# ivanalberico/End-To-End-Self-Supervised-SLAM

Measured on AMD Instinct MI355X. Metric: online refinement steps/sec @640x480, seq_len=60, higher is better.
Workload: dtype f32

## Files before the change

### end-to-end-self-supervised-slam_amd/csrc/conv.hip

```cpp
#include <cassert>
#include <type_traits>

#include "e2e_common.h"

typedef float f4v __attribute__((ext_vector_type(4)));
typedef float f16v __attribute__((ext_vector_type(16)));

#define CBK 16

enum { ACT_NONE = 0, ACT_RELU = 1, ACT_ELU = 2, ACT_DISP = 3 };

struct ConvArgs {
    const float* src0;
    const float* src1;
    const float* w;
    const float* scale;
    const float* shift;
    const float* res;
    float* out;
    int B, Hs, Ws;
    int Cin, C1, up;
    int Hd, Wd;
    int Ncols, ldw;
    int KH, KW, stride, pad, pad_mode;
// ... 1060 lines not shown
                        int ys = oh * a.stride + b_kh[j] - a.pad, xs = ow * a.stride + b_kw[j] - a.pad;
                        bool ok = true;
                        if (a.pad_mode == 1) { ys = reflect1(ys, a.Hs); xs = reflect1(xs, a.Ws); }
                        else ok = ys >= 0 && ys < a.Hs && xs >= 0 && xs < a.Ws;
                        if (ok) {
                            const int ci = b_ci[j];
                            const float* q = (ci < a.C1)
                                ? a.src0 + (((int64_t)b * Hl + ys / a.up) * Wl + xs / a.up) * a.C1 + ci
                                : a.src1 + (((int64_t)b * a.Hs + ys) * a.Ws + xs) * C2 + (ci - a.C1);
                            v = *(const f4v*)q;
                        }
                    } else if (a.has_bias && b_col[j] == Kconv) {
                        v[0] = 1.f;
                    }
                } else {
#pragma unroll
                    for (int e = 0; e < 4; ++e) {
                        const int n = b_col[j] + e;
                        if (n < Kconv) {
                            const int tp = n / a.Cin, c = n - tp * a.Cin, kh1 = tp / a.KW, kw1 = tp - kh1 * a.KW;
                            const int ys = oh * a.stride + kh1 - a.pad, xs = ow * a.stride + kw1 - a.pad;
                            if (ys >= 0 && ys < a.Hs && xs >= 0 && xs < a.Ws)
                                v[e] = (a.src0[(((int64_t)b * a.Hs + ys) * a.Ws + xs) * a.Cin + c] - a.in_sub) * a.in_mul;
                        } else if (a.has_bias && n == Kconv) v[e] = 1.f;
                    }
                }
            }
            breg[j] = v;
            pow_[j] += CBK;
            while (pow_[j] >= a.Wo) { pow_[j] -= a.Wo; if (++poh[j] == a.Ho) { poh[j] = 0; ++pb[j]; } }
        }
        ++ld_chunk;
    };
    auto store_chunk = [&](int buf) {
#pragma unroll
        for (int j = 0; j < A_PER; ++j) {
            const int idx = tid + j * NT;
            if (idx >= A_CNT) continue;
            const int kr = idx / (BM / 4), mq = idx - kr * (BM / 4);
            *(f4v*)&As[buf][kr][mq * 4] = areg[j];
        }
#pragma unroll
        for (int j = 0; j < B_PER; ++j) {
            const int idx = tid + j * NT;
            if (idx >= B_CNT) continue;
            const int nq = idx - b_kr[j] * (BN / 4);
            *(f4v*)&Bs[buf][b_kr[j]][nq * 4] = breg[j];
        }
    };
    f16v acc;
#pragma unroll
    for (int r = 0; r < 16; ++r) acc[r] = 0.f;
    if (nchunks > 0) {
        load_chunk();
        store_chunk(0);
    }
    __syncthreads();
    const int khalf = lane >> 5;
    for (int c = 0; c < nchunks; ++c) {
        const int buf = c & 1;
        if (c + 1 < nchunks) load_chunk();
        float av[CBK / 2], bv[CBK / 2];
#pragma unroll
        for (int kk = 0; kk < CBK / 2; ++kk) {
            av[kk] = As[buf][kk * 2 + khalf][wm * 32 + (lane & 31)];
            bv[kk] = Bs[buf][kk * 2 + khalf][wn * 32 + (lane & 31)];
        }
#pragma unroll
        for (int kk = 0; kk < CBK / 2; ++kk) acc = __builtin_amdgcn_mfma_f32_32x32x2f32(av[kk], bv[kk], acc, 0, 0, 0);
        __builtin_amdgcn_sched_group_barrier(0x100, CBK / 2, 0);
        __builtin_amdgcn_sched_group_barrier(0x008, CBK / 2, 0);
        if (c + 1 < nchunks) store_chunk(buf ^ 1);
        __syncthreads();
    }
    float* slab = a.slabs + (int64_t)bz * a.Mpad * a.Npad;
    const int n = nn0 + wn * 32 + (lane & 31);
#pragma unroll
    for (int r = 0; r < 16; ++r) {
        const int m = m0 + wm * 32 + (r & 3) + 8 * (r >> 2) + 4 * khalf;
        if (m < a.Mpad && n < a.Npad) slab[(int64_t)m * a.Npad + n] = acc[r];
    }
}

template <int WM, int WN, int CB>
struct WgradGemm4Lds {
    float As[2][CB][32 * WM];
    float Bs[2][CB][32 * WN];
};

template <int WM, int WN, int CB, bool TWO, class Ids>
__device__ __forceinline__ void wgrad_gemm4_body(const WgradArgs& a, const Ids& wg, float (*As)[CB][32 * WM], float (*Bs)[CB][32 * WN]) {
    constexpr int BM = 32 * WM, BN = 32 * WN, NT = 256;
    constexpr int A_CNT = CB * (BM / 4), B_CNT = CB * (BN / 4);
    constexpr int A_PER = A_CNT / NT, B_PER = B_CNT / NT;
    static_assert(A_CNT % NT == 0 && B_CNT % NT == 0, "tile / thread-count mismatch");
    const int tid = threadIdx.x, lane = tid & 63, wave = tid >> 6;
    const int wm = wave % WM, wn = wave / WM;
    unsigned bx, by, bz;
    set_wave_priority(wg.lin());
    {
        const unsigned lin = xcd_contiguous(wg.lin(), wg.gx() * wg.gy() * wg.gz());
        bx = lin % wg.gx();
        const unsigned t_ = lin / wg.gx();
        by = t_ % wg.gy();
        bz = t_ / wg.gy();
    }
    const int m0 = by * BM, nn0 = bx * BN;
    const int P = a.B * a.Ho * a.Wo;
    const int p0 = (int)((int64_t)bz * a.pix_per_slice);
    const int p1 = (p0 + a.pix_per_slice < P) ? (int)(p0 + a.pix_per_slice) : P;
    const int npix = (p1 > p0) ? p1 - p0 : 0;
    const int nchunks = (npix + CB - 1) / CB;
    const int sh = a.up >> 1;
    const int Hl = a.Hs >> sh, Wl = a.Ws >> sh, C2 = a.Cin - a.C1;
    const int Kconv = a.KH * a.KW * a.Cin;
    constexpr unsigned OOB = 0x80000000u;
    const __amdgpu_buffer_rsrc_t rsz = __builtin_amdgcn_make_buffer_rsrc((void*)a.dz, 0, (int)((int64_t)P * a.Cout * 4), 0x00020000);
    const __amdgpu_buffer_rsrc_t rs0 = __builtin_amdgcn_make_buffer_rsrc((void*)a.src0, 0, (int)((int64_t)a.B * Hl * Wl * a.C1 * 4), 0x00020000);
    const __amdgpu_buffer_rsrc_t rs1 = __builtin_amdgcn_make_buffer_rsrc((void*)(a.src1 ? a.src1 : a.src0), 0,
                                                                         (int)(a.src1 ? (int64_t)a.B * a.Hs * a.Ws * C2 * 4 : 0), 0x00020000);

    int a_kr[A_PER];
    unsigned a_off[A_PER];
#pragma unroll
    for (int j = 0; j < A_PER; ++j) {
        const int idx = tid + j * NT;
        a_kr[j] = idx / (BM / 4);
        const int m = m0 + (idx - a_kr[j] * (BM / 4)) * 4;
        a_off[j] = (m < a.Cout) ? (unsigned)(a_kr[j] * a.Cout + m) * 4u : OOB;
    }
    const float inv_cin = 1.0f / (float)a.Cin, inv_kw = 1.0f / (float)a.KW;
    constexpr int QG = (BN / 4) / B_PER;
    static_assert(NT / QG == CB, "one pixel row of the chunk per thread");
    const int b_row = tid / QG;
    int b_quad[B_PER], b_kh[B_PER], b_kw[B_PER], b_ci[B_PER];
    bool b_conv[B_PER], b_ones[B_PER], b_src0[B_PER];
#pragma unroll
    for (int j = 0; j < B_PER; ++j) {
        b_quad[j] = tid % QG + j * QG;
        const int col = nn0 + b_quad[j] * 4;
        b_conv[j] = col < Kconv;
        b_ones[j] = a.has_bias && col == Kconv;
        const int cc = b_conv[j] ? col : 0;
        int tap = (int)((float)cc * inv_cin);
        tap -= (tap * a.Cin > cc) ? 1 : 0;
        tap += ((tap + 1) * a.Cin <= cc) ? 1 : 0;
        b_ci[j] = cc - tap * a.Cin;
        b_src0[j] = b_ci[j] < a.C1;
        int tkh = (int)((float)tap * inv_kw);
        tkh -= (tkh * a.KW > tap) ? 1 : 0;
        tkh += ((tkh + 1) * a.KW <= tap) ? 1 : 0;
        b_kh[j] = tkh - a.pad;
        b_kw[j] = tap - tkh * a.KW - a.pad;
    }
    const int hw = a.Ho * a.Wo;
    const float inv_hw = 1.0f / (float)hw, inv_wo = 1.0f / (float)a.Wo;
    const bool reflect = a.pad_mode == 1;
    f4v areg[2][A_PER], breg[2][B_PER], breg1[2][TWO ? B_PER : 1];
    int left_of[2] = {0, 0};
    int ld_chunk = 0;
    int cur_b = 0, cur_oh = 0, cur_ow = 0;
    const bool incremental = a.Wo >= 11 && a.Ho >= 3;
    auto load_chunk = [&](int set) {
        const int left = npix - ld_chunk * CB;
        left_of[set] = left;
        const int pc = p0 + ld_chunk * CB;
        const int soffz = pc * a.Cout * 4;
#pragma unroll
        for (int j = 0; j < A_PER; ++j)
            areg[set][j] = __builtin_bit_cast(f4v, __builtin_amdgcn_raw_buffer_load_b128(rsz, (a_kr[j] < left) ? a_off[j] : OOB, soffz, 0));
        if (!incremental || ld_chunk == 0) {
            const unsigned p = (unsigned)(pc + b_row);
            unsigned b = (unsigned)((float)p * inv_hw);
            b -= (__umul24(b, (unsigned)hw) > p) ? 1u : 0u;
            b += (__umul24(b + 1u, (unsigned)hw) <= p) ? 1u : 0u;
            const unsigned r = p - __umul24(b, (unsigned)hw);
            unsigned oh = (unsigned)((float)r * inv_wo);
            oh -= (__umul24(oh, (unsigned)a.Wo) > r) ? 1u : 0u;
            oh += (__umul24(oh + 1u, (unsigned)a.Wo) <= r) ? 1u : 0u;
            cur_b = (int)b; cur_oh = (int)oh; cur_ow = (int)(r - __umul24(oh, (unsigned)a.Wo));
        } else {
            cur_ow += CB;
#pragma unroll
            for (int t = 0; t < 3; ++t) {
                const bool c = cur_ow >= a.Wo;
                cur_ow -= c ? a.Wo : 0;
                cur_oh += c ? 1 : 0;
            }
            const bool c = cur_oh >= a.Ho;
            cur_oh -= c ? a.Ho : 0;
            cur_b += c ? 1 : 0;
        }
        const int ybase = (int)__umul24((unsigned)cur_oh, (unsigned)a.stride), xbase = (int)__umul24((unsigned)cur_ow, (unsigned)a.stride);
#pragma unroll
        for (int j = 0; j < B_PER; ++j) {
            const int ys0 = ybase + b_kh[j], xs0 = xbase + b_kw[j];
            const bool inside = ((unsigned)ys0 < (unsigned)a.Hs) & ((unsigned)xs0 < (unsigned)a.Ws);
            const int ys = reflect ? reflect1(ys0, a.Hs) : ys0, xs = reflect ? reflect1(xs0, a.Ws) : xs0;
            const bool ok = b_conv[j] & (b_row < left) & (reflect | inside);
            const unsigned pix0 = umad24(umad24((unsigned)cur_b, (unsigned)Hl, (unsigned)(ys >> sh)), (unsigned)Wl, (unsigned)(xs >> sh));
            const unsigned o0 = umad24(pix0, (unsigned)a.C1, (unsigned)b_ci[j]) * 4u;
            breg[set][j] = __builtin_bit_cast(f4v, __builtin_amdgcn_raw_buffer_load_b128(rs0, o0 | ((ok && b_src0[j]) ? 0u : OOB), 0, 0));
            if (TWO) {
                const unsigned pix1 = umad24(umad24((unsigned)cur_b, (unsigned)a.Hs, (unsigned)ys), (unsigned)a.Ws, (unsigned)xs);
                const unsigned o1 = umad24(pix1, (unsigned)C2, (unsigned)(b_ci[j] - a.C1)) * 4u;
                breg1[set][j] = __builtin_bit_cast(f4v, __builtin_amdgcn_raw_buffer_load_b128(rs1, o1 | ((ok && !b_src0[j]) ? 0u : OOB), 0, 0));
            }
        }
        ++ld_chunk;
    };
    auto store_chunk = [&](int buf, int set) {
#pragma unroll
        for (int j = 0; j < A_PER; ++j) {
            const int idx = tid + j * NT;
            *(f4v*)&As[buf][a_kr[j]][(idx - a_kr[j] * (BM / 4)) * 4] = areg[set][j];
        }
#pragma unroll
        for (int j = 0; j < B_PER; ++j) {
            f4v v = breg[set][j];
            if (TWO) v = b_src0[j] ? v : breg1[set][j];
            const f4v ones = {(b_row < left_of[set]) ? 1.f : 0.f, 0.f, 0.f, 0.f};
            *(f4v*)&Bs[buf][b_row][b_quad[j] * 4] = b_ones[j] ? ones : v;
        }
    };
    f16v acc;
#pragma unroll
    for (int r = 0; r < 16; ++r) acc[r] = 0.f;
    load_chunk(0);
    load_chunk(1);
    store_chunk(0, 0);
    __syncthreads();
    const int khalf = lane >> 5;
    float fa[2][CB / 2], fb[2][CB / 2];
    auto read_frags = [&](auto buf_c) {
        constexpr int buf = decltype(buf_c)::value;
#pragma unroll
        for (int kk = 0; kk < CB / 2; ++kk) {
            fa[buf][kk] = As[buf][kk * 2 + khalf][wm * 32 + (lane & 31)];
            fb[buf][kk] = Bs[buf][kk * 2 + khalf][wn * 32 + (lane & 31)];
        }
    };
    auto pipe_step = [&](auto buf_c) {
        constexpr int buf = decltype(buf_c)::value;
        load_chunk(buf);
        store_chunk(buf ^ 1, buf ^ 1);
#pragma unroll
        for (int kk = 0; kk < CB / 4; ++kk) acc = __builtin_amdgcn_mfma_f32_32x32x2f32(fa[buf][kk], fb[buf][kk], acc, 0, 0, 0);
#pragma unroll
        for (int g = 0; g < CB / 4; ++g) {
            __builtin_amdgcn_sched_group_barrier(0x008, 1, 0);
            __builtin_amdgcn_sched_group_barrier(0x002, 14, 0);
            __builtin_amdgcn_sched_group_barrier(0x004, 4, 0);
            __builtin_amdgcn_sched_group_barrier(0x020, 1, 0);
            __builtin_amdgcn_sched_group_barrier(0x200, 1, 0);
        }
        __builtin_amdgcn_sched_barrier(0);
        __syncthreads();
        __builtin_amdgcn_sched_barrier(0);
        read_frags(std::integral_constant<int, buf ^ 1>{});
#pragma unroll
        for (int kk = CB / 4; kk < CB / 2; ++kk) acc = __builtin_amdgcn_mfma_f32_32x32x2f32(fa[buf][kk], fb[buf][kk], acc, 0, 0, 0);
#pragma unroll
        for (int g = 0; g < CB / 4; ++g) {
            __builtin_amdgcn_sched_group_barrier(0x008, 1, 0);
            __builtin_amdgcn_sched_group_barrier(0x100, 2, 0);
        }
        __builtin_amdgcn_sched_barrier(0);
    };
    if (nchunks > 0) {
        read_frags(std::integral_constant<int, 0>{});
        int c = 0;
        for (; c + 1 < nchunks; c += 2) {
            pipe_step(std::integral_constant<int, 0>{});
            pipe_step(std::integral_constant<int, 1>{});
        }
        if (c < nchunks) pipe_step(std::integral_constant<int, 0>{});
    }
    {
        const __amdgpu_buffer_rsrc_t rsl = __builtin_amdgcn_make_buffer_rsrc((void*)(a.slabs + (int64_t)bz * a.Mpad * a.Npad), 0, a.Mpad * a.Npad * 4, 0x00020000);
        const int n = nn0 + wn * 32 + (lane & 31), mb = m0 + wm * 32 + 4 * khalf;
        const int rows_left = a.Mpad - mb;
        const unsigned voff = (n < a.Npad && rows_left > 0) ? (unsigned)(mb * a.Npad + n) * 4u : OOB;
#pragma unroll
        for (int r = 0; r < 16; ++r) {
            const int dr = (r & 3) + 8 * (r >> 2);
            const float v = acc[r];
            __builtin_amdgcn_raw_buffer_store_b32(__float_as_uint(v), rsl, (dr < rows_left) ? voff : OOB, dr * a.Npad * 4, 0);
        }
    }
}

template <int WM, int WN, int CB, bool TWO>
__global__ __launch_bounds__(256) void k_wgrad_gemm4(WgradArgs a) {
    __shared__ float As[2][CB][32 * WM];
    __shared__ float Bs[2][CB][32 * WN];
    wgrad_gemm4_body<WM, WN, CB, TWO>(a, HwIds{}, As, Bs);
}

struct PairGrid {
    unsigned dgx, dgy, dgz;
    unsigned wgx, wgy, wgz;
    unsigned first;
    int wgrad_first;
};

template <int DWM, int DWN, bool TWO>
__global__ __launch_bounds__(256) void k_conv_bwd_pair(ConvArgs d, WgradArgs w, PairGrid pg) {
    using DL = ConvGemmLds<DWM, DWN, 1, 1, 4, 32>;
    using WL = WgradGemm4Lds<2, 2, 32>;
    static_assert(64 * DWM * DWN == 256, "both parts run 256 threads");
    __shared__ union { DL d; WL w; } lds;
    const bool in_first = blockIdx.x < pg.first;
    const unsigned l = in_first ? blockIdx.x : blockIdx.x - pg.first;
    if (in_first == (pg.wgrad_first != 0)) {
        if (l >= pg.wgx * pg.wgy * pg.wgz) return;
        wgrad_gemm4_body<2, 2, 32, TWO>(w, PartIds{l, pg.wgx, pg.wgy, pg.wgz}, lds.w.As, lds.w.Bs);
    } else {
        if (l >= pg.dgx * pg.dgy * pg.dgz) return;
        conv_gemm_body<DWM, DWN, 1, 1, 4, true, 32>(d, PartIds{l, pg.dgx, pg.dgy, pg.dgz}, lds.d.As, lds.d.Bs);
    }
}

template <int NTL, int CB>
__global__ __launch_bounds__(256) void k_wgrad_gemm16(WgradArgs a) {
    constexpr int BM = 16, BN = 16 * NTL, BNS = (BN % 32 == 16) ? BN : BN + 16, NT = 256;
    constexpr int A_CNT = CB * (BM / 4), B_CNT = CB * (BN / 4);
    constexpr int A_PER = (A_CNT + NT - 1) / NT, B_PER = (B_CNT + NT - 1) / NT;
    static_assert(2 * CB * (BM + BNS) >= 3 * NTL * 4 * 64, "tile memory is reused for the cross-wave sum");
    __shared__ float smem[2 * CB * (BM + BNS)];
    float (*As)[CB][BM] = reinterpret_cast<float (*)[CB][BM]>(smem);
    float (*Bs)[CB][BNS] = reinterpret_cast<float (*)[CB][BNS]>(smem + 2 * CB * BM);
    const int tid = threadIdx.x, lane = tid & 63, wave = tid >> 6;
    WGRAD_BLOCK_IDS
    (void)by;
    const int nn0 = bx * BN;
    const int64_t P = (int64_t)a.B * a.Ho * a.Wo;
    const int64_t p0 = (int64_t)bz * a.pix_per_slice;
    const int64_t p1 = (p0 + a.pix_per_slice < P) ? p0 + a.pix_per_slice : P;
    const int npix = (p1 > p0) ? (int)(p1 - p0) : 0;
    const int nchunks = (npix + CB - 1) / CB;
    const int sh = a.up >> 1;
    const int Hl = a.Hs >> sh, Wl = a.Ws >> sh, C2 = a.Cin - a.C1;
    const int Kconv = a.KH * a.KW * a.Cin;
    constexpr unsigned OOB = 0x80000000u;
    const __amdgpu_buffer_rsrc_t rsz = __builtin_amdgcn_make_buffer_rsrc((void*)a.dz, 0, (int)(P * a.Cout * 4), 0x00020000);
    const __amdgpu_buffer_rsrc_t rs0 = __builtin_amdgcn_make_buffer_rsrc((void*)a.src0, 0, (int)((int64_t)a.B * Hl * Wl * a.C1 * 4), 0x00020000);
    const __amdgpu_buffer_rsrc_t rs1 = __builtin_amdgcn_make_buffer_rsrc((void*)(a.src1 ? a.src1 : a.src0), 0,
                                                                         (int)(a.src1 ? (int64_t)a.B * a.Hs * a.Ws * C2 * 4 : 0), 0x00020000);
    int a_kr[A_PER];
    unsigned a_off[A_PER];
#pragma unroll
    for (int j = 0; j < A_PER; ++j) {
        const int idx = tid + j * NT;
        a_kr[j] = idx / (BM / 4);
        const int m = (idx - a_kr[j] * (BM / 4)) * 4;
        a_off[j] = (idx < A_CNT && m < a.Cout) ? (unsigned)(a_kr[j] * a.Cout + m) * 4u : OOB;
    }
    int b_kr[B_PER], b_kh[B_PER], b_kw[B_PER], b_ci[B_PER], pb[B_PER], poh[B_PER], pow_[B_PER];
    bool b_conv[B_PER], b_ones[B_PER], b_src0[B_PER];
#pragma unroll
    for (int j = 0; j < B_PER; ++j) {
        const int idx = tid + j * NT;
        b_kr[j] = idx / (BN / 4);
        const int col = nn0 + (idx - b_kr[j] * (BN / 4)) * 4;
        b_conv[j] = idx < B_CNT && col < Kconv;
        b_ones[j] = idx < B_CNT && a.has_bias && col == Kconv;
        const int tap = b_conv[j] ? col / a.Cin : 0;
        b_ci[j] = b_conv[j] ? col - tap * a.Cin : 0;
        b_src0[j] = b_ci[j] < a.C1;
        b_kh[j] = tap / a.KW;
        b_kw[j] = tap - b_kh[j] * a.KW;
        const int64_t p = p0 + b_kr[j];
        const int hw = a.Ho * a.Wo;
        pb[j] = (int)(p / hw);
        const int r = (int)(p - (int64_t)pb[j] * hw);
        poh[j] = r / a.Wo;
        pow_[j] = r - poh[j] * a.Wo;
    }
    f4v areg[A_PER], breg[B_PER];
    int ld_chunk = 0;
    auto load_chunk = [&]() {
        const int left = npix - ld_chunk * CB;
        const int soffz = (int)((p0 + (int64_t)ld_chunk * CB) * a.Cout * 4);
#pragma unroll
        for (int j = 0; j < A_PER; ++j)
            areg[j] = __builtin_bit_cast(f4v, __builtin_amdgcn_raw_buffer_load_b128(rsz, (a_kr[j] < left) ? a_off[j] : OOB, soffz, 0));
#pragma unroll
        for (int j = 0; j < B_PER; ++j) {
            int ys = poh[j] * a.stride + b_kh[j] - a.pad, xs = pow_[j] * a.stride + b_kw[j] - a.pad;
            bool ok = b_conv[j] && b_kr[j] < left;
            if (a.pad_mode == 1) { ys = reflect1(ys, a.Hs); xs = reflect1(xs, a.Ws); }
            else ok = ok && ys >= 0 && ys < a.Hs && xs >= 0 && xs < a.Ws;
            const unsigned o0 = (unsigned)(((pb[j] * Hl + (ys >> sh)) * Wl + (xs >> sh)) * a.C1 + b_ci[j]) * 4u;
            const unsigned o1 = (unsigned)(((pb[j] * a.Hs + ys) * a.Ws + xs) * C2 + (b_ci[j] - a.C1)) * 4u;
            f4v v = __builtin_bit_cast(f4v, __builtin_amdgcn_raw_buffer_load_b128(rs0, (ok && b_src0[j]) ? o0 : OOB, 0, 0));
            if (a.src1 != nullptr) {
                const f4v v1 = __builtin_bit_cast(f4v, __builtin_amdgcn_raw_buffer_load_b128(rs1, (ok && !b_src0[j]) ? o1 : OOB, 0, 0));
                v = b_src0[j] ? v : v1;
            }
            if (b_ones[j]) v = (f4v){(b_kr[j] < left) ? 1.f : 0.f, 0.f, 0.f, 0.f};
            breg[j] = v;
            pow_[j] += CB;
#pragma unroll
            for (int w2 = 0; w2 < 4; ++w2)
                if (pow_[j] >= a.Wo) { pow_[j] -= a.Wo; if (++poh[j] == a.Ho) { poh[j] = 0; ++pb[j]; } }
        }
        ++ld_chunk;
    };
    auto store_chunk = [&](int buf) {
#pragma unroll
        for (int j = 0; j < A_PER; ++j) {
            const int idx = tid + j * NT;
            if (idx >= A_CNT) continue;
            *(f4v*)&As[buf][a_kr[j]][(idx - a_kr[j] * (BM / 4)) * 4] = areg[j];
        }
#pragma unroll
        for (int j = 0; j < B_PER; ++j) {
            const int idx = tid + j * NT;
            if (idx >= B_CNT) continue;
            *(f4v*)&Bs[buf][b_kr[j]][(idx - b_kr[j] * (BN / 4)) * 4] = breg[j];
        }
    };
    f4v acc[NTL];
#pragma unroll
    for (int t = 0; t < NTL; ++t) acc[t] = (f4v){0.f, 0.f, 0.f, 0.f};
    if (nchunks > 0) {
        load_chunk();
        store_chunk(0);
    }
    __syncthreads();
    const int kq = lane >> 4, l16 = lane & 15;
    for (int c = 0; c < nchunks; ++c) {
        const int buf = c & 1;
        if (c + 1 < nchunks) load_chunk();
#pragma unroll
        for (int ks = 0; ks < CB / 16; ++ks) {
            const int row = wave * (CB / 4) + ks * 4 + kq;
            const float av = As[buf][row][l16];
#pragma unroll
            for (int t = 0; t < NTL; ++t) acc[t] = __builtin_amdgcn_mfma_f32_16x16x4f32(av, Bs[buf][row][t * 16 + l16], acc[t], 0, 0, 0);
        }
        if (c + 1 < nchunks) store_chunk(buf ^ 1);
        __syncthreads();
    }
    float* red = smem;
    if (wave > 0) {
#pragma unroll
        for (int t = 0; t < NTL; ++t)
#pragma unroll
            for (int i = 0; i < 4; ++i) red[((wave - 1) * NTL * 4 + t * 4 + i) * 64 + lane] = acc[t][i];
    }
    __syncthreads();
    if (wave > 0) return;
    float* slab = a.slabs + (int64_t)bz * a.Mpad * a.Npad;
#pragma unroll
    for (int t = 0; t < NTL; ++t)
#pragma unroll
        for (int i = 0; i < 4; ++i) {
            float v = acc[t][i];
#pragma unroll
            for (int w2 = 0; w2 < 3; ++w2) v += red[(w2 * NTL * 4 + t * 4 + i) * 64 + lane];
            const int m = 4 * kq + i, n = nn0 + t * 16 + l16;
            if (n < a.Npad) slab[(int64_t)m * a.Npad + n] = v;
        }
}

struct ThinWgradArgs {
    const float* dz;
    const float* src0;
    const float* src1;
    float* slabs;
    int B, Hd, Wd, Cin, C1, up, npad, has_bias, tiles_x, nxg;
};

template <int MT>
__global__ __launch_bounds__(256) void k_wgrad3x3_thin(ThinWgradArgs a) {
    constexpr int TH = 4, TW = 64, PH = TH + 2, PW = TW + 2, CO = 16 * MT, NA = 10 * MT;
    __shared__ float smem[PH * PW * 16 + TH * TW * CO];
    float* patch = smem;
    float* dzs = smem + PH * PW * 16;
    const int tid = threadIdx.x, lane = tid & 63, wave = tid >> 6, l16 = lane & 15, kq = lane >> 4;
    const int nhalf = a.Cin >> 4, n0 = a.C1 >> 4;
    const int b = blockIdx.z / nhalf, hf = blockIdx.z % nhalf;
    const bool first = hf < n0;
    const int sh = first ? (a.up >> 1) : 0, Cs = first ? a.C1 : a.Cin - a.C1, cs0 = (first ? hf : hf - n0) * 16;
    const int Hs = a.Hd >> sh, Ws = a.Wd >> sh;
    const int y0 = blockIdx.y * TH;
    const float* sb = (first ? a.src0 : a.src1) + (int64_t)b * Hs * Ws * Cs + cs0;
    const float* zb = a.dz + (int64_t)b * a.Hd * a.Wd * CO;
    f4v acc[NA];
#pragma unroll
    for (int t = 0; t < NA; ++t) acc[t] = (f4v){0.f, 0.f, 0.f, 0.f};
    const float one = (l16 == 0) ? 1.f : 0.f;
    for (int tx = 0; tx < a.tiles_x; ++tx) {
        const int x0 = (blockIdx.x * a.tiles_x + tx) * TW;
        if (x0 >= a.Wd) break;
        __syncthreads();
        for (int idx = tid; idx < PH * PW * 4; idx += 256) {
            const int q = idx & 3, pix = idx >> 2;
            const int py = pix / PW, px = pix - py * PW;
            const int Y = min(max(reflect1(y0 - 1 + py, a.Hd), 0), a.Hd - 1), X = min(max(reflect1(x0 - 1 + px, a.Wd), 0), a.Wd - 1);
            *(f4v*)&patch[pix * 16 + q * 4] = *(const f4v*)(sb + ((int64_t)(Y >> sh) * Ws + (X >> sh)) * Cs + q * 4);
        }
        for (int idx = tid; idx < TH * TW * (CO / 4); idx += 256) {
            const int q = idx % (CO / 4), pix = idx / (CO / 4);
            const int r = pix / TW, x = pix - r * TW;
            const bool ok = y0 + r < a.Hd && x0 + x < a.Wd;
            *(f4v*)&dzs[pix * CO + q * 4] = ok ? *(const f4v*)(zb + ((int64_t)(y0 + r) * a.Wd + x0 + x) * CO + q * 4) : (f4v){0.f, 0.f, 0.f, 0.f};
        }
        __syncthreads();
        const float* ap = dzs + (wave * TW + kq) * CO + l16;
        const float* bp = patch + (wave * PW + kq) * 16 + l16;
#pragma unroll 2
        for (int ks = 0; ks < TW / 4; ++ks) {
            float av[MT];
#pragma unroll
            for (int mt = 0; mt < MT; ++mt) av[mt] = ap[ks * 4 * CO + mt * 16];
#pragma unroll
            for (int t = 0; t < 9; ++t) {
                const float bv = bp[((t / 3) * PW + (t % 3)) * 16 + ks * 64];
#pragma unroll
                for (int mt = 0; mt < MT; ++mt) acc[mt * 10 + t] = __builtin_amdgcn_mfma_f32_16x16x4f32(av[mt], bv, acc[mt * 10 + t], 0, 0, 0);
            }
#pragma unroll
            for (int mt = 0; mt < MT; ++mt) acc[mt * 10 + 9] = __builtin_amdgcn_mfma_f32_16x16x4f32(av[mt], one, acc[mt * 10 + 9], 0, 0, 0);
        }
    }
    float* red = smem;
    static_assert(2 * NA * 4 * 64 <= PH * PW * 16 + TH * TW * CO, "reduction scratch");
    __syncthreads();
    if (wave >= 2) {
#pragma unroll
        for (int t = 0; t < NA; ++t)
#pragma unroll
            for (int i = 0; i < 4; ++i) red[((wave - 2) * NA * 4 + t * 4 + i) * 64 + lane] = acc[t][i];
    }
    __syncthreads();
    if (wave < 2) {
#pragma unroll
        for (int t = 0; t < NA; ++t)
#pragma unroll
            for (int i = 0; i < 4; ++i) acc[t][i] += red[(wave * NA * 4 + t * 4 + i) * 64 + lane];
    }
    __syncthreads();
    if (wave == 1) {
#pragma unroll
        for (int t = 0; t < NA; ++t)
#pragma unroll
            for (int i = 0; i < 4; ++i) red[(t * 4 + i) * 64 + lane] = acc[t][i];
    }
    __syncthreads();
    if (wave != 0) return;
    const int64_t sid = ((int64_t)b * gridDim.y + blockIdx.y) * a.nxg + blockIdx.x;
    float* slab = a.slabs + sid * CO * a.npad;
    const int kconv = 9 * a.Cin, cg0 = hf * 16;
#pragma unroll
    for (int mt = 0; mt < MT; ++mt)
#pragma unroll
        for (int t = 0; t < 10; ++t)
#pragma unroll
            for (int i = 0; i < 4; ++i) {
                const float v = acc[mt * 10 + t][i] + red[((mt * 10 + t) * 4 + i) * 64 + lane];
                const int co = mt * 16 + 4 * kq + i;
                if (t < 9) slab[co * a.npad + t * a.Cin + cg0 + l16] = v;
                else if (a.has_bias && hf == 0 && l16 == 0) slab[co * a.npad + kconv] = v;
            }
}

struct StemWgradArgs {
    const float* dz;
    const float* src;
    float* slabs;
    int B, Hs, Ws, Hd, Wd, tiles_x, nxg;
    float in_sub, in_mul;
};

__global__ __launch_bounds__(256) void k_wgrad7x7_stem(StemWgradArgs a) {
    constexpr int TH = 4, TW = 32, PH = 2 * TH + 6, PW = 2 * TW + 5, ROW = 208, NPAD = 148;
    __shared__ float patch[PH * ROW];
    __shared__ float dzs[TH * TW * 64];
    const int tid = threadIdx.x, lane = tid & 63, wave = tid >> 6, l16 = lane & 15, kq = lane >> 4;
    const int y0 = blockIdx.y * TH, b = blockIdx.z;
    int offn[10];
#pragma unroll
    for (int nt = 0; nt < 10; ++nt) {
        const int k = 16 * nt + l16;
        offn[nt] = k + (k / 21) * (ROW - 21) + 48 * kq;
    }
    f4v acc[10];
#pragma unroll
    for (int nt = 0; nt < 10; ++nt) acc[nt] = (f4v){0.f, 0.f, 0.f, 0.f};
    const float* sb = a.src + (int64_t)b * a.Hs * a.Ws * 3;
    const float* zb = a.dz + (int64_t)b * a.Hd * a.Wd * 64;
    for (int tx = 0; tx < a.tiles_x; ++tx) {
        const int x0 = (blockIdx.x * a.tiles_x + tx) * TW;
        if (x0 >= a.Wd) break;
        __syncthreads();
        for (int idx = tid; idx < PH * ROW; idx += 256) {
            const int py = idx / ROW, e = idx - py * ROW;
            const int Y = 2 * y0 - 3 + py, X = 2 * x0 - 3 + e / 3;
            const bool ok = e < 3 * PW && Y >= 0 && Y < a.Hs && X >= 0 && X < a.Ws;
            patch[idx] = ok ? (sb[((int64_t)Y * a.Ws + X) * 3 + (e - (e / 3) * 3)] - a.in_sub) * a.in_mul : 0.f;
        }
        for (int idx = tid; idx < TH * TW * 16; idx += 256) {
            const int q = idx & 15, pix = idx >> 4;
            const int r = pix / TW, x = pix - r * TW;
            const bool ok = y0 + r < a.Hd && x0 + x < a.Wd;
            *(f4v*)&dzs[pix * 64 + q * 4] = ok ? *(const f4v*)(zb + ((int64_t)(y0 + r) * a.Wd + x0 + x) * 64 + q * 4) : (f4v){0.f, 0.f, 0.f, 0.f};
        }
        __syncthreads();
#pragma unroll 1
        for (int r = 0; r < TH; ++r) {
            const float* ap = dzs + (r * TW + 8 * kq) * 64 + 16 * wave + l16;
            const float* bp = patch + 2 * r * ROW;
#pragma unroll 2
            for (int ks = 0; ks < TW / 4; ++ks) {
                const float av = ap[ks * 64];
#pragma unroll
                for (int nt = 0; nt < 10; ++nt) acc[nt] = __builtin_amdgcn_mfma_f32_16x16x4f32(av, bp[offn[nt] + ks * 6], acc[nt], 0, 0, 0);
            }
        }
    }
    float* slab = a.slabs + (((int64_t)b * gridDim.y + blockIdx.y) * a.nxg + blockIdx.x) * 64 * NPAD;
#pragma unroll
    for (int nt = 0; nt < 10; ++nt)
#pragma unroll
        for (int i = 0; i < 4; ++i) {
            const int n = 16 * nt + l16;
            if (n < 147) slab[(16 * wave + 4 * kq + i) * NPAD + n] = acc[nt][i];
        }
}

struct TapWgradArgs {
    const float* dz;
    const float* src0;
    const float* src1;
    float* slabs;
    int B, H, W, Cin, C1, up, Cout, reflect, has_bias, Mpad, Npad;
    int ptx, pty;
    int nchunks, cps;
};

#define TAP_NT 192
template <bool BIAS>
__global__ __launch_bounds__(TAP_NT) void k_wgrad3x3_taps(TapWgradArgs a) {
    __shared__ float dzs[64 * 32];
    __shared__ float xs[100 * 32];
    const int tid = threadIdx.x, lane = tid & 63, wave = tid >> 6, kh_ = lane >> 5, l32 = lane & 31;
    const int ci0 = blockIdx.x * 32, co0 = blockIdx.y * 32;
    const bool first = ci0 < a.C1;
    const int sh = first ? (a.up >> 1) : 0, Cs = first ? a.C1 : a.Cin - a.C1, cs0 = first ? ci0 : ci0 - a.C1;
    const int Hs = a.H >> sh, Ws = a.W >> sh;
    const float* sbase = first ? a.src0 : a.src1;
    const int c_begin = blockIdx.z * a.cps, c_end = min(c_begin + a.cps, a.nchunks);
    const bool want_bias = BIAS && blockIdx.x == 0 && wave == 0;
    f16v acc[3], accb;
#pragma unroll
    for (int t = 0; t < 3; ++t)
#pragma unroll
        for (int r = 0; r < 16; ++r) acc[t][r] = 0.f;
#pragma unroll
    for (int r = 0; r < 16; ++r) accb[r] = 0.f;
    const float one = (l32 == 0) ? 1.f : 0.f;
    f4v rz[3], rx[5];
    auto load_chunk = [&](int g) {
        const int b = g / (a.pty * a.ptx), rem = g - b * (a.pty * a.ptx), py = rem / a.ptx, px = rem - py * a.ptx;
        const int y0 = py * 8, x0 = px * 8;
        const float* zb = a.dz + (int64_t)b * a.H * a.W * a.Cout + co0;
        const float* sb = sbase + (int64_t)b * Hs * Ws * Cs + cs0;
#pragma unroll
        for (int i = 0; i < 3; ++i) {
            const int f = tid + TAP_NT * i, pix = f >> 3, q = f & 7, y = y0 + (pix >> 3), x = x0 + (pix & 7);
            const bool ok = f < 512 && y < a.H && x < a.W;
            rz[i] = ok ? *(const f4v*)(zb + ((int64_t)y * a.W + x) * a.Cout + q * 4) : (f4v){0.f, 0.f, 0.f, 0.f};
        }
#pragma unroll
        for (int i = 0; i < 5; ++i) {
            const int f = tid + TAP_NT * i;
            f4v v = {0.f, 0.f, 0.f, 0.f};
            if (f < 800) {
                const int pix = f >> 3, q = f & 7;
                int y = y0 - 1 + pix / 10, x = x0 - 1 + pix % 10;
                bool ok = true;
                if (a.reflect) {
                    y = min(max(reflect1(y, a.H), 0), a.H - 1);
                    x = min(max(reflect1(x, a.W), 0), a.W - 1);
                } else {
                    ok = y >= 0 && y < a.H && x >= 0 && x < a.W;
                }
                if (ok) v = *(const f4v*)(sb + ((int64_t)(y >> sh) * Ws + (x >> sh)) * Cs + q * 4);
            }
            rx[i] = v;
        }
    };
    auto store_chunk = [&]() {
#pragma unroll
        for (int i = 0; i < 3; ++i) {
            const int f = tid + TAP_NT * i;
            if (f < 512) *(f4v*)&dzs[f * 4] = rz[i];
        }
#pragma unroll
        for (int i = 0; i < 5; ++i) {
            const int f = tid + TAP_NT * i;
            if (f < 800) *(f4v*)&xs[f * 4] = rx[i];
        }
    };
    if (c_begin < c_end) load_chunk(c_begin);
    const float* ap = dzs + kh_ * 32 + l32;
    const float* bp = xs + (kh_ + wave * 10) * 32 + l32;
    for (int c = c_begin; c < c_end; ++c) {
        __syncthreads();
        store_chunk();
        __syncthreads();
        if (c + 1 < c_end) load_chunk(c + 1);
        constexpr int QB = 4, NQ = 32 / QB;
        float av[2][QB], bv[2][QB][3];
        auto read_q = [&](int set, int qt) {
#pragma unroll
            for (int j = 0; j < QB; ++j) {
                const int ks = QB * qt + j, q0 = (ks >> 2) * 10 + 2 * (ks & 3);
                av[set][j] = ap[2 * ks * 32];
#pragma unroll
                for (int t = 0; t < 3; ++t) bv[set][j][t] = bp[(q0 + t) * 32];
            }
        };
        auto pin_q = [&](int set) {
#pragma unroll
            for (int j = 0; j < QB; ++j) {
                asm volatile("" : "+v"(av[set][j]));
#pragma unroll
                for (int t = 0; t < 3; ++t) asm volatile("" : "+v"(bv[set][j][t]));
            }
        };
        read_q(0, 0);
#pragma unroll
        for (int qt = 0; qt < NQ; ++qt) {
            if (qt + 1 < NQ) read_q((qt + 1) & 1, qt + 1);
            __builtin_amdgcn_sched_barrier(0);
            pin_q(qt & 1);
            __builtin_amdgcn_sched_barrier(0);
#pragma unroll
            for (int j = 0; j < QB; ++j) {
#pragma unroll
                for (int t = 0; t < 3; ++t) acc[t] = __builtin_amdgcn_mfma_f32_32x32x2f32(av[qt & 1][j], bv[qt & 1][j][t], acc[t], 0, 0, 0);
                if (BIAS && want_bias) accb = __builtin_amdgcn_mfma_f32_32x32x2f32(av[qt & 1][j], one, accb, 0, 0, 0);
            }
            __builtin_amdgcn_sched_barrier(0);
        }
    }
    float* slab = a.slabs + (int64_t)blockIdx.z * a.Mpad * a.Npad;
#pragma unroll
    for (int t = 0; t < 3; ++t)
#pragma unroll
        for (int r = 0; r < 16; ++r) {
            const int m = co0 + (r & 3) + 8 * (r >> 2) + 4 * kh_;
            slab[(int64_t)m * a.Npad + (wave * 3 + t) * a.Cin + ci0 + l32] = acc[t][r];
        }
    if (BIAS && want_bias && l32 == 0) {
#pragma unroll
        for (int r = 0; r < 16; ++r) slab[(int64_t)(co0 + (r & 3) + 8 * (r >> 2) + 4 * kh_) * a.Npad + 9 * a.Cin] = accb[r];
    }
}

template <int ZL>
__device__ __forceinline__ void wgrad_reduce_group(const float* __restrict__ slabs, int S, int Mpad, int Npad, int Cout, int Cin, int KH, int KW, int has_bias,
                                                   float* __restrict__ dw, float* __restrict__ dbias, int accumulate, const float* __restrict__ scale,
                                                   int64_t base, int e, int w, f4v (*part)[64]) {
    const int Kconv = KH * KW * Cin, Ng = Kconv + (has_bias ? 1 : 0);
    const int nq = (Ng + 3) / 4;
    const int64_t totalq = (int64_t)Cout * nq;
    const int64_t slab_q = (int64_t)Mpad * Npad / 4;
    const f4v zero = {0.f, 0.f, 0.f, 0.f};
    const int64_t q = base + e;
    const bool on = q < totalq;
    const int m = on ? (int)(q / nq) : 0, n = on ? (int)(q - (int64_t)m * nq) * 4 : 0;
    const f4v* src = (const f4v*)(slabs + (int64_t)m * Npad + n);
    f4v sacc = zero;
    int z = w;
    for (; z + 3 * ZL < S; z += 4 * ZL) {
        f4v v[4];
#pragma unroll
        for (int j = 0; j < 4; ++j) v[j] = on ? src[(int64_t)(z + ZL * j) * slab_q] : zero;
#pragma unroll
        for (int j = 0; j < 4; ++j) sacc += v[j];
    }
    for (; z < S; z += ZL) sacc += on ? src[(int64_t)z * slab_q] : zero;
    part[w][e] = sacc;
    __syncthreads();
    if (w == 0 && on) {
        f4v t = part[0][e];
#pragma unroll
        for (int j = 1; j < ZL; ++j) t += part[j][e];
        const float sc = scale ? scale[m] : 1.f;
#pragma unroll
        for (int k = 0; k < 4; ++k) {
            const int nn = n + k;
            if (nn < Kconv) {
                const int tap = nn / Cin, ci = nn - tap * Cin, kh = tap / KW, kw = tap - kh * KW;
                float* d = dw + (((int64_t)m * Cin + ci) * KH + kh) * KW + kw;
                const float v = scale ? t[k] * sc : t[k];
                *d = accumulate ? *d + v : v;
            } else if (nn == Kconv && dbias) {
                dbias[m] = accumulate ? dbias[m] + t[k] : t[k];
            }
        }
    }
    __syncthreads();
}

template <int ZL>
__global__ __launch_bounds__(64 * ZL) void k_wgrad_reduce(const float* __restrict__ slabs, int S, int Mpad, int Npad, int Cout, int Cin,
                                                         int KH, int KW, int has_bias, float* __restrict__ dw, float* __restrict__ dbias,
                                                         int accumulate, const float* __restrict__ scale) {
    __shared__ f4v part[ZL][64];
    const int64_t totalq = (int64_t)Cout * ((KH * KW * Cin + (has_bias ? 1 : 0) + 3) / 4);
    for (int64_t base = (int64_t)blockIdx.x * 64; base < totalq; base += (int64_t)gridDim.x * 64)
        wgrad_reduce_group<ZL>(slabs, S, Mpad, Npad, Cout, Cin, KH, KW, has_bias, dw, dbias, accumulate, scale, base, threadIdx.x & 63, threadIdx.x >> 6, part);
}

__global__ __launch_bounds__(512) void k_wgrad_reduce_batched(const e2e_wgrad_reduce_desc* __restrict__ d, int n, long long total_items) {
    __shared__ f4v part[8][64];
    const int e = threadIdx.x & 63, w = threadIdx.x >> 6;
    for (long long item = blockIdx.x; item < total_items; item += gridDim.x) {
        int lo = 0, hi = n - 1;
        while (lo < hi) {
            const int mid = (lo + hi + 1) >> 1;
            if (d[mid].first_item <= item) lo = mid; else hi = mid - 1;
        }
        const e2e_wgrad_reduce_desc D = d[lo];
        const long long local = item - D.first_item;
        if (D.zl == 8)
            wgrad_reduce_group<8>(D.slabs, D.S, D.Mpad, D.Npad, D.Cout, D.Cin, D.KH, D.KW, D.has_bias, D.dw, D.dbias, D.accumulate, D.scale, local * 64, e, w, part);
        else
            wgrad_reduce_group<2>(D.slabs, D.S, D.Mpad, D.Npad, D.Cout, D.Cin, D.KH, D.KW, D.has_bias, D.dw, D.dbias, D.accumulate, D.scale,
                                  (local * 4 + (w >> 1)) * 64, e, w & 1, part + 2 * (w >> 1));
    }
}

__global__ __launch_bounds__(256) void k_weight_layouts(const float* __restrict__ w, int Cout, int Cin, int KH, int KW,
                                                        float* __restrict__ wf, int ldf, float* __restrict__ wb, int ldb) {
    const int64_t total = (int64_t)Cout * Cin * KH * KW;
    for (int64_t i = (int64_t)blockIdx.x * 256 + threadIdx.x; i < total; i += (int64_t)gridDim.x * 256) {
        int64_t t = i;
        const int kw = (int)(t % KW); t /= KW;
        const int kh = (int)(t % KH); t /= KH;
        const int ci = (int)(t % Cin); t /= Cin;
        const int co = (int)t;
        const float v = w[i];
        if (wf) wf[((int64_t)(kh * KW + kw) * Cin + ci) * ldf + co] = v;
        if (wb) wb[((int64_t)(kh * KW + kw) * Cout + co) * ldb + ci] = v;
    }
}

constexpr int WL_TS = 32, WL_ELEMS = 1024, WL_MAXL = 256;

template <int T>
__device__ __forceinline__ void weight_layout_tile(const float* __restrict__ w, float* __restrict__ wf, float* __restrict__ wb, const float* __restrict__ bsc,
                                                   int Cout, int Cin, int ldf, int ldb, int co0, int ci0, float* tile) {
    constexpr int R = WL_TS * T + 1;
    const int nci = min(WL_TS, Cin - ci0), nco = min(WL_TS, Cout - co0);
    const int lane = threadIdx.x & 63, wave = threadIdx.x >> 6;
    const int row = nci * T;
    if ((Cin & 3) == 0 && ((uintptr_t)w & 15) == 0) {
        const int rot = (lane >> 3) & 3;
        for (int co_l = wave; co_l < nco; co_l += 4) {
            const f4v* src = (const f4v*)(w + ((int64_t)(co0 + co_l) * Cin + ci0) * T);
            float* dst = tile + co_l * R;
            for (int x = lane; x < row / 4; x += 64) {
                const f4v v = src[x];
#pragma unroll
                for (int s = 0; s < 4; ++s) {
                    const int k = (s + rot) & 3;
                    dst[4 * x + k] = k == 0 ? v[0] : k == 1 ? v[1] : k == 2 ? v[2] : v[3];
                }
            }
        }
    } else {
        for (int co_l = wave; co_l < nco; co_l += 4) {
            const float* src = w + ((int64_t)(co0 + co_l) * Cin + ci0) * T;
            float* dst = tile + co_l * R;
            for (int x = lane; x < row; x += 64) dst[x] = src[x];
        }
    }
    __syncthreads();
    const int l32 = threadIdx.x & 31, g = threadIdx.x >> 5;
    if (wf) {
        const int co_l = (l32 & 7) * 4, ci_l = g * 4 + (l32 >> 3);
        if (ci_l < nci && co_l < nco) {
            const bool quad = co_l + 4 <= nco && (((uintptr_t)wf | (uintptr_t)(ldf * 4)) & 15) == 0;
            const float* s = tile + co_l * R + ci_l * T;
#pragma unroll
            for (int tap = 0; tap < T; ++tap) {
                const f4v v = {s[tap], s[R + tap], s[2 * R + tap], s[3 * R + tap]};
                float* o = wf + ((int64_t)tap * Cin + ci0 + ci_l) * ldf + co0 + co_l;
                if (quad) *(f4v*)o = v;
                else
#pragma unroll
                    for (int k = 0; k < 4; ++k)
                        if (co_l + k < nco) o[k] = v[k];
            }
        }
    }
    if (wb) {
        const int ci_l = (l32 & 7) * 4, co_l = g * 4 + (l32 >> 3);
        if (co_l < nco && ci_l < nci) {
            const bool quad = ci_l + 4 <= nci && (((uintptr_t)wb | (uintptr_t)(ldb * 4)) & 15) == 0;
            const float sc = bsc ? bsc[co0 + co_l] : 1.f;
            const float* s = tile + co_l * R + ci_l * T;
#pragma unroll
            for (int tap = 0; tap < T; ++tap) {
                f4v v = {s[tap], s[T + tap], s[2 * T + tap], s[3 * T + tap]};
                if (bsc) v *= sc;
                float* o = wb + ((int64_t)tap * Cout + co0 + co_l) * ldb + ci0 + ci_l;
                if (quad) *(f4v*)o = v;
                else
#pragma unroll
                    for (int k = 0; k < 4; ++k)
                        if (ci_l + k < nci) o[k] = v[k];
            }
        }
    }
    __syncthreads();
}

__global__ __launch_bounds__(256) void k_weight_layouts_batched(const long long* __restrict__ desc, int nlayers) {
    __shared__ float tile[WL_TS * (WL_TS * 9 + 1)];
    __shared__ int cnt[WL_MAXL], pre[WL_MAXL + 1];
    for (int i = threadIdx.x; i < nlayers; i += 256) {
        const long long* d = desc + (int64_t)i * 10;
        const int Cout = (int)d[3], Cin = (int)d[4], T = (int)d[5] * (int)d[6];
        cnt[i] = (T == 1 || T == 9) ? ((Cout + WL_TS - 1) / WL_TS) * ((Cin + WL_TS - 1) / WL_TS) : (int)(((int64_t)Cout * Cin * T + WL_ELEMS - 1) / WL_ELEMS);
    }
    __syncthreads();
    for (int i = threadIdx.x; i <= nlayers; i += 256) {
        int s = 0;
        for (int j = 0; j < i; ++j) s += cnt[j];
        pre[i] = s;
    }
    __syncthreads();
    const int total = pre[nlayers];
    for (int t = blockIdx.x; t < total; t += gridDim.x) {
        int lo = 0, hi = nlayers - 1;
        while (lo < hi) {
            const int mid = (lo + hi + 1) >> 1;
            if (pre[mid] <= t) lo = mid; else hi = mid - 1;
        }
        lo = __builtin_amdgcn_readfirstlane(lo);
        const int local = t - pre[lo];
        const long long* d = desc + (int64_t)lo * 10;
        const float* __restrict__ w = (const float*)d[0];
        float* __restrict__ wf = (float*)d[1];
        float* __restrict__ wb = (float*)d[2];
        const int Cout = (int)d[3], Cin = (int)d[4], KH = (int)d[5], KW = (int)d[6], ldf = (int)d[7], ldb = (int)d[8];
        const float* __restrict__ bsc = (const float*)d[9];
        const int T = KH * KW;
        if (T == 1 || T == 9) {
            const int nit = (Cin + WL_TS - 1) / WL_TS;
            const int co0 = (local / nit) * WL_TS, ci0 = (local % nit) * WL_TS;
            if (T == 9) weight_layout_tile<9>(w, wf, wb, bsc, Cout, Cin, ldf, ldb, co0, ci0, tile);
            else weight_layout_tile<1>(w, wf, wb, bsc, Cout, Cin, ldf, ldb, co0, ci0, tile);
        } else {
            const int64_t total_e = (int64_t)Cout * Cin * T;
            for (int64_t i = (int64_t)local * WL_ELEMS + threadIdx.x; i < min(total_e, (int64_t)(local + 1) * WL_ELEMS); i += 256) {
                const int tap = (int)(i % T);
                const int64_t r = i / T;
                const int ci = (int)(r % Cin), co = (int)(r / Cin);
                const float v = w[i];
                if (wf) wf[((int64_t)tap * Cin + ci) * ldf + co] = v;
                if (wb) wb[((int64_t)tap * Cout + co) * ldb + ci] = bsc ? v * bsc[co] : v;
            }
        }
    }
}

__global__ __launch_bounds__(256) void k_act_bwd(const float* __restrict__ dy, const float* __restrict__ y, const float* __restrict__ scale,
                                                 float* __restrict__ dz, int64_t n, int C, int act, int accumulate) {
    for (int64_t i = (int64_t)blockIdx.x * 256 + threadIdx.x; i < n; i += (int64_t)gridDim.x * 256) {
        float g = dy[i];
        const float v = y[i];
        if (act == ACT_RELU) g = v > 0.f ? g : 0.f;
        else if (act == ACT_ELU) g = v > 0.f ? g : g * (v + 1.f);
        else if (act == ACT_DISP) { const float s = (v - 0.01f) * 0.1f; g = g * 10.f * s * (1.f - s); }
        if (scale) g *= scale[i % C];
        dz[i] = accumulate ? dz[i] + g : g;
    }
}

__global__ __launch_bounds__(256) void k_gather_adjoint(const float* __restrict__ dxp, int B, int Hs, int Ws, int Cin, int C1, int up,
                                                        int pp, float* __restrict__ d0, float* __restrict__ d1, int acc0, int acc1,
                                                        const float* __restrict__ x0, int act0, const float* __restrict__ x1, int act1) {
    const int Hp = Hs + 2 * pp, Wp = Ws + 2 * pp, C2 = Cin - C1, Hl = Hs / up, Wl = Ws / up;
    const int64_t n0 = (int64_t)B * Hl * Wl * C1, n1 = (int64_t)B * Hs * Ws * C2;
    for (int64_t i = (int64_t)blockIdx.x * 256 + threadIdx.x; i < n0 + n1; i += (int64_t)gridDim.x * 256) {
        const bool first = i < n0;
        int64_t t = first ? i : i - n0;
        const int Cx = first ? C1 : C2, Hx = first ? Hl : Hs, Wx = first ? Wl : Ws, u = first ? up : 1;
        const int c = (int)(t % Cx); t /= Cx;
        const int x = (int)(t % Wx); t /= Wx;
        const int y = (int)(t % Hx); t /= Hx;
        const int b = (int)t;
        const int cc = first ? c : C1 + c;
        float s = 0.f;
        for (int dy = 0; dy < u; ++dy)
            for (int dx = 0; dx < u; ++dx) {
                const int fy = y * u + dy, fx = x * u + dx;
                int ys[3] = {fy + pp, -1, -1}, xs[3] = {fx + pp, -1, -1};
                if (pp) {
                    if (fy == 1) ys[1] = 0;
                    if (fy == Hs - 2) ys[2] = Hp - 1;
                    if (fx == 1) xs[1] = 0;
                    if (fx == Ws - 2) xs[2] = Wp - 1;
                }
                for (int iy = 0; iy < 3; ++iy)
                    for (int ix = 0; ix < 3; ++ix)
                        if (ys[iy] >= 0 && xs[ix] >= 0) s += dxp[(((int64_t)b * Hp + ys[iy]) * Wp + xs[ix]) * Cin + cc];
            }
        float* d = first ? d0 + i : d1 + (i - n0);
        const int acc = first ? acc0 : acc1;
        if (first ? act0 : act1) s *= act_deriv(first ? x0[i] : x1[i - n0], first ? act0 : act1);
        *d = acc ? *d + s : s;
    }
}

__global__ __launch_bounds__(256) void k_gather_adjoint4(const float* __restrict__ dxp, int B, int Hs, int Ws, int Cin, int C1, int up,
                                                         int pp, float* __restrict__ d0, float* __restrict__ d1, int acc0, int acc1,
                                                         const float* __restrict__ x0, int act0, const float* __restrict__ x1, int act1) {
    const int Hp = Hs + 2 * pp, Wp = Ws + 2 * pp, C2 = Cin - C1, Hl = Hs / up, Wl = Ws / up;
    const unsigned q0 = (unsigned)B * Hl * Wl * (C1 >> 2), q1 = (unsigned)B * Hs * Ws * (C2 >> 2);
    for (unsigned i = blockIdx.x * 256u + threadIdx.x; i < q0 + q1; i += gridDim.x * 256u) {
        const bool first = i < q0;
        unsigned t = first ? i : i - q0;
        const unsigned Cq = (unsigned)(first ? C1 : C2) >> 2, Hx = first ? Hl : Hs, Wx = first ? Wl : Ws;
        const int u = first ? up : 1;
        const unsigned cq = t % Cq; t /= Cq;
        const unsigned x = t % Wx; t /= Wx;
        const unsigned y = t % Hx;
        const unsigned b = t / Hx;
        const int cc = (first ? 0 : C1) + (int)cq * 4;
        f4v s = {0.f, 0.f, 0.f, 0.f};
        for (int dy = 0; dy < u; ++dy)
            for (int dx = 0; dx < u; ++dx) {
                const int fy = (int)y * u + dy, fx = (int)x * u + dx;
                int ys[3] = {fy + pp, -1, -1}, xs[3] = {fx + pp, -1, -1};
                if (pp) {
                    if (fy == 1) ys[1] = 0;
                    if (fy == Hs - 2) ys[2] = Hp - 1;
                    if (fx == 1) xs[1] = 0;
                    if (fx == Ws - 2) xs[2] = Wp - 1;
                }
#pragma unroll
                for (int iy = 0; iy < 3; ++iy)
#pragma unroll
                    for (int ix = 0; ix < 3; ++ix)
                        if (ys[iy] >= 0 && xs[ix] >= 0) s += *(const f4v*)(dxp + (((int64_t)b * Hp + ys[iy]) * Wp + xs[ix]) * Cin + cc);
            }
        const int64_t e = (int64_t)(first ? i : i - q0) * 4;
        const int act = first ? act0 : act1;
        if (act) {
            const f4v xv = *(const f4v*)((first ? x0 : x1) + e);
#pragma unroll
            for (int k = 0; k < 4; ++k) s[k] *= act_deriv(xv[k], act);
        }
        f4v* d = (f4v*)((first ? d0 : d1) + e);
        if (first ? acc0 : acc1) s += *d;
        *d = s;
    }
}

#define HC 16
__global__ __launch_bounds__(256) void k_head_fwd(const float* __restrict__ x, const float* __restrict__ w ,
                                                  const float* __restrict__ bias, float* __restrict__ y, int B, int H, int W, int act) {
    __shared__ float sw[9 * HC];
    for (int i = threadIdx.x; i < 9 * HC; i += 256) {
        const int ci = i / 9, tap = i - ci * 9;
        sw[tap * HC + ci] = w[i];
    }
    __syncthreads();
    const int64_t N = (int64_t)B * H * W;
    const int q = threadIdx.x & 3;
    for (int64_t n0 = (int64_t)blockIdx.x * 64; n0 < N; n0 += (int64_t)gridDim.x * 64) {
        const int64_t n = n0 + (threadIdx.x >> 2);
        const bool on = n < N;
        const int64_t nn = on ? n : N - 1;
        const int b = (int)(nn / ((int64_t)H * W));
        const int r = (int)(nn - (int64_t)b * H * W), h = r / W, ww = r - h * W;
        float acc = 0.f;
#pragma unroll
        for (int kh = 0; kh < 3; ++kh)
#pragma unroll
            for (int kw = 0; kw < 3; ++kw) {
                const int ys = reflect1(h + kh - 1, H), xs = reflect1(ww + kw - 1, W);
                const f4v v = *(const f4v*)(x + (((int64_t)b * H + ys) * W + xs) * HC + q * 4);
                const float* wt = &sw[(kh * 3 + kw) * HC + q * 4];
                acc = fmaf(v[0], wt[0], fmaf(v[1], wt[1], fmaf(v[2], wt[2], fmaf(v[3], wt[3], acc))));
            }
        acc += __shfl_xor(acc, 1, 64);
        acc += __shfl_xor(acc, 2, 64);
        if (on && q == 0) y[n] = apply_act(acc + (bias ? bias[0] : 0.f), act);
    }
}

__global__ __launch_bounds__(256) void k_head_bwd_data(const float* __restrict__ dz, const float* __restrict__ w, float* __restrict__ dx,
                                                       int B, int H, int W, const float* __restrict__ xin, int dact) {
    __shared__ float sw[9 * HC];
    for (int i = threadIdx.x; i < 9 * HC; i += 256) {
        const int ci = i / 9, tap = i - ci * 9;
        sw[tap * HC + ci] = w[i];
    }
    __syncthreads();
    const int64_t N = (int64_t)B * H * W;
    const int cq = threadIdx.x & 3;
    for (int64_t n = (int64_t)blockIdx.x * 64 + (threadIdx.x >> 2); n < N; n += (int64_t)gridDim.x * 64) {
        const int b = (int)(n / ((int64_t)H * W));
        const int r = (int)(n - (int64_t)b * H * W), h = r / W, ww = r - h * W;
        f4v acc = {0.f, 0.f, 0.f, 0.f};
        const int ry = (h == 1) ? 0 : ((h == H - 2) ? H + 1 : -100);
        const int rx = (ww == 1) ? 0 : ((ww == W - 2) ? W + 1 : -100);
        const float* gz = dz + (int64_t)b * H * W;
#pragma unroll
        for (int kh = 0; kh < 3; ++kh)
#pragma unroll
            for (int kw = 0; kw < 3; ++kw) {
                const float* wt = &sw[(kh * 3 + kw) * HC + cq * 4];
                const int qy0 = h - kh + 1, qx0 = ww - kw + 1, qy1 = ry - kh, qx1 = rx - kw;
                const bool y0 = qy0 >= 0 && qy0 < H, x0 = qx0 >= 0 && qx0 < W, y1 = qy1 >= 0 && qy1 < H, x1 = qx1 >= 0 && qx1 < W;
                float g = (y0 && x0) ? gz[(int64_t)qy0 * W + qx0] : 0.f;
                if (y1 | x1) {
                    if (y0 && x1) g += gz[(int64_t)qy0 * W + qx1];
                    if (y1 && x0) g += gz[(int64_t)qy1 * W + qx0];
                    if (y1 && x1) g += gz[(int64_t)qy1 * W + qx1];
                }
#pragma unroll
                for (int c = 0; c < 4; ++c) acc[c] = fmaf(g, wt[c], acc[c]);
            }
        if (dact) {
            const f4v xv = *(const f4v*)(xin + n * HC + cq * 4);
#pragma unroll
            for (int e = 0; e < 4; ++e) acc[e] *= act_deriv(xv[e], dact);
        }
// ... 69 lines not shown
    X(64, 64, 2, 2, 1, 1, 32) X(128, 64, 2, 2, 2, 1, 32) X(128, 128, 2, 2, 2, 2, 16) X(128, 32, 4, 1, 1, 1, 32) \
    X(32, 128, 1, 4, 1, 1, 32) X(32, 64, 1, 2, 1, 1, 32) X(64, 32, 2, 1, 1, 1, 32) X(32, 32, 1, 1, 1, 1, 32)
static int tile_max_cb(int bm, int bn) {
#define X(BM, BN, WM, WN, TM, TN, MAXCB) if (bm == BM && bn == BN) return MAXCB;
    CONV_TILE_SHAPES(X)
#undef X
    return 0;
}
static void demote_cb16_only(GemmCfg& c) { if (tile_max_cb(c.bm, c.bn) == 16) c.bn = 64; }

static GemmCfg choose_cfg(int64_t rows, int cols, int K, int cb, bool allow_split, GemmCfg force = GemmCfg{0, 0, 0}) {
    if (force.bm) { GemmCfg f = force; if (!allow_split && f.S > 1) f.S = 1; if (cb != 16) demote_cb16_only(f); return f; }
    GemmCfg c = {64, 64, 1};
    if (cols >= 128) { c.bm = 32; c.bn = 128; }
    if (cols <= 32) {
        c.bm = 128; c.bn = 32;
        if (((rows + 127) / 128) * ((cols + 31) / 32) < 600) c.bm = 64;
    }
    if (allow_split && cols > 32) {
        const int64_t tiles = ((rows + c.bm - 1) / c.bm) * ((cols + c.bn - 1) / c.bn);
        const int nchunks = (K + cb - 1) / cb;
        const int depth = nchunks * cb / 32;
        int S = tiles >= 500 ? 1 : depth < 30 ? 1 : depth < 60 ? 3 : depth < 120 ? 4 : 6;
        while (S < 12 && tiles * S < 200 && (nchunks / (S + 1)) * cb >= 288) ++S;
        while (S > 1 && tiles * S > 1300) --S;
        while (S > 1 && (nchunks / S) * cb < 288) --S;
        if (S < 1) S = 1;
        auto model = [&](int s) {
            const double wgs = (double)tiles * s, per_cu = wgs <= 256 ? 1 : wgs <= 512 ? 2 : wgs <= 768 ? 3 : 0;
            const double f = per_cu == 1 ? 1.0 : per_cu == 2 ? 1.76 : per_cu == 3 ? 2.41 : 2.41 * wgs / 768.0;
            return f * ((double)nchunks / s + 6.0) + (s > 1 ? 4.0 : 0.0);
        };
        if (tiles < 500 && S > 1) {
            int best = S;
            for (int s = S - 2; s <= S + 2; ++s) {
                if (s < 2 || s > 12 || s == S || (nchunks / s) * cb < 288 || tiles * s > 1300) continue;
                if (model(s) < 0.93 * model(best)) best = s;
            }
            S = best;
        }
        c.S = S;
    }
    return c;
}

template <bool TR>
static void launch_tile(ConvArgs& a, int cb, GemmCfg c, dim3 g, hipStream_t st) {
#define X(BM, BN, WM, WN, TM, TN, MAXCB)                                                                                                 \
    if (c.bm == BM && c.bn == BN) {                                                                                                      \
        if constexpr (MAXCB == 32)                                                                                                       \
            if (cb == 32) { hipLaunchKernelGGL((k_conv_gemm<WM, WN, TM, TN, 4, TR, 32>), g, dim3(64 * WM * WN), 0, st, a); return; }     \
        hipLaunchKernelGGL((k_conv_gemm<WM, WN, TM, TN, 4, TR, 16>), g, dim3(64 * WM * WN), 0, st, a);                                   \
        return;                                                                                                                          \
    }
    CONV_TILE_SHAPES(X)
#undef X
    assert(!"launch_tile: shape not in CONV_TILE_SHAPES");
}

template <bool TR>
static void launch_streamk(ConvArgs& a, int cb, int G, float* workspace, hipStream_t st) {
    const int64_t Ntot = (int64_t)a.B * a.Hd * a.Wd;
    SkArgs s;
    s.flags = (unsigned*)workspace;
    s.slabs = workspace + SK_FLAG_FLOATS;
    s.tiles_n = (a.Ncols + 63) / 64;
    s.C = a.KH * a.KW * a.Cin / cb;
    s.I = ((Ntot + 63) / 64) * s.tiles_n * (long long)s.C;
    if (G > SK_MAX_G) G = SK_MAX_G;
    if ((long long)G > s.I) G = (int)s.I;
    s.G = G;
    if (cb == 32) hipLaunchKernelGGL((k_conv_gemm_sk<TR, 32>), dim3(G), dim3(256), 0, st, a, s);
    else hipLaunchKernelGGL((k_conv_gemm_sk<TR, 16>), dim3(G), dim3(256), 0, st, a, s);
}

enum GemmKind { GK_SCALAR, GK_STREAMK, GK_TILE };
enum GemmTail { GT_NONE, GT_SPLITK4, GT_SPLITK, GT_CLS };
struct GemmLaunch { GemmKind kind; GemmTail tail; GemmCfg c; int cb; dim3 g; int G; };

#define CLS_TAP_SLICES 4
static int64_t cls_rows(int B, int Hd, int Wd) { return (int64_t)B * ((Hd + 1) / 2) * ((Wd + 1) / 2); }
static int64_t cls_slab_floats(int B, int Hd, int Wd, int cols) { return CLS_TAP_SLICES * 4 * cls_rows(B, Hd, Wd) * cols; }

template <bool TR>
static GemmLaunch plan_gemm(ConvArgs& a, int vec, float* workspace_all, GemmCfg force) {
    GemmLaunch p{GK_TILE, GT_NONE, GemmCfg{0, 0, 0}, 16, dim3(1), 0};
    const int64_t Ntot = (int64_t)a.B * a.Hd * a.Wd;
    const int K = a.KH * a.KW * a.Cin;
    const int cb = (vec == 4 && a.Cin % 32 == 0 && (a.C1 == a.Cin || a.C1 % 32 == 0)) ? 32 : 16;
    float* workspace = workspace_all ? workspace_all + SK_FLAG_FLOATS : nullptr;
    a.ksplit = 1; a.cps = 0; a.slab = workspace;
    a.bytes0 = (int64_t)a.B * (a.Hs / a.up) * (a.Ws / a.up) * a.C1 * 4;
    a.bytes1 = (int64_t)a.B * a.Hs * a.Ws * (a.Cin - a.C1) * 4;
    a.bytesw = (int64_t)K * a.ldw * 4;
    p.cb = cb;
    if (vec == 1) {
        p.kind = GK_SCALAR;
        p.g = dim3((unsigned)((Ntot + 127) / 128), (unsigned)((a.Ncols + 63) / 64));
        return p;
    }
    if (TR && a.cls) {
        const int64_t Nc = cls_rows(a.B, a.Hd, a.Wd);
        GemmCfg c = choose_cfg(Nc * 4, a.Ncols, (K * 9 / 16 + cb - 1) / cb * cb, cb, false, force.S < 0 ? GemmCfg{0, 0, 0} : force);
        demote_cb16_only(c);
        p.c = c;
        const int64_t total = Ntot * a.Ncols;
        const int64_t cls_wgs = 4 * ((Nc + c.bm - 1) / c.bm) * ((a.Ncols + c.bn - 1) / c.bn);
        if (workspace && cls_wgs < 500 && a.KH == 3 && a.KW == 3 && a.Cin % cb == 0 && a.Ncols % 4 == 0 && total < (1ll << 31) && !a.scale && !a.shift &&
            a.act == ACT_NONE) {
            a.ksplit = CLS_TAP_SLICES; a.cps = a.Cin / cb; a.cls_rows = Nc;
            p.g = dim3((unsigned)(4 * ((Nc + c.bm - 1) / c.bm)), (unsigned)((a.Ncols + c.bn - 1) / c.bn), (unsigned)CLS_TAP_SLICES);
            p.tail = GT_CLS;
            return p;
        }
        p.g = dim3((unsigned)(4 * ((Nc + c.bm - 1) / c.bm)), (unsigned)((a.Ncols + c.bn - 1) / c.bn));
        return p;
    }
    const GemmCfg c = choose_cfg(Ntot, a.Ncols, K, cb, workspace != nullptr, force);
    p.c = c;
    if (c.S < 0 && workspace && vec == 4 && K % cb == 0 && a.Cin % cb == 0) {
        p.kind = GK_STREAMK;
        p.G = -c.S;
        return p;
    }
    if (c.S > 1) {
        const int nchunks = (K + cb - 1) / cb;
        a.cps = (nchunks + c.S - 1) / c.S;
        const int Sz = (nchunks + a.cps - 1) / a.cps;
        a.ksplit = Sz;
        if (Sz > 1) {
            p.g = dim3((unsigned)((Ntot + c.bm - 1) / c.bm), (unsigned)((a.Ncols + c.bn - 1) / c.bn), (unsigned)Sz);
            const int64_t total = Ntot * a.Ncols;
            p.tail = (a.Ncols % 4 == 0 && total < (1ll << 31)) ? GT_SPLITK4 : GT_SPLITK;
            return p;
        }
        a.ksplit = 1; a.cps = 0;
    }
    p.g = dim3((unsigned)((Ntot + c.bm - 1) / c.bm), (unsigned)((a.Ncols + c.bn - 1) / c.bn));
    return p;
}

template <bool TR>
static void launch_gemm_main(ConvArgs& a, const GemmLaunch& p, float* workspace_all, hipStream_t st) {
    if (p.kind == GK_SCALAR) hipLaunchKernelGGL((k_conv_gemm<4, 1, 1, 2, 1, TR, 16>), p.g, dim3(256), 0, st, a);
    else if (p.kind == GK_STREAMK) launch_streamk<TR>(a, p.cb, p.G, workspace_all, st);
    else launch_tile<TR>(a, p.cb, p.c, p.g, st);
}

static void launch_gemm_tail(const ConvArgs& a, const GemmLaunch& p, hipStream_t st) {
    const int64_t total = (int64_t)a.B * a.Hd * a.Wd * a.Ncols;
    if (p.tail == GT_CLS)
        hipLaunchKernelGGL(k_conv_splitk_epilogue_cls, dim3(egrid(total / 4)), dim3(256), 0, st, a.slab, a.cls_rows, a.B, a.Hd, a.Wd, a.Ncols, a.KH, a.KW, a.off,
                           a.res, a.out, a.xin, a.dact, a.pre);
    else if (p.tail == GT_SPLITK4)
        hipLaunchKernelGGL(k_conv_splitk_epilogue4, dim3(egrid(total / 4)), dim3(256), 0, st, a.slab, a.ksplit, (unsigned)(total / 4), a.Ncols, a.scale, a.shift,
                           a.res, a.out, a.act, a.xin, a.dact, a.pre);
    else if (p.tail == GT_SPLITK)
        hipLaunchKernelGGL(k_conv_splitk_epilogue, dim3(egrid(total)), dim3(256), 0, st, a.slab, a.ksplit, total, a.Ncols, a.scale, a.shift, a.res, a.out, a.act,
                           a.xin, a.dact, a.pre);
}

template <bool TR>
static void launch_gemm(ConvArgs a, int vec, float* workspace_all, GemmCfg force, hipStream_t st) {
    const GemmLaunch p = plan_gemm<TR>(a, vec, workspace_all, force);
    launch_gemm_main<TR>(a, p, workspace_all, st);
    launch_gemm_tail(a, p, st);
}

extern "C" {

int e2e_conv_weight_layouts(const float* w, int Cout, int Cin, int KH, int KW, float* w_fwd, int ld_fwd, float* w_bwd,
                            int ld_bwd, void* stream) {
    E2E_REQUIRE(w && Cout > 0 && Cin > 0 && KH > 0 && KW > 0 && (w_fwd || w_bwd), E2E_ERR_ARG, "e2e_conv_weight_layouts: bad argument");
    E2E_REQUIRE((!w_fwd || (ld_fwd >= Cout && ld_fwd % 4 == 0)) && (!w_bwd || (ld_bwd >= Cin && ld_bwd % 4 == 0)), E2E_ERR_ARG,
                "e2e_conv_weight_layouts: leading dimensions must cover the columns and be multiples of 4");
    hipLaunchKernelGGL(k_weight_layouts, dim3(egrid((int64_t)Cout * Cin * KH * KW)), dim3(256), 0, (hipStream_t)stream, w, Cout, Cin, KH,
                       KW, w_fwd, ld_fwd, w_bwd, ld_bwd);
    E2E_LAUNCH_CHECK("e2e_conv_weight_layouts");
    return E2E_OK;
}

static int device_cus() {
    static const int cus = [] {
        int dev = 0, n = 0;
        if (hipGetDevice(&dev) != hipSuccess || hipDeviceGetAttribute(&n, hipDeviceAttributeMultiprocessorCount, dev) != hipSuccess || n <= 0) n = 256;
        return n;
    }();
    return cus;
}

int e2e_conv_weight_layouts_batched(const long long* desc, int nlayers, void* stream) {
    E2E_REQUIRE(desc && nlayers > 0, E2E_ERR_ARG, "e2e_conv_weight_layouts_batched: bad argument");
    const int grid = device_cus() * 8;
    for (int l0 = 0; l0 < nlayers; l0 += WL_MAXL)
        hipLaunchKernelGGL(k_weight_layouts_batched, dim3(grid), dim3(256), 0, (hipStream_t)stream, desc + (int64_t)l0 * 10, nlayers - l0 < WL_MAXL ? nlayers - l0 : WL_MAXL);
    E2E_LAUNCH_CHECK("e2e_conv_weight_layouts_batched");
    return E2E_OK;
}

int64_t e2e_conv2d_splitk_workspace_floats(int64_t rows, int cols, int K) {
    if (K % 16 != 0) return 0;
    int smax = 1;
    bool sk = false;
    for (int cb = 16; cb <= 32; cb += 16) {
        const GemmCfg c = choose_cfg(rows, cols, K, cb, true);
        if (c.S > smax) smax = c.S;
        if (c.S < 0) sk = true;
    }
    int64_t n = smax > 1 ? (int64_t)smax * rows * cols : 0;
    if (sk && n < (int64_t)SK_MAX_G * 64 * 64) n = (int64_t)SK_MAX_G * 64 * 64;
    return n ? n + SK_FLAG_FLOATS : 0;
}

int64_t e2e_conv2d_bwd_data_workspace_floats(int B, int Hd, int Wd, int cols, int K, int stride) {
    const int64_t plain = e2e_conv2d_splitk_workspace_floats((int64_t)B * Hd * Wd, cols, K);
    if (stride != 2) return plain;
    const int64_t cls = SK_FLAG_FLOATS + cls_slab_floats(B, Hd, Wd, cols);
    return cls > plain ? cls : plain;
}

int64_t e2e_conv_tuned_workspace_floats(int64_t rows, int cols) {
    int64_t n = (int64_t)16 * rows * cols;
    if (n < (int64_t)SK_MAX_G * 64 * 64) n = (int64_t)SK_MAX_G * 64 * 64;
    return n + SK_FLAG_FLOATS;
}
int e2e_conv_workspace_flag_floats(void) { return SK_FLAG_FLOATS; }
int e2e_conv_streamk_error_index(void) { return SK_ERR_INDEX; }

int e2e_conv_gemm_choice(int64_t rows, int cols, int K, int chunk_depth, int allow_split, int* out3) {
    E2E_REQUIRE(out3 && rows > 0 && cols > 0 && K > 0 && (chunk_depth == 16 || chunk_depth == 32), E2E_ERR_ARG, "e2e_conv_gemm_choice: bad argument");
    const GemmCfg c = choose_cfg(rows, cols, K, chunk_depth, allow_split != 0);
    out3[0] = c.bm; out3[1] = c.bn; out3[2] = c.S;
    return E2E_OK;
}

struct ConvGeom { int B, Hs, Ws, Cin, Cout, Ho, Wo, KH, KW, stride, pad, pad_mode, C1, up; float in_sub, in_mul; };
#define GEOM_LAYER(g) ConvGeom g{}; g.B = B; g.Hs = Hs; g.Ws = Ws; g.Cin = Cin; g.Cout = Cout; g.KH = KH; g.KW = KW; g.stride = stride; g.pad = pad; g.pad_mode = pad_mode
#define GEOM_SOURCES(g) g.C1 = C1; g.up = up; g.in_sub = in_sub; g.in_mul = in_mul
#define GEOM_OUTPUT(g) g.Ho = Ho; g.Wo = Wo
#define GEOM_BWD_DATA(g) GEOM_LAYER(g); GEOM_OUTPUT(g)
#define GEOM_BWD_WEIGHT(g) GEOM_LAYER(g); GEOM_OUTPUT(g); GEOM_SOURCES(g)
#define GEOM_WGRAD_QUERY(g) ConvGeom g{}; g.B = B; g.Ho = Ho; g.Wo = Wo; g.Cin = Cin; g.Cout = Cout; g.KH = KH; g.KW = KW
struct FwdOps { const float *src0, *src1, *w_fwd; int ld_fwd; const float *scale, *shift, *residual; float* out; int act; };
struct BwdDataOps { const float* dz; const float* w_bwd; int ld_bwd; float* dxp; int accumulate; const float* x_in; int in_act; const float* pre_add; };
struct WgradIn { const float *dz, *src0, *src1; float* workspace; };

static int conv_fwd_impl(const FwdOps& f, const ConvGeom& g, float* workspace, GemmCfg force, void* stream) {
    const int B = g.B, Hs = g.Hs, Ws = g.Ws, Cin = g.Cin, Cout = g.Cout, KH = g.KH, KW = g.KW, stride = g.stride, pad = g.pad, pad_mode = g.pad_mode;
    const int C1 = g.C1, up = g.up, ld_fwd = f.ld_fwd;
    E2E_REQUIRE(f.src0 && f.w_fwd && f.out && B > 0 && Hs > 0 && Ws > 0 && Cin > 0 && Cout > 0, E2E_ERR_ARG, "e2e_conv2d_fwd: bad argument");
    E2E_REQUIRE(up == 1 || up == 2, E2E_ERR_ARG, "e2e_conv2d_fwd: upsample factor must be 1 or 2");
    E2E_REQUIRE(C1 > 0 && C1 <= Cin && (C1 == Cin || f.src1), E2E_ERR_ARG, "e2e_conv2d_fwd: bad channel split");
    E2E_REQUIRE(pad_mode == 0 || (pad_mode == 1 && pad == 1 && Hs >= 2 && Ws >= 2), E2E_ERR_ARG, "e2e_conv2d_fwd: reflection padding needs pad == 1");
    E2E_REQUIRE(stride == 1 || stride == 2, E2E_ERR_ARG, "e2e_conv2d_fwd: stride must be 1 or 2");
    E2E_REQUIRE(Hs % up == 0 && Ws % up == 0 && ld_fwd % 4 == 0 && ld_fwd >= Cout, E2E_ERR_ARG, "e2e_conv2d_fwd: bad sizes");
    const int vec = (Cin % 16 == 0 && (C1 == Cin || C1 % 16 == 0)) ? 4 : 1;
    E2E_REQUIRE(vec == 4 || (C1 == Cin && up == 1), E2E_ERR_ARG, "e2e_conv2d_fwd: the scalar path (Cin %% 16 != 0) takes a single full-resolution source");
    E2E_REQUIRE((int64_t)B * Hs * Ws * Cin * 4 < (1ll << 30) && (int64_t)KH * KW * Cin * ld_fwd * 4 < (1ll << 31), E2E_ERR_ARG,
                "e2e_conv2d_fwd: activations must stay below 1 GB, weights below 2 GB (32-bit buffer offsets with out-of-range markers)");
    E2E_REQUIRE(vec != 4 || (KH <= 3 && KW <= 3), E2E_ERR_ARG, "e2e_conv2d_fwd: the channel-quad loader takes kernels up to 3 x 3");
    ConvArgs a{};
    a.src0 = f.src0; a.src1 = f.src1; a.w = f.w_fwd; a.scale = f.scale; a.shift = f.shift; a.res = f.residual; a.out = f.out;
    a.B = B; a.Hs = Hs; a.Ws = Ws; a.Cin = Cin; a.C1 = C1; a.up = up;
    a.Hd = (Hs + 2 * pad - KH) / stride + 1; a.Wd = (Ws + 2 * pad - KW) / stride + 1;
    a.Ncols = Cout; a.ldw = ld_fwd; a.KH = KH; a.KW = KW; a.stride = stride; a.pad = pad; a.pad_mode = pad_mode; a.off = 0; a.act = f.act;
    a.in_sub = g.in_sub; a.in_mul = g.in_mul;
    if (!force.bm && KH == 7 && KW == 7 && stride == 2 && pad == 3 && pad_mode == 0 && Cin == 3 && Cout == 64 && C1 == Cin && up == 1 && !f.residual && ld_fwd >= 64) {
        StemArgs t{f.src0, f.w_fwd, f.scale, f.shift, f.out, B, Hs, Ws, a.Hd, a.Wd, ld_fwd, f.act, g.in_sub, g.in_mul};
        hipLaunchKernelGGL(k_conv7x7_stem, dim3((a.Wd + 31) / 32, (a.Hd + 3) / 4, B), dim3(256), 0, (hipStream_t)stream, t);
    }
    else if (!force.bm && KH == 3 && KW == 3 && stride == 1 && pad == 1 && pad_mode == 1 && Cout == 16 && C1 == Cin && !f.scale && !f.residual && ld_fwd >= 16 &&
        ((Cin == 16 && up == 2) || (Cin == 32 && up == 1))) {
        ThinArgs t{f.src0, f.w_fwd, f.shift, f.out, B, Hs / up, Ws / up, Hs, Ws, ld_fwd, f.act, 1, 0};
        if (Cin == 16) hipLaunchKernelGGL((k_conv3x3_thin<16, 2, true, 8>), dim3((Ws + 63) / 64, (Hs + 7) / 8, B), dim3(256), 0, (hipStream_t)stream, t);
        else hipLaunchKernelGGL((k_conv3x3_thin<32, 1, true, 4>), dim3((Ws + 63) / 64, (Hs + 3) / 4, B), dim3(256), 0, (hipStream_t)stream, t);
    } else
        launch_gemm<false>(a, vec, workspace, force, (hipStream_t)stream);
    E2E_LAUNCH_CHECK("e2e_conv2d_fwd");
    return E2E_OK;
}

int e2e_conv2d_fwd(const float* src0, const float* src1, int C1, int up, const float* w_fwd, int ld_fwd, const float* scale,
                   const float* shift, const float* residual, float* out, int B, int Hs, int Ws, int Cin, int Cout, int KH,
                   int KW, int stride, int pad, int pad_mode, int act, float in_sub, float in_mul, float* workspace, void* stream) {
    GEOM_LAYER(g); GEOM_SOURCES(g);
    return conv_fwd_impl(FwdOps{src0, src1, w_fwd, ld_fwd, scale, shift, residual, out, act}, g, workspace, GemmCfg{0, 0, 0}, stream);
}

static bool tuning_ok(int tile_m, int tile_n, int ksplit) {
    if (tile_m == 0) return true;
    if (ksplit < 0) return tile_m == 64 && tile_n == 64 && -ksplit <= SK_MAX_G;
    return tile_max_cb(tile_m, tile_n) != 0 && ksplit >= 1 && ksplit <= 16;
}

int e2e_conv2d_fwd_tuned(const float* src0, const float* src1, int C1, int up, const float* w_fwd, int ld_fwd, const float* scale,
                         const float* shift, const float* residual, float* out, int B, int Hs, int Ws, int Cin, int Cout, int KH,
                         int KW, int stride, int pad, int pad_mode, int act, float in_sub, float in_mul, float* workspace, int tile_m, int tile_n,
                         int ksplit, void* stream) {
    E2E_REQUIRE(tuning_ok(tile_m, tile_n, ksplit), E2E_ERR_ARG, "e2e_conv2d_fwd_tuned: unsupported decomposition %d x %d / %d", tile_m, tile_n, ksplit);
    GEOM_LAYER(g); GEOM_SOURCES(g);
    return conv_fwd_impl(FwdOps{src0, src1, w_fwd, ld_fwd, scale, shift, residual, out, act}, g, workspace, GemmCfg{tile_m, tile_n, ksplit}, stream);
}

static int bwd_data_setup(const BwdDataOps& d, const ConvGeom& g, GemmCfg force, hipStream_t stream, ConvArgs& a, bool& done) {
    const int B = g.B, Hs = g.Hs, Ws = g.Ws, Cin = g.Cin, Cout = g.Cout, Ho = g.Ho, Wo = g.Wo, KH = g.KH, KW = g.KW, stride = g.stride, pad = g.pad;
    const int pad_mode = g.pad_mode, ld_bwd = d.ld_bwd;
    done = false;
    E2E_REQUIRE(d.pre_add == nullptr || pad_mode == 0, E2E_ERR_ARG, "e2e_conv2d_bwd_data: the pre-activation addend takes a zero-padded layer");
    E2E_REQUIRE(d.in_act == 0 || (d.x_in && (d.in_act == ACT_RELU || d.in_act == ACT_ELU) && pad_mode == 0), E2E_ERR_ARG,
                "e2e_conv2d_bwd_data: the fused input-activation derivative takes ReLU / ELU, the activation's output and a zero-padded layer");
    E2E_REQUIRE(d.dz && d.w_bwd && d.dxp && B > 0 && Cin > 0 && Cout > 0 && Cout % 16 == 0, E2E_ERR_ARG, "e2e_conv2d_bwd_data: bad argument (Cout %% 16 == 0)");
    E2E_REQUIRE(ld_bwd % 4 == 0 && ld_bwd >= Cin && (stride == 1 || stride == 2), E2E_ERR_ARG, "e2e_conv2d_bwd_data: bad sizes");
    E2E_REQUIRE((int64_t)B * Ho * Wo * Cout * 4 < (1ll << 30) && (int64_t)KH * KW * Cout * ld_bwd * 4 < (1ll << 31) && KH <= 3 && KW <= 3, E2E_ERR_ARG,
                "e2e_conv2d_bwd_data: gradients must stay below 1 GB, weights below 2 GB (32-bit buffer offsets), kernels up to 3 x 3");
    if (!force.bm && KH == 3 && KW == 3 && stride == 1 && pad == 1 && pad_mode == 1 && Cin == 16 && Cout == 16 && !d.accumulate && !d.in_act && !d.pre_add && ld_bwd >= 16) {
        ThinArgs t{d.dz, d.w_bwd, nullptr, d.dxp, B, Ho, Wo, Hs + 2, Ws + 2, ld_bwd, ACT_NONE, 2, 1};
        hipLaunchKernelGGL((k_conv3x3_thin<16, 1, false, 8>), dim3((Ws + 2 + 63) / 64, (Hs + 2 + 7) / 8, B), dim3(256), 0, stream, t);
        done = true;
        return E2E_OK;
    }
    a = ConvArgs{};
    a.src0 = d.dz; a.src1 = nullptr; a.w = d.w_bwd; a.out = d.dxp;
    a.B = B; a.Hs = Ho; a.Ws = Wo; a.Cin = Cout; a.C1 = Cout; a.up = 1;
    const int pp = pad_mode == 1 ? pad : 0;
    a.Hd = Hs + 2 * pp; a.Wd = Ws + 2 * pp; a.off = pad_mode == 1 ? 0 : pad;
    a.Ncols = Cin; a.ldw = ld_bwd; a.KH = KH; a.KW = KW; a.stride = stride; a.pad = pad; a.pad_mode = 0; a.act = ACT_NONE;
    a.cls = (stride == 2 && cls_rows(B, a.Hd, a.Wd) < (1 << 24)) ? 1 : 0;
    if (a.cls && (KH < 2 || KW < 2) && !d.accumulate)
        (void)hipMemsetAsync(d.dxp, 0, (size_t)B * a.Hd * a.Wd * Cin * sizeof(float), stream);
    if (d.accumulate) a.res = d.dxp;
    a.xin = d.in_act ? d.x_in : nullptr; a.dact = d.in_act; a.pre = d.pre_add;
    return E2E_OK;
}

static int bwd_data_impl(const BwdDataOps& d, const ConvGeom& g, float* workspace, void* stream, GemmCfg force = GemmCfg{0, 0, 0}) {
    ConvArgs a;
    bool done;
    const int rc = bwd_data_setup(d, g, force, (hipStream_t)stream, a, done);
    if (rc != E2E_OK) return rc;
    if (!done) launch_gemm<true>(a, 4, workspace, force, (hipStream_t)stream);
    E2E_LAUNCH_CHECK("e2e_conv2d_bwd_data");
    return E2E_OK;
}

int e2e_conv2d_bwd_data(const float* dz, const float* w_bwd, int ld_bwd, float* dxp, int B, int Hs, int Ws, int Cin, int Cout,
                        int Ho, int Wo, int KH, int KW, int stride, int pad, int pad_mode, float* workspace, void* stream) {
    GEOM_BWD_DATA(g);
    return bwd_data_impl(BwdDataOps{dz, w_bwd, ld_bwd, dxp, 0, nullptr, 0, nullptr}, g, workspace, stream);
}

int e2e_conv2d_bwd_data_acc(const float* dz, const float* w_bwd, int ld_bwd, float* dxp, int B, int Hs, int Ws, int Cin, int Cout,
                            int Ho, int Wo, int KH, int KW, int stride, int pad, int pad_mode, int accumulate, float* workspace,
                            void* stream) {
    GEOM_BWD_DATA(g);
    return bwd_data_impl(BwdDataOps{dz, w_bwd, ld_bwd, dxp, accumulate, nullptr, 0, nullptr}, g, workspace, stream);
}

int e2e_conv2d_bwd_data_fused(const float* da, const float* w_bwd, int ld_bwd, float* dxp, int B, int Hs, int Ws, int Cin, int Cout,
                              int Ho, int Wo, int KH, int KW, int stride, int pad, int pad_mode, int accumulate, const float* x_in,
                              int in_act, const float* pre_add, float* workspace, void* stream) {
    GEOM_BWD_DATA(g);
    return bwd_data_impl(BwdDataOps{da, w_bwd, ld_bwd, dxp, accumulate, x_in, in_act, pre_add}, g, workspace, stream);
}

int e2e_conv2d_bwd_data_fused_tuned(const float* da, const float* w_bwd, int ld_bwd, float* dxp, int B, int Hs, int Ws, int Cin, int Cout,
                                    int Ho, int Wo, int KH, int KW, int stride, int pad, int pad_mode, int accumulate, const float* x_in,
                                    int in_act, const float* pre_add, float* workspace, int tile_m, int tile_n, int ksplit, void* stream) {
    E2E_REQUIRE(tuning_ok(tile_m, tile_n, ksplit), E2E_ERR_ARG, "e2e_conv2d_bwd_data_fused_tuned: unsupported decomposition %d x %d / %d", tile_m, tile_n, ksplit);
    GEOM_BWD_DATA(g);
    return bwd_data_impl(BwdDataOps{da, w_bwd, ld_bwd, dxp, accumulate, x_in, in_act, pre_add}, g, workspace, stream, GemmCfg{tile_m, tile_n, ksplit});
}

struct GatherAdjoint { const float* dxp; int B, Hs, Ws, Cin, C1, up, padded; float *d0, *d1; int acc0, acc1; const float* x0; int act0; const float* x1; int act1; };
static void launch_gather_adjoint(const GatherAdjoint& q, hipStream_t st) {
    const int64_t n = (int64_t)q.B * (q.Hs / q.up) * (q.Ws / q.up) * q.C1 + (int64_t)q.B * q.Hs * q.Ws * (q.Cin - q.C1);
    if (q.Cin % 4 == 0 && q.C1 % 4 == 0 && n < (1ll << 31))
        hipLaunchKernelGGL(k_gather_adjoint4, dim3(egrid(n / 4)), dim3(256), 0, st, q.dxp, q.B, q.Hs, q.Ws, q.Cin, q.C1, q.up, q.padded ? 1 : 0, q.d0, q.d1, q.acc0, q.acc1,
                           q.x0, q.act0, q.x1, q.act1);
    else
        hipLaunchKernelGGL(k_gather_adjoint, dim3(egrid(n)), dim3(256), 0, st, q.dxp, q.B, q.Hs, q.Ws, q.Cin, q.C1, q.up, q.padded ? 1 : 0, q.d0, q.d1, q.acc0, q.acc1,
                           q.x0, q.act0, q.x1, q.act1);
}

int e2e_conv2d_gather_adjoint(const float* dxp, int B, int Hs, int Ws, int Cin, int C1, int up, int padded, float* d_src0,
                              float* d_src1, int accumulate0, int accumulate1, void* stream) {
    E2E_REQUIRE(dxp && d_src0 && B > 0 && Cin > 0 && C1 > 0 && C1 <= Cin && (C1 == Cin || d_src1) && (up == 1 || up == 2), E2E_ERR_ARG,
                "e2e_conv2d_gather_adjoint: bad argument");
    launch_gather_adjoint(GatherAdjoint{dxp, B, Hs, Ws, Cin, C1, up, padded, d_src0, d_src1, accumulate0, accumulate1, nullptr, 0, nullptr, 0}, (hipStream_t)stream);
    E2E_LAUNCH_CHECK("e2e_conv2d_gather_adjoint");
    return E2E_OK;
}

int e2e_conv2d_gather_adjoint_act(const float* dxp, int B, int Hs, int Ws, int Cin, int C1, int up, int padded, float* d_src0, float* d_src1,
                                  int accumulate0, int accumulate1, const float* src0, int act0, const float* src1, int act1, void* stream) {
    E2E_REQUIRE(dxp && d_src0 && B > 0 && Cin > 0 && C1 > 0 && C1 <= Cin && (C1 == Cin || d_src1) && (up == 1 || up == 2), E2E_ERR_ARG,
                "e2e_conv2d_gather_adjoint_act: bad argument");
    E2E_REQUIRE((act0 == 0 || src0) && (act1 == 0 || src1) && act0 >= 0 && act0 <= 2 && act1 >= 0 && act1 <= 2, E2E_ERR_ARG,
                "e2e_conv2d_gather_adjoint_act: an activation derivative needs the activation's output");
    launch_gather_adjoint(GatherAdjoint{dxp, B, Hs, Ws, Cin, C1, up, padded, d_src0, d_src1, accumulate0, accumulate1, src0, act0, src1, act1}, (hipStream_t)stream);
    E2E_LAUNCH_CHECK("e2e_conv2d_gather_adjoint_act");
    return E2E_OK;
}

int e2e_conv2d_act_bwd(const float* dy, const float* y, const float* scale, float* dz, int64_t n, int C, int act, void* stream) {
    E2E_REQUIRE(dy && y && dz && n > 0 && C > 0 && act >= 0 && act <= 3, E2E_ERR_ARG, "e2e_conv2d_act_bwd: bad argument");
    hipLaunchKernelGGL(k_act_bwd, dim3(egrid(n)), dim3(256), 0, (hipStream_t)stream, dy, y, scale, dz, n, C, act, 0);
    E2E_LAUNCH_CHECK("e2e_conv2d_act_bwd");
    return E2E_OK;
}

int e2e_conv2d_act_bwd_acc(const float* dy, const float* y, const float* scale, float* dz, int64_t n, int C, int act, int accumulate,
                           void* stream) {
    E2E_REQUIRE(dy && y && dz && n > 0 && C > 0 && act >= 0 && act <= 3, E2E_ERR_ARG, "e2e_conv2d_act_bwd_acc: bad argument");
    hipLaunchKernelGGL(k_act_bwd, dim3(egrid(n)), dim3(256), 0, (hipStream_t)stream, dy, y, scale, dz, n, C, act, accumulate);
    E2E_LAUNCH_CHECK("e2e_conv2d_act_bwd_acc");
    return E2E_OK;
}

#define HEAD_PARTS 2048
int e2e_head_fwd(const float* x, const float* w, const float* bias, float* y, int B, int H, int W, int Cin, int act, void* stream) {
    E2E_REQUIRE(x && w && y && B > 0 && H >= 2 && W >= 2 && Cin == HC, E2E_ERR_ARG, "e2e_head_fwd: bad argument (the head takes %d channels)", HC);
    hipLaunchKernelGGL(k_head_fwd, dim3(egrid((int64_t)B * H * W * 4)), dim3(256), 0, (hipStream_t)stream, x, w, bias, y, B, H, W, act);
    E2E_LAUNCH_CHECK("e2e_head_fwd");
    return E2E_OK;
}
int64_t e2e_head_workspace_floats(void) { return (int64_t)HEAD_PARTS * (9 * HC + 1); }
int e2e_head_bwd_act(const float* dz, const float* x, const float* w, float* dx, float* dw, float* dbias, float* workspace, int B, int H,
                     int W, int Cin, int in_act, void* stream) {
    E2E_REQUIRE(dz && x && w && workspace && B > 0 && H >= 2 && W >= 2 && Cin == HC && in_act >= 0 && in_act <= 2, E2E_ERR_ARG, "e2e_head_bwd: bad argument");
    E2E_REQUIRE((int64_t)B * H * W * HC < (1ll << 31), E2E_ERR_ARG, "e2e_head_bwd: activation too large for 32-bit element offsets");
    hipStream_t st = (hipStream_t)stream;
    if (dx) hipLaunchKernelGGL(k_head_bwd_data, dim3(egrid((int64_t)B * H * W * 4)), dim3(256), 0, st, dz, w, dx, B, H, W, x, in_act);
    if (dw) {
        hipLaunchKernelGGL(k_head_bwd_weight, dim3(HEAD_PARTS), dim3(256), 0, st, dz, x, workspace, B, H, W);
        hipLaunchKernelGGL(k_head_wreduce, dim3(9 * HC + 1), dim3(256), 0, st, workspace, HEAD_PARTS, dw, dbias);
    }
    E2E_LAUNCH_CHECK("e2e_head_bwd");
    return E2E_OK;
}

int e2e_head_bwd(const float* dz, const float* x, const float* w, float* dx, float* dw, float* dbias, float* workspace, int B, int H,
                 int W, int Cin, void* stream) {
    return e2e_head_bwd_act(dz, x, w, dx, dw, dbias, workspace, B, H, W, Cin, 0, stream);
}

enum WgradPath { WP_STEM, WP_THIN, WP_TAPS, WP_GEMM16, WP_GEMM_LEAN, WP_GEMM, WP_COUNT };
struct WgradPlan { WgradPath path; bool open; int64_t S; int Mpad, Npad, tm, tn, nxg, ny, tiles_x, ptx, pty, nchunks, cps; };
#define TAP_TARGET 640
static WgradPlan wgrad_plan(WgradPath path, const ConvGeom& g, int has_bias, bool tuned, int wg_target) {
    const int B = g.B, Ho = g.Ho, Wo = g.Wo, Cin = g.Cin, Cout = g.Cout, KH = g.KH, KW = g.KW;
    WgradPlan p{path};
    if (path == WP_STEM) {
        if (tuned || !(KH == 7 && KW == 7 && Cin == 3 && Cout == 64)) return p;
        p.nxg = ((Wo + 31) / 32 + 1) / 2; p.ny = (Ho + 3) / 4;
        p.S = (int64_t)B * p.ny * p.nxg; p.Mpad = 64; p.Npad = 148;
    } else if (path == WP_THIN) {
        if (tuned || !(KH == 3 && KW == 3 && ((Cout == 16 && (Cin == 16 || Cin == 32)) || (Cout == 32 && Cin == 96)))) return p;
        const int txt = (Wo + 63) / 64;
        p.ny = (Ho + 3) / 4;
        const int64_t total = (int64_t)B * p.ny * txt * (Cin / 16);
        p.tiles_x = 1;
        while (total / p.tiles_x > 1400 && p.tiles_x < txt) ++p.tiles_x;
        p.nxg = (txt + p.tiles_x - 1) / p.tiles_x;
        p.S = (int64_t)B * p.ny * p.nxg; p.Mpad = Cout; p.Npad = (9 * Cin + (has_bias ? 1 : 0) + 3) / 4 * 4;
    } else if (path == WP_TAPS) {
        if (tuned || !(KH == 3 && KW == 3 && Cin % 32 == 0 && Cout % 32 == 0)) return p;
        p.ptx = (Wo + 7) / 8; p.pty = (Ho + 7) / 8;
        p.nchunks = B * p.ptx * p.pty;
        const int tiles = (Cin / 32) * (Cout / 32);
        int S = (TAP_TARGET + tiles - 1) / tiles;
        if (S > p.nchunks) S = p.nchunks;
        if (S < 1) S = 1;
        p.cps = (p.nchunks + S - 1) / S;
        p.S = (p.nchunks + p.cps - 1) / p.cps; p.Mpad = Cout; p.Npad = (9 * Cin + (has_bias ? 1 : 0) + 3) / 4 * 4;
    } else {
        const bool use16 = path == WP_GEMM16;
        if (use16 && Cout != 16) return p;
        const int Ng = KH * KW * Cin + (has_bias ? 1 : 0);
        p.tm = Cout <= 32 ? 32 : 64; p.tn = Cout <= 32 ? 128 : 64;
        if (use16) { p.tm = 16; p.tn = 160; }
        p.Mpad = (Cout + p.tm - 1) / p.tm * p.tm; p.Npad = (Ng + p.tn - 1) / p.tn * p.tn;
        const int64_t P = (int64_t)B * Ho * Wo;
        const int64_t tiles = (int64_t)(p.Mpad / p.tm) * (p.Npad / p.tn);
        const int target = use16 ? wg_target * 3 / 4 : wg_target;
        int64_t S = (target + tiles - 1) / tiles;
        const int64_t maxS = (P + 255) / 256;
        if (S > maxS) S = maxS;
        if (S < 1) S = 1;
        p.S = S;
    }
    p.open = true;
    return p;
}

static int64_t wgrad_workspace_floats(const ConvGeom& g, int has_bias, bool tuned, int wg_target) {
    int64_t n = 0;
    for (int i = 0; i < WP_COUNT; ++i) {
        const WgradPlan p = wgrad_plan((WgradPath)i, g, has_bias, tuned, wg_target);
        if (p.open && p.S * p.Mpad * p.Npad > n) n = p.S * p.Mpad * p.Npad;
    }
    return n;
}

static WgradPlan wgrad_choose(const ConvGeom& g, int has_bias, bool has_src1, bool tuned, int wg_target) {
    const int Hs = g.Hs, Ws = g.Ws, Cin = g.Cin, Cout = g.Cout, Ho = g.Ho, Wo = g.Wo, stride = g.stride, pad = g.pad, pad_mode = g.pad_mode, C1 = g.C1, up = g.up;
    const int vec = (Cin % 4 == 0 && C1 % 4 == 0) ? 4 : 1;
    const int64_t P = (int64_t)g.B * Ho * Wo;
    auto plan = [&](WgradPath w) { return wgrad_plan(w, g, has_bias, tuned, wg_target); };
    const bool lean = vec == 4 && Cout % 4 == 0 && Wo >= 8 && (int64_t)g.B * Hs * Ws * Cin * 4 < (1ll << 31) && P * Cout * 4 < (1ll << 31) && P < (1ll << 24);
    WgradPlan p{WP_GEMM};
    if (stride == 2 && pad == 3 && pad_mode == 0 && C1 == Cin && up == 1 && !has_bias && Ho == (Hs + 6 - 7) / 2 + 1 && Wo == (Ws + 6 - 7) / 2 + 1 &&
        (p = plan(WP_STEM)).open)
        return p;
    if (lean && stride == 1 && pad == 1 && pad_mode == 1 && C1 % 16 == 0 && Ho == Hs && Wo == Ws && (C1 == Cin || has_src1) && Hs % up == 0 && Ws % up == 0 &&
        (p = plan(WP_THIN)).open)
        return p;
    if (vec == 4 && stride == 1 && pad == 1 && Ho == Hs && Wo == Ws && (up == 1 || up == 2) && Hs % up == 0 && Ws % up == 0 && (C1 == Cin || (has_src1 && C1 % 32 == 0)) &&
        getenv("E2E_WGRAD_TAPS") != nullptr && getenv("E2E_WGRAD_TAPS")[0] == '1' && (p = plan(WP_TAPS)).open)
        return p;
    return lean && (p = plan(WP_GEMM16)).open ? p : plan(lean ? WP_GEMM_LEAN : WP_GEMM);
}

int64_t e2e_conv2d_wgrad_workspace_floats(int B, int Ho, int Wo, int Cin, int Cout, int KH, int KW, int has_bias) {
    GEOM_WGRAD_QUERY(g);
    return wgrad_workspace_floats(g, has_bias, false, WGRAD_TARGET);
}

struct WgradOut { float* dw; float* dbias; const float* out_scale; int accumulate; e2e_wgrad_reduce_desc* defer; };

static void wgrad_reduce(const WgradArgs& a, const WgradOut& o, int S, int Mpad, int Npad, int zl, hipStream_t st) {
    if (o.defer) {
        *o.defer = e2e_wgrad_reduce_desc{a.slabs, o.dw, o.dbias, o.out_scale, S, Mpad, Npad, a.Cout, a.Cin, a.KH, a.KW, a.has_bias, o.accumulate, zl, 0};
        return;
    }
    const int64_t tq = (int64_t)a.Cout * ((a.Ngemm + 3) / 4);
    if (zl == 8)
        hipLaunchKernelGGL((k_wgrad_reduce<8>), dim3(egrid(tq * 4)), dim3(512), 0, st, a.slabs, S, Mpad, Npad, a.Cout, a.Cin, a.KH, a.KW, a.has_bias, o.dw,
                           o.dbias, o.accumulate, o.out_scale);
    else
        hipLaunchKernelGGL((k_wgrad_reduce<2>), dim3(egrid(tq * 4)), dim3(128), 0, st, a.slabs, S, Mpad, Npad, a.Cout, a.Cin, a.KH, a.KW, a.has_bias, o.dw,
                           o.dbias, o.accumulate, o.out_scale);
}

enum WgradKernel { WK_DONE, WK_GEMM16, WK_GEMM4_32, WK_GEMM4_64, WK_GEMM_32, WK_GEMM_64 };
struct WgradLaunch { WgradKernel k; dim3 g; int Sz; };

static int wgrad_setup(const WgradIn& in, const ConvGeom& g, int wg_target, const WgradOut& o, hipStream_t st, WgradArgs& a, WgradLaunch& L) {
    const int B = g.B, Cin = g.Cin, Cout = g.Cout, Ho = g.Ho, Wo = g.Wo;
    const bool tuned = wg_target != 0;
    if (!tuned) wg_target = WGRAD_TARGET;
    L = WgradLaunch{WK_DONE, dim3(1), 0};
    E2E_REQUIRE(in.dz && in.src0 && o.dw && in.workspace && B > 0 && Cin > 0 && Cout > 0, E2E_ERR_ARG, "e2e_conv2d_bwd_weight: bad argument");
    const int vec = (Cin % 4 == 0 && g.C1 % 4 == 0) ? 4 : 1;
    E2E_REQUIRE(vec == 4 || (g.C1 == Cin && g.up == 1 && g.pad_mode == 0), E2E_ERR_ARG, "e2e_conv2d_bwd_weight: scalar path takes one full-resolution zero-padded source");
    a = WgradArgs{};
    a.dz = in.dz; a.src0 = in.src0; a.src1 = in.src1; a.slabs = in.workspace;
    a.B = B; a.Hs = g.Hs; a.Ws = g.Ws; a.Cin = Cin; a.C1 = g.C1; a.up = g.up; a.Ho = Ho; a.Wo = Wo; a.Cout = Cout;
    a.KH = g.KH; a.KW = g.KW; a.stride = g.stride; a.pad = g.pad; a.pad_mode = g.pad_mode; a.has_bias = o.dbias ? 1 : 0;
    a.Ngemm = g.KH * g.KW * Cin + a.has_bias;
    const WgradPlan p = wgrad_choose(g, a.has_bias, in.src1 != nullptr, tuned, wg_target);
    const int S = (int)p.S;
    if (p.path == WP_STEM) {
        StemWgradArgs ta{in.dz, in.src0, in.workspace, B, g.Hs, g.Ws, Ho, Wo, 2, p.nxg, g.in_sub, g.in_mul};
        hipLaunchKernelGGL(k_wgrad7x7_stem, dim3(p.nxg, p.ny, B), dim3(256), 0, st, ta);
    } else if (p.path == WP_THIN) {
        ThinWgradArgs ta{in.dz, in.src0, in.src1, in.workspace, B, Ho, Wo, Cin, g.C1, g.up, p.Npad, a.has_bias, p.tiles_x, p.nxg};
        const dim3 tg((unsigned)p.nxg, (unsigned)p.ny, (unsigned)(B * (Cin / 16)));
        if (Cout == 32) hipLaunchKernelGGL((k_wgrad3x3_thin<2>), tg, dim3(256), 0, st, ta);
        else hipLaunchKernelGGL((k_wgrad3x3_thin<1>), tg, dim3(256), 0, st, ta);
    } else if (p.path == WP_TAPS) {
        TapWgradArgs ta{in.dz, in.src0, in.src1, in.workspace, B, Ho, Wo, Cin, g.C1, g.up, Cout, g.pad_mode == 1 ? 1 : 0, a.has_bias,
                        p.Mpad, p.Npad, p.ptx, p.pty, p.nchunks, p.cps};
        const dim3 tg((unsigned)(Cin / 32), (unsigned)(Cout / 32), (unsigned)S);
        if (a.has_bias) hipLaunchKernelGGL(k_wgrad3x3_taps<true>, tg, dim3(TAP_NT), 0, st, ta);
        else hipLaunchKernelGGL(k_wgrad3x3_taps<false>, tg, dim3(TAP_NT), 0, st, ta);
    }
    if (p.path == WP_STEM || p.path == WP_THIN || p.path == WP_TAPS) {
        wgrad_reduce(a, o, S, p.Mpad, p.Npad, (p.path == WP_TAPS && S < 8) ? 2 : 8, st);
        return E2E_OK;
    }
    const bool use16 = p.path == WP_GEMM16, lean = p.path != WP_GEMM;
    a.Mpad = p.Mpad; a.Npad = p.Npad;
    a.in_sub = g.in_sub; a.in_mul = g.in_mul; a.vec = vec;
    const int64_t P = (int64_t)B * Ho * Wo;
    const int cbp = lean ? 32 : CBK;
    a.pix_per_slice = ((P + p.S - 1) / p.S + cbp - 1) / cbp * cbp;
    L.Sz = (int)((P + a.pix_per_slice - 1) / a.pix_per_slice);
    L.g = dim3((unsigned)(a.Npad / p.tn), (unsigned)(a.Mpad / p.tm), (unsigned)L.Sz);
    L.k = use16 ? WK_GEMM16 : lean ? (p.tm == 32 ? WK_GEMM4_32 : WK_GEMM4_64) : (p.tm == 32 ? WK_GEMM_32 : WK_GEMM_64);
    return E2E_OK;
}

static void wgrad_launch_gemm(const WgradArgs& a, const WgradLaunch& L, hipStream_t st) {
    const dim3 g = L.g;
    const bool two = a.src1 != nullptr;
    if (L.k == WK_GEMM16) hipLaunchKernelGGL((k_wgrad_gemm16<10, 32>), g, dim3(256), 0, st, a);
    else if (L.k == WK_GEMM4_32 && two) hipLaunchKernelGGL((k_wgrad_gemm4<1, 4, 32, true>), g, dim3(256), 0, st, a);
    else if (L.k == WK_GEMM4_32) hipLaunchKernelGGL((k_wgrad_gemm4<1, 4, 32, false>), g, dim3(256), 0, st, a);
    else if (L.k == WK_GEMM4_64 && two) hipLaunchKernelGGL((k_wgrad_gemm4<2, 2, 32, true>), g, dim3(256), 0, st, a);
    else if (L.k == WK_GEMM4_64) hipLaunchKernelGGL((k_wgrad_gemm4<2, 2, 32, false>), g, dim3(256), 0, st, a);
    else if (L.k == WK_GEMM_32 && a.vec == 4) hipLaunchKernelGGL((k_wgrad_gemm<1, 4, 4>), g, dim3(256), 0, st, a);
    else if (L.k == WK_GEMM_32) hipLaunchKernelGGL((k_wgrad_gemm<1, 4, 1>), g, dim3(256), 0, st, a);
    else if (L.k == WK_GEMM_64 && a.vec == 4) hipLaunchKernelGGL((k_wgrad_gemm<2, 2, 4>), g, dim3(256), 0, st, a);
    else if (L.k == WK_GEMM_64) hipLaunchKernelGGL((k_wgrad_gemm<2, 2, 1>), g, dim3(256), 0, st, a);
}

static int bwd_weight_impl(const WgradIn& in, const ConvGeom& g, const WgradOut& o, void* stream, int wg_target = 0) {
    const hipStream_t st = (hipStream_t)stream;
    WgradArgs a;
    WgradLaunch L;
    const int rc = wgrad_setup(in, g, wg_target, o, st, a, L);
    if (rc != E2E_OK) return rc;
    if (L.k != WK_DONE) {
        wgrad_launch_gemm(a, L, st);
        wgrad_reduce(a, o, L.Sz, a.Mpad, a.Npad, L.Sz >= 8 ? 8 : 2, st);
    }
    E2E_LAUNCH_CHECK("e2e_conv2d_bwd_weight");
    return E2E_OK;
}

int e2e_conv2d_bwd_weight(const float* dz, const float* src0, const float* src1, int C1, int up, float* dw, float* dbias,
                          float* workspace, int B, int Hs, int Ws, int Cin, int Cout, int Ho, int Wo, int KH, int KW, int stride,
                          int pad, int pad_mode, int accumulate, float in_sub, float in_mul, void* stream) {
    GEOM_BWD_WEIGHT(g);
    return bwd_weight_impl(WgradIn{dz, src0, src1, workspace}, g, WgradOut{dw, dbias, nullptr, accumulate, nullptr}, stream);
}

int e2e_conv2d_bwd_weight_scaled(const float* da, const float* out_scale, const float* src0, const float* src1, int C1, int up, float* dw,
                                 float* dbias, float* workspace, int B, int Hs, int Ws, int Cin, int Cout, int Ho, int Wo, int KH, int KW,
                                 int stride, int pad, int pad_mode, int accumulate, float in_sub, float in_mul, void* stream) {
    GEOM_BWD_WEIGHT(g);
    return bwd_weight_impl(WgradIn{da, src0, src1, workspace}, g, WgradOut{dw, dbias, out_scale, accumulate, nullptr}, stream);
}

int e2e_conv2d_bwd_weight_scaled_deferred(const float* da, const float* out_scale, const float* src0, const float* src1, int C1, int up, float* dw,
                                          float* dbias, float* workspace, int B, int Hs, int Ws, int Cin, int Cout, int Ho, int Wo, int KH, int KW,
                                          int stride, int pad, int pad_mode, int accumulate, float in_sub, float in_mul,
                                          e2e_wgrad_reduce_desc* desc_out, void* stream) {
    E2E_REQUIRE(desc_out, E2E_ERR_ARG, "e2e_conv2d_bwd_weight_scaled_deferred: desc_out is NULL");
    GEOM_BWD_WEIGHT(g);
    return bwd_weight_impl(WgradIn{da, src0, src1, workspace}, g, WgradOut{dw, dbias, out_scale, accumulate, desc_out}, stream);
}

int e2e_conv2d_bwd_pair_deferred(const float* da, const float* w_bwd, int ld_bwd, float* dxp, int B, int Hs, int Ws, int Cin, int Cout, int Ho, int Wo,
                                 int KH, int KW, int stride, int pad, int pad_mode, int accumulate, const float* x_in, int in_act, const float* pre_add,
                                 float* workspace, const float* out_scale, const float* src0, const float* src1, int C1, int up, float* dw, float* dbias,
                                 float* workspace_w, int accumulate_w, float in_sub, float in_mul, e2e_wgrad_reduce_desc* desc_out, int wgrad_first,
                                 void* stream) {
    E2E_REQUIRE(desc_out, E2E_ERR_ARG, "e2e_conv2d_bwd_pair_deferred: desc_out is NULL");
    const hipStream_t st = (hipStream_t)stream;
    ConvArgs ad;
    bool data_done;
    GEOM_BWD_WEIGHT(g);
    int rc = bwd_data_setup(BwdDataOps{da, w_bwd, ld_bwd, dxp, accumulate, x_in, in_act, pre_add}, g, GemmCfg{0, 0, 0}, st, ad, data_done);
    if (rc != E2E_OK) return rc;
    const WgradOut o{dw, dbias, out_scale, accumulate_w, desc_out};
    WgradArgs aw;
    WgradLaunch lw;
    rc = wgrad_setup(WgradIn{da, src0, src1, workspace_w}, g, 0, o, st, aw, lw);
    if (rc != E2E_OK) return rc;
    GemmLaunch pd{};
    if (!data_done) pd = plan_gemm<true>(ad, 4, workspace, GemmCfg{0, 0, 0});
    const bool d14 = pd.c.bm == 32 && pd.c.bn == 128, d22 = pd.c.bm == 64 && pd.c.bn == 64;
    const bool paired = !data_done && pd.kind == GK_TILE && pd.cb == 32 && (d14 || d22) && lw.k == WK_GEMM4_64;
    if (paired) {
        PairGrid pg;
        pg.dgx = pd.g.x; pg.dgy = pd.g.y; pg.dgz = pd.g.z;
        pg.wgx = lw.g.x; pg.wgy = lw.g.y; pg.wgz = lw.g.z;
        const unsigned nd = pg.dgx * pg.dgy * pg.dgz, nw = pg.wgx * pg.wgy * pg.wgz;
        pg.wgrad_first = wgrad_first ? 1 : 0;
        pg.first = ((wgrad_first ? nw : nd) + 7u) / 8u * 8u;
        const dim3 grid(pg.first + (wgrad_first ? nd : nw));
        const bool two = aw.src1 != nullptr;
        if (d14) {
            if (two) hipLaunchKernelGGL((k_conv_bwd_pair<1, 4, true>), grid, dim3(256), 0, st, ad, aw, pg);
            else hipLaunchKernelGGL((k_conv_bwd_pair<1, 4, false>), grid, dim3(256), 0, st, ad, aw, pg);
        } else {
            if (two) hipLaunchKernelGGL((k_conv_bwd_pair<2, 2, true>), grid, dim3(256), 0, st, ad, aw, pg);
            else hipLaunchKernelGGL((k_conv_bwd_pair<2, 2, false>), grid, dim3(256), 0, st, ad, aw, pg);
        }
    } else {
        if (!data_done) launch_gemm_main<true>(ad, pd, workspace, st);
        if (lw.k != WK_DONE) wgrad_launch_gemm(aw, lw, st);
    }
    if (!data_done) launch_gemm_tail(ad, pd, st);
    if (lw.k != WK_DONE) wgrad_reduce(aw, o, lw.Sz, aw.Mpad, aw.Npad, lw.Sz >= 8 ? 8 : 2, st);
    E2E_LAUNCH_CHECK("e2e_conv2d_bwd_pair_deferred");
    return E2E_OK;
}

long long e2e_wgrad_reduce_batch_prepare(e2e_wgrad_reduce_desc* descs_host, int n) {
    if (!descs_host || n <= 0) return -1;
    long long total = 0;
    for (int i = 0; i < n; ++i) {
        e2e_wgrad_reduce_desc& d = descs_host[i];
        if (!d.slabs || !d.dw || d.S <= 0 || d.Mpad <= 0 || d.Npad <= 0 || d.Npad % 4 || d.Cout <= 0 || d.Cin <= 0 || d.KH <= 0 || d.KW <= 0 || (d.zl != 8 && d.zl != 2))
            return -1;
        const long long quads = (long long)d.Cout * ((d.KH * d.KW * d.Cin + (d.has_bias ? 1 : 0) + 3) / 4);
        d.first_item = total;
        total += (quads + (d.zl == 8 ? 63 : 255)) / (d.zl == 8 ? 64 : 256);
    }
    return total;
}

int e2e_wgrad_reduce_batched(const e2e_wgrad_reduce_desc* descs_dev, int n, long long total_items, void* stream) {
    E2E_REQUIRE(descs_dev && n > 0 && total_items > 0, E2E_ERR_ARG, "e2e_wgrad_reduce_batched: bad argument");
    hipLaunchKernelGGL(k_wgrad_reduce_batched, dim3((unsigned)(total_items < 4096 ? total_items : 4096)), dim3(512), 0, (hipStream_t)stream, descs_dev, n, total_items);
    E2E_LAUNCH_CHECK("e2e_wgrad_reduce_batched");
    return E2E_OK;
}

int e2e_conv2d_bwd_weight_scaled_tuned(const float* da, const float* out_scale, const float* src0, const float* src1, int C1, int up, float* dw,
                                       float* dbias, float* workspace, int B, int Hs, int Ws, int Cin, int Cout, int Ho, int Wo, int KH, int KW,
                                       int stride, int pad, int pad_mode, int accumulate, float in_sub, float in_mul, int target_workgroups, void* stream) {
    E2E_REQUIRE(target_workgroups >= 64 && target_workgroups <= 8192, E2E_ERR_ARG, "e2e_conv2d_bwd_weight_scaled_tuned: 64 .. 8192 workgroups");
    GEOM_BWD_WEIGHT(g);
    return bwd_weight_impl(WgradIn{da, src0, src1, workspace}, g, WgradOut{dw, dbias, out_scale, accumulate, nullptr}, stream, target_workgroups);
}

int64_t e2e_conv2d_wgrad_tuned_workspace_floats(int B, int Ho, int Wo, int Cin, int Cout, int KH, int KW, int has_bias, int target_workgroups) {
    GEOM_WGRAD_QUERY(g);
    return wgrad_workspace_floats(g, has_bias, true, target_workgroups);
}

}
```

### end-to-end-self-supervised-slam_amd/e2ehip/netplan.py

```python
import ctypes
import os

import torch

from . import _lib as L
from .conv import ACT, _ld, epoch_sum

_f32 = torch.float32
PAIR_WGRAD_FIRST = 0


class Buf:
    __slots__ = ("t", "g", "written", "B", "h", "w", "C", "act")

    def __init__(self, B, h, w, C, dev, need_grad=True, act=0):
        self.B, self.h, self.w, self.C = B, h, w, C
        self.act = act
        self.t = torch.empty(B, h, w, C, device=dev, dtype=_f32)
        self.g = torch.empty(B, h, w, C, device=dev, dtype=_f32) if need_grad else None
        self.written = False

    def nchw(self):
        return self.t.permute(0, 3, 1, 2)


def _at(t, slot):
    return L.ptr(t if slot is None else t[slot])


def _sink_of(p):
    s = getattr(p, "_e2e_grad_sink", None)
    if s is None:
        if p.grad is None:
            p.grad = torch.zeros_like(p)
        s = p.grad
    return s


class _Conv:
    def __init__(self, plan, src0, src1, weight, bias, bn, residual, act, stride, pad, pad_mode, up, in_norm):
        dev = plan.dev
        self.src0, self.src1, self.res = src0, src1, residual
        self.weight, self.bias = weight, bias
        self.Cout, self.Cin, self.KH, self.KW = weight.shape
        self.C1 = src0.C
        if self.C1 + (src1.C if src1 is not None else 0) != self.Cin:
            raise ValueError("channel mismatch in the launch plan")
        self.up, self.stride, self.pad, self.pm, self.act = up, stride, pad, 1 if pad_mode == "reflect" else 0, ACT[act]
        self.isub, self.imul = in_norm if in_norm is not None else (0.0, 1.0)
        B = src0.B
        self.Hs, self.Ws = src0.h * up, src0.w * up
        self.Ho, self.Wo = (self.Hs + 2 * pad - self.KH) // stride + 1, (self.Ws + 2 * pad - self.KW) // stride + 1
        if self.act not in (0, ACT["relu"], ACT["elu"]):
            raise NotImplementedError("launch plan: convolution epilogues are none / ReLU / ELU (the sigmoid head has its own op)")
        self.out = Buf(B, self.Ho, self.Wo, self.Cout, dev, act=self.act)
        self.ldf, self.ldb = _ld(self.Cout), _ld(self.Cin)
        self.wf = torch.zeros(self.KH * self.KW * self.Cin, self.ldf, device=dev, dtype=_f32)
        self.need_dx = src0.g is not None
        self.wb = torch.zeros(self.KH * self.KW * self.Cout, self.ldb, device=dev, dtype=_f32) if self.need_dx else None
        self.scale = self.shift = None
        if bn is not None:
            w, b, rm, rv, eps = bn
            with torch.no_grad():
                self.scale = (w / torch.sqrt(rv + eps)).contiguous()
                self.shift = (b - rm * self.scale).contiguous()
        self.geom = dict(B=B, Hs=self.Hs, Ws=self.Ws, Cin=self.Cin, Cout=self.Cout, Ho=self.Ho, Wo=self.Wo, KH=self.KH, KW=self.KW, stride=stride,
                         pad=pad, pad_mode=self.pm, C1=self.C1, up=up, in_sub=float(self.isub), in_mul=float(self.imul))
        n = max(L.query("e2e_conv2d_splitk_workspace_floats", b * self.Ho * self.Wo, self.Cout, self.KH * self.KW * self.Cin) for b in {B, 1})
        self.ws_f = torch.zeros(n, device=dev, dtype=_f32) if n else None
        self.pp = pad if self.pm == 1 else 0
        self.direct = self.pp == 0 and up == 1 and src1 is None
        if self.need_dx:
            n = L.query("e2e_conv2d_bwd_data_workspace_floats", geom=self.geom, Hd=self.Hs + 2 * self.pp, Wd=self.Ws + 2 * self.pp, cols=self.Cin,
                        K=self.KH * self.KW * self.Cout)
            self.ws_b = torch.zeros(n, device=dev, dtype=_f32) if n else None
            self.dxp = None if self.direct else torch.empty(B, self.Hs + 2 * self.pp, self.Ws + 2 * self.pp, self.Cin, device=dev, dtype=_f32)
        self.ws_w = torch.empty(L.query("e2e_conv2d_wgrad_workspace_floats", geom=self.geom, has_bias=1 if bias is not None else 0), device=dev, dtype=_f32)
        self.res_via, self.res_aliased, self.pre_from = None, False, None
        self.reduce_desc = L.WgradReduceDesc()

    def layout_row(self):
        return [self.weight.data_ptr(), self.wf.data_ptr(), self.wb.data_ptr() if self.wb is not None else 0, self.Cout, self.Cin, self.KH, self.KW,
                self.ldf, self.ldb, self.scale.data_ptr() if (self.scale is not None and self.wb is not None) else 0]

    def fwd(self, plan, st, slot=None):
        s = self
        L.call("e2e_conv2d_fwd", geom=s.geom, B=s.src0.B if slot is None else 1, src0=_at(s.src0.t, slot),
               src1=_at(s.src1.t, slot) if s.src1 is not None else None, w_fwd=L.ptr(s.wf), ld_fwd=s.ldf, scale=L.ptr(s.scale),
               shift=L.ptr(s.shift if s.bias is None else s.bias), residual=_at(s.res.t, slot) if s.res is not None else None,
               out=_at(s.out.t, slot), act=s.act, workspace=L.ptr(s.ws_f), stream=st)

    def bwd(self, plan, st):
        s = self
        n = s.out.t.numel()
        g = s.out.g
        if s.res is not None and s.res_via is None and not s.res_aliased:
            L.call("e2e_conv2d_act_bwd_acc", L.ptr(g), L.ptr(s.res.t), None, L.ptr(s.res.g), n, s.Cout, s.res.act, 1 if s.res.written else 0, st)
            s.res.written = True
        if s.need_dx and plan.paired and not plan.overlap:
            pre = s.pre_from.out.g if (s.direct and s.pre_from is not None) else None
            L.call("e2e_conv2d_bwd_pair_deferred", geom=s.geom, da=L.ptr(g), w_bwd=L.ptr(s.wb), ld_bwd=s.ldb, dxp=L.ptr(s.src0.g if s.direct else s.dxp),
                   accumulate=(1 if s.src0.written else 0) if s.direct else 0, x_in=L.ptr(s.src0.t) if s.direct else None,
                   in_act=s.src0.act if s.direct else 0, pre_add=L.ptr(pre), workspace=L.ptr(s.ws_b), workspace_w=L.ptr(s.ws_w), accumulate_w=0,
                   wgrad_first=PAIR_WGRAD_FIRST, stream=st, **s._wgrad_operands(plan))
            if s.direct:
                s.src0.written = True
            else:
                self._gather_adjoint(st)
            return
        if s.need_dx:
            if s.direct:
                pre = s.pre_from.out.g if s.pre_from is not None else None
                L.call("e2e_conv2d_bwd_data_fused", geom=s.geom, da=L.ptr(g), w_bwd=L.ptr(s.wb), ld_bwd=s.ldb, dxp=L.ptr(s.src0.g),
                       accumulate=1 if s.src0.written else 0, x_in=L.ptr(s.src0.t), in_act=s.src0.act, pre_add=L.ptr(pre), workspace=L.ptr(s.ws_b), stream=st)
                s.src0.written = True
            else:
                L.call("e2e_conv2d_bwd_data", geom=s.geom, dz=L.ptr(g), w_bwd=L.ptr(s.wb), ld_bwd=s.ldb, dxp=L.ptr(s.dxp), workspace=L.ptr(s.ws_b), stream=st)
                self._gather_adjoint(st)
        st_w = plan.fork(st)
        L.call("e2e_conv2d_bwd_weight_scaled_deferred", geom=s.geom, da=L.ptr(g), workspace=L.ptr(s.ws_w), accumulate=0, stream=st_w, **s._wgrad_operands(plan))

    def _wgrad_operands(self, plan):
        s = self
        return dict(out_scale=L.ptr(s.scale), src0=L.ptr(s.src0.t), src1=L.ptr(s.src1.t) if s.src1 is not None else None, dw=L.ptr(plan.sink(s.weight)),
                    dbias=L.ptr(plan.sink(s.bias)) if s.bias is not None else None, desc_out_host=ctypes.byref(s.reduce_desc))

    def _gather_adjoint(self, st):
        s, s1 = self, self.src1
        L.call("e2e_conv2d_gather_adjoint_act", geom=s.geom, dxp=L.ptr(s.dxp), padded=1 if s.pp else 0, d_src0=L.ptr(s.src0.g),
               d_src1=L.ptr(s1.g) if s1 is not None else None, accumulate0=1 if s.src0.written else 0,
               accumulate1=1 if (s1 is not None and s1.written) else 0, src0=L.ptr(s.src0.t), act0=s.src0.act,
               src1=L.ptr(s1.t) if s1 is not None else None, act1=s1.act if s1 is not None else 0, stream=st)
        s.src0.written = True
        if s1 is not None:
            s1.written = True


class _Head:

    def __init__(self, plan, src, weight, bias, act):
        self.src, self.weight, self.bias, self.act = src, weight, bias, ACT[act]
        self.out = Buf(src.B, src.h, src.w, 1, plan.dev)
        self.dz = torch.empty_like(self.out.t)
        self.ws = torch.empty(L.load().e2e_head_workspace_floats(), device=plan.dev, dtype=_f32)

    def fwd(self, plan, st, slot=None):
        s = self.src
        L.call("e2e_head_fwd", _at(s.t, slot), L.ptr(self.weight), L.ptr(self.bias), _at(self.out.t, slot), s.B if slot is None else 1, s.h, s.w, s.C, self.act, st)

    def bwd(self, plan, st):
        s, n = self.src, self.out.t.numel()
        L.call("e2e_conv2d_act_bwd", L.ptr(self.out.g), L.ptr(self.out.t), None, L.ptr(self.dz), n, 1, self.act, st)
        if s.written:
            raise RuntimeError("the disparity head's input has a single consumer")
        L.call("e2e_head_bwd_act", dz=L.ptr(self.dz), x=L.ptr(s.t), w=L.ptr(self.weight), dx=L.ptr(s.g), dw=L.ptr(plan.sink(self.weight)),
               dbias=L.ptr(plan.sink(self.bias)) if self.bias is not None else None, workspace=L.ptr(self.ws), B=s.B, H=s.h, W=s.w, Cin=s.C,
               in_act=s.act, stream=st)
        s.written = True


class _MaxPool:
    def __init__(self, plan, src):
        self.src = src
        self.out = Buf(src.B, (src.h - 1) // 2 + 1, (src.w - 1) // 2 + 1, src.C, plan.dev)
        self.argmax = torch.empty(self.out.t.shape, device=plan.dev, dtype=torch.uint8)

    def fwd(self, plan, st, slot=None):
        s = self.src
        L.call("e2e_maxpool3x3s2_fwd_idx", _at(s.t, slot), _at(self.out.t, slot), _at(self.argmax, slot), s.B if slot is None else 1, s.h, s.w, s.C, st)

    def bwd(self, plan, st):
        s = self.src
        if s.act not in (0, ACT["relu"]):
            raise NotImplementedError("launch plan: the max-pool follows a ReLU (ResNet stem)")
        L.call("e2e_maxpool3x3s2_bwd_idx", x=L.ptr(s.t), argmax=L.ptr(self.argmax), dy=L.ptr(self.out.g), dx=L.ptr(s.g), B=s.B, H=s.h, W=s.w, C=s.C,
               accumulate=1 if s.written else 0, mul_relu=1 if s.act else 0, stream=st)
        s.written = True


class _BNAffine:

    def __init__(self, plan, src, bn_mod):
        self.src, self.bn = src, bn_mod
        C = src.C
        self.out = Buf(src.B, src.h, src.w, C, plan.dev)
        self.scale, self.shift, self.rstd = (torch.empty(C, device=plan.dev, dtype=_f32) for _ in range(3))
        self.ws = torch.empty(L.load().e2e_affine_bwd_workspace_floats(C), device=plan.dev, dtype=_f32)

    def fwd(self, plan, st, slot=None):
        b, s = self.bn, self.src
        L.call("e2e_bn_fold", L.ptr(b.weight), L.ptr(b.bias), L.ptr(b.running_mean), L.ptr(b.running_var), float(b.eps), L.ptr(self.scale),
               L.ptr(self.shift), L.ptr(self.rstd), s.C, st)
        L.call("e2e_affine_fwd", _at(s.t, slot), L.ptr(self.scale), L.ptr(self.shift), None, 0, _at(self.out.t, slot),
               s.t.numel() if slot is None else s.t[0].numel(), s.C, st)

    def bwd(self, plan, st):
        b, s = self.bn, self.src
        n = s.t.numel()
        L.call("e2e_affine_bwd", dy=L.ptr(self.out.g), z=L.ptr(s.t), mean=L.ptr(b.running_mean), rstd=L.ptr(self.rstd), P=n // s.C, C=s.C,
               dgamma=L.ptr(plan.sink(b.weight)), dbeta=L.ptr(plan.sink(b.bias)), accumulate=0, workspace=L.ptr(self.ws), stream=st)
        if s.act != 0:
            raise NotImplementedError("launch plan: a trainable BatchNorm follows a plain convolution")
        L.call("e2e_conv2d_act_bwd_acc", L.ptr(self.out.g), L.ptr(self.out.g), L.ptr(self.scale), L.ptr(s.g), n, s.C, 0, 1 if s.written else 0, st)
        s.written = True


class NetPlan:
    def __init__(self, model, B, H, W, device, overlap=True):
        from depth_estimation.networks import BasicBlock
        self.model, self.dev, self.overlap = model, torch.device(device), overlap
        self.paired = os.environ.get("E2E_PAIRED_BWD", "1") != "0"
        self.B, self.H, self.W = B, H, W
        if H % 32 or W % 32:
            raise ValueError(f"launch plan: the encoder halves the image five times and the decoder doubles it back before every skip "
                             f"concatenation (networks.py:277-292): height and width must be multiples of 32, got {H} x {W}")
        self.ops, self._sinks, self._side = [], {}, None
        enc, dec = model.encoder.encoder, model.decoder
        if any(m.training for m in model.modules() if isinstance(m, torch.nn.BatchNorm2d)):
            raise NotImplementedError("the launch plan runs BatchNorm in eval mode (refinement mode, online_adaption.py:175-184)")
        self.x = Buf(B, H, W, 3, self.dev, need_grad=False)

        def bn_args(bn):
            return (bn.weight, bn.bias, bn.running_mean, bn.running_var, bn.eps)

        def conv_bn(src, conv, bn, relu, residual=None, in_norm=None):
            if bn.weight.requires_grad or bn.bias.requires_grad:
                if relu or residual is not None or in_norm is not None:
                    raise NotImplementedError("launch plan: a trainable BatchNorm is expected on the downsample branches only (set_refinement_mode)")
                z = self._add(_Conv(self, src, None, conv.weight, None, None, None, None, conv.stride[0], conv.padding[0], "zeros", 1, None))
                return self._add(_BNAffine(self, z, bn))
            return self._add(_Conv(self, src, None, conv.weight, None, bn_args(bn), residual, "relu" if relu else None, conv.stride[0],
                                   conv.padding[0], "zeros", 1, in_norm))

        f = conv_bn(self.x, enc.conv1, enc.bn1, True, in_norm=(0.45, 1.0 / 0.225))
        feats = [f]
        x = self._add(_MaxPool(self, f))
        for stage in (enc.layer1, enc.layer2, enc.layer3, enc.layer4):
            if stage is enc.layer4:
                self.split_index = len(self.ops)
            for blk in stage:
                if not isinstance(blk, BasicBlock):
                    raise NotImplementedError("launch plan: BasicBlock encoders (ResNet-18 / 34)")
                idt = x if blk.downsample is None else conv_bn(x, blk.downsample[0], blk.downsample[1], False)
                idt_op = self.ops[-1]
                h = conv_bn(x, blk.conv1, blk.bn1, True)
                c1 = self.ops[-1]
                x = conv_bn(h, blk.conv2, blk.bn2, True, residual=idt)
                c2 = self.ops[-1]
                if blk.downsample is None:
                    if c1.direct and c1.need_dx:
                        c2.res_via, c1.pre_from = c1, c2
                elif isinstance(idt_op, _BNAffine) and idt.act == 0:
                    idt.g = c2.out.g
                    c2.res_aliased = True
            feats.append(x)
        self.features = feats
        x = feats[-1]
        for i in range(4, -1, -1):
            c0, c1 = dec.convs[("upconv", i, 0)].conv, dec.convs[("upconv", i, 1)].conv
            x = self._add(_Conv(self, x, None, c0.conv.weight, c0.conv.bias, None, None, "elu", 1, 1, c0.pad_mode, 1, None))
            skip = feats[i - 1] if (dec.use_skips and i > 0) else None
            x = self._add(_Conv(self, x, skip, c1.conv.weight, c1.conv.bias, None, None, "elu", 1, 1, c1.pad_mode, 2, None))
        hc = dec.convs[("dispconv", 0)]
        if tuple(hc.conv.weight.shape) != (1, 16, 3, 3) or hc.pad_mode != "reflect":
            raise NotImplementedError("launch plan: the indoor decoder's 16 -> 1 reflect head")
        self.head = _Head(self, x, hc.conv.weight, hc.conv.bias, "disp")
        self.ops.append(self.head)
        self.disp = self.head.out
        self._desc = None
        self._desc_key = None
        self._retired_tables = []
        self._move_tables = {}
        self._reduce_tables = {}

    def _add(self, op):
        self.ops.append(op)
        return op.out

    def parameters(self):
        out = []
        for op in self.ops:
            if isinstance(op, _Conv) or isinstance(op, _Head):
                out.append(op.weight)
                if op.bias is not None:
                    out.append(op.bias)
            elif isinstance(op, _BNAffine):
                out += [op.bn.weight, op.bn.bias]
        return out

    def sink(self, p):
        s = self._sinks.get(id(p))
        if s is None or s.data_ptr() != _sink_of(p).data_ptr():
            s = self._sinks[id(p)] = _sink_of(p)
            if not s.is_contiguous() or tuple(s.shape) != tuple(p.shape):
                raise RuntimeError("gradient sink of a parameter must be a contiguous tensor of the parameter's shape")
        return s

    def refresh_layouts(self, st=None):
        convs = [op for op in self.ops if isinstance(op, _Conv)]
        key = tuple(op.weight.data_ptr() for op in convs)
        if self._desc is None or self._desc_key != key:
            self._desc = torch.tensor([op.layout_row() for op in convs], dtype=torch.int64).to(self.dev)
            self._desc_key = key
        L.call("e2e_conv_weight_layouts_batched", L.ptr(self._desc), len(convs), st if st is not None else L.stream())
        self.mark_layouts_current()

    def _stamp(self):
        ws = [op.weight for op in self.ops if isinstance(op, _Conv)]
        return (tuple(w.data_ptr() for w in ws), tuple(w._version for w in ws), epoch_sum(ws))

    def mark_layouts_current(self):
        self._epoch = self._stamp()

    def layouts_current(self):
        return self._desc is not None and getattr(self, "_epoch", None) == self._stamp()

    def fork(self, st):
        if not self.overlap:
            return st
        if self._side is None:
            self._side = torch.cuda.Stream(self.dev)
            self._record_side_stream_use()
        self._side.wait_stream(torch.cuda.current_stream(self.dev))
        self._forked = True
        return ctypes.c_void_p(self._side.cuda_stream)

    def join(self):
        if self.overlap and self._side is not None and getattr(self, "_forked", False):
            torch.cuda.current_stream(self.dev).wait_stream(self._side)
            self._forked = False

    def _record_side_stream_use(self):
        seen = set()
        for op in self.ops:
            ts = [op.out.t, op.out.g]
            if isinstance(op, _Conv):
                ts += [op.scale, op.ws_w, op.src0.t, op.src1.t if op.src1 is not None else None]
                for p in (op.weight, op.bias):
                    if p is not None:
                        ts.append(_sink_of(p))
            for t in ts:
                if t is not None and t.is_cuda and t.untyped_storage().data_ptr() not in seen:
                    seen.add(t.untyped_storage().data_ptr())
                    t.record_stream(self._side)

    def close(self):
        if self._side is not None:
            self._side.synchronize()
        torch.cuda.current_stream(self.dev).synchronize()
        self.ops, self._sinks, self._desc, self._reduce_tables = [], {}, None, {}

    def forward(self, frames=None):
        if frames is not None:
            self.x.t.copy_(frames)
        st = L.stream()
        for op in self.ops:
            op.fwd(self, st)
        return self.disp.t.view(self.B, 1, self.H, self.W)

    def forward_one(self, slot):
        if not 0 <= slot < self.B:
            raise ValueError("slot out of range")
        st = L.stream()
        for op in self.ops:
            op.fwd(self, st, slot)

    def move_slot(self, src, dst):
        held = self._move_tables.get((src, dst))
        if held is None:
            if not 0 <= src < self.B or not 0 <= dst < self.B or src == dst:
                raise ValueError("slots out of range")
            if torch.cuda.is_current_stream_capturing():
                raise RuntimeError("launch plan: move_slot builds its copy table on first use; run it eagerly once before capturing it")
            pairs = []
            for op in self.ops:
                pairs.append((op.out.t[src], op.out.t[dst]))
                if isinstance(op, _MaxPool):
                    pairs.append((op.argmax[src], op.argmax[dst]))
            if any(a.numel() * a.element_size() % 16 or a.data_ptr() % 16 or b.data_ptr() % 16 for a, b in pairs):
                for a, b in pairs:
                    b.copy_(a)
                return
            arr = (L.CopyDesc * len(pairs))(*[L.CopyDesc(a.data_ptr(), b.data_ptr(), a.numel() * a.element_size(), 0) for a, b in pairs])
            total = L.load().e2e_copy_batch_prepare(arr, len(pairs))
            if total <= 0:
                raise RuntimeError("launch plan: malformed copy descriptor")
            held = self._move_tables[(src, dst)] = (torch.frombuffer(bytearray(bytes(arr)), dtype=torch.uint8).to(self.dev), len(pairs), total)
        L.call("e2e_copy_batched", L.ptr(held[0]), held[1], held[2], L.stream())

    def backward(self, g_disp=None):
        if g_disp is not None:
            self.disp.g.copy_(g_disp.reshape(self.disp.g.shape))
        self.backward_late_layers()
        self.backward_early_layers()

    def backward_late_layers(self):
        st = L.stream()
        for op in self.ops:
            op.out.written = False
        for op in reversed(self.ops[self.split_index:]):
            op.bwd(self, st)
        self.join()
        self._reduce_weight_gradients("late", self.ops[self.split_index:])
        self._written_after_late = [op.out.written for op in self.ops]

    def backward_early_layers(self):
        st = L.stream()
        state = getattr(self, "_written_after_late", None)
        if state is None:
            raise RuntimeError("launch plan: backward_early_layers() follows backward_late_layers()")
        for op, w in zip(self.ops, state):
            op.out.written = w
        for op in reversed(self.ops[:self.split_index]):
            op.bwd(self, st)
        self.join()
        self._reduce_weight_gradients("early", self.ops[:self.split_index])

    def _reduce_weight_gradients(self, which, ops):
        convs = [op for op in ops if isinstance(op, _Conv)]
        if not convs:
            return
        arr = (L.WgradReduceDesc * len(convs))(*[op.reduce_desc for op in convs])
        total = L.load().e2e_wgrad_reduce_batch_prepare(arr, len(convs))
        if total <= 0:
            raise RuntimeError("launch plan: malformed backward-weight reduction descriptor")
        raw = bytes(arr)
        held = self._reduce_tables.get(which)
        if held is None or held[0] != raw:
            if torch.cuda.is_current_stream_capturing():
                raise RuntimeError("launch plan: the backward-weight reduction table changed under stream capture; run the plan eagerly once first")
            table = torch.frombuffer(bytearray(raw), dtype=torch.uint8).to(self.dev)
            if held is not None:
                self._retired_tables.append(held[1])
            held = self._reduce_tables[which] = (raw, table, total)
        L.call("e2e_wgrad_reduce_batched", L.ptr(held[1]), len(convs), held[2], L.stream())

    def split_offset(self, flat):
        off_of = {id(p): o for p, o in zip(flat.params, flat.offsets)}

        def params_of(ops):
            out = []
            for op in ops:
                for name in ("weight", "bias"):
                    p = getattr(op, name, None)
                    if isinstance(p, torch.nn.Parameter) and p.requires_grad and id(p) in off_of:
                        out.append(off_of[id(p)])
                bn = getattr(op, "bn", None)
                if bn is not None:
                    out += [off_of[id(p)] for p in (bn.weight, bn.bias) if p.requires_grad and id(p) in off_of]
            return out
        late, early = params_of(self.ops[self.split_index:]), params_of(self.ops[:self.split_index])
        if not late or not early or min(late) <= max(early):
            raise RuntimeError("launch plan: the late layers' parameters are not the tail of the flat bucket")
        return min(late)
```

### include/e2eslam.h

```cpp
#ifndef E2ESLAM_H
#define E2ESLAM_H

#include <stdint.h>

#ifdef __cplusplus
extern "C" {
#endif

#define E2E_OK 0
#define E2E_ERR_ARG (-1)
#define E2E_ERR_LAUNCH (-2)
#define E2E_ERR_WORKSPACE (-3)

#define E2E_PADDING_ZEROS 0
#define E2E_PADDING_BORDER 1

typedef struct e2e_strides {
    int64_t sb, sc, sh, sw;
} e2e_strides;

int e2e_version(void);
const char* e2e_last_error(void);


int e2e_backproject_fwd(const float* depth, const float* inv_K, float* cam_points,
                        int B, int H, int W, void* stream);
int e2e_backproject_bwd(const float* g_cam, const float* inv_K, float* g_depth,
                        int B, int H, int W, void* stream);

int e2e_project3d_fwd(const float* points, const float* K, const float* T, float* grid, float* valid,
                      float* z_out, int B, int H, int W, void* stream);
int e2e_project3d_bwd(const float* points, const float* K, const float* T, const float* g_grid,
                      const float* g_z, float* g_points, int B, int H, int W, void* stream);

int e2e_grid_sample_fwd(const float* input, e2e_strides in_strides, const float* grid, float* out,
                        int B, int C, int Hi, int Wi, int Ho, int Wo, int padding_mode,
                        int align_corners, void* stream);
int e2e_grid_sample_bwd(const float* input, e2e_strides in_strides, const float* grid,
                        const float* g_out, float* g_grid, float* g_input, int B, int C, int Hi,
                        int Wi, int Ho, int Wo, int padding_mode, int align_corners, void* stream);
int e2e_grid_sample_bwd_exact(const float* input, e2e_strides in_strides, const float* grid, const float* g_out,
                              float* g_grid, long long* g_input_fixed, float* g_input, int B, int C, int Hi, int Wi,
                              int Ho, int Wo, int padding_mode, int align_corners, void* stream);


int e2e_photometric_fwd(const float* x, e2e_strides xs, const float* y, e2e_strides ys,
                        float* ssim_out, float* pmap_out, int B, int C, int H, int W, void* stream);
int e2e_photometric_bwd(const float* x, e2e_strides xs, const float* y, e2e_strides ys,
                        const float* g_pmap, const float* g_ssim, float* g_x, int B, int C, int H,
                        int W, void* stream);


int64_t e2e_warp_photo_workspace_floats(int B, int H, int W);

int e2e_warp_photo_fwd(const float* depth_tgt, const float* src, e2e_strides src_strides,
                       const float* tgt, e2e_strides tgt_strides, const float* K, const float* inv_K,
                       const float* T, float* synth, float* valid, float* pmap, int use_mask,
                       int padding_mode, int reg_kind, const float* reg_init_tgt,
                       const float* reg_init_src, const float* depth_src, float* loss_out,
                       float* workspace, int B, int H, int W, void* stream);

int e2e_warp_photo_bwd(const float* depth_tgt, const float* src, e2e_strides src_strides,
                       const float* tgt, e2e_strides tgt_strides, const float* K, const float* inv_K,
                       const float* T, const float* synth, const float* valid, int use_mask,
                       int padding_mode, int reg_kind, const float* reg_init_tgt,
                       const float* reg_init_src, const float* depth_src, const float* g_loss,
                       float* g_depth_tgt, float* g_depth_src, int B, int H, int W, void* stream);

int64_t e2e_warp_photo_lossgrad_workspace_floats(int B, int H, int W);
int e2e_warp_photo_lossgrad(const float* depth_tgt, const float* src, e2e_strides src_strides,
                            const float* tgt, e2e_strides tgt_strides, const float* K,
                            const float* inv_K, const float* T, int use_mask, int padding_mode,
                            int reg_kind, const float* reg_init_tgt, const float* reg_init_src,
                            const float* depth_src, float w_photo, float w_reg, float* loss_out,
                            float* g_depth_tgt, float* g_depth_src, float* workspace, int B, int H,
                            int W, void* stream);

int e2e_warp_photo_lossgrad_hostgeo(const float* depth_tgt, const float* src, e2e_strides src_strides,
                                    const float* tgt, e2e_strides tgt_strides,
                                    const float* geometry12_host, int use_mask, int padding_mode,
                                    int reg_kind, const float* reg_init_tgt, const float* reg_init_src,
                                    const float* depth_src, float w_photo, float w_reg, float* loss_out,
                                    float* g_depth_tgt, float* g_depth_src, float* workspace, int H,
                                    int W, void* stream);

int e2e_warp_photo_lossgrad_chain(const float* depth_tgt, const float* src, e2e_strides src_strides,
                                  const float* tgt, e2e_strides tgt_strides, const float* K,
                                  const float* inv_K, const float* T, const float* geometry12_host,
                                  int use_mask, int padding_mode, int reg_kind, const float* reg_init_tgt,
                                  const float* reg_init_src, const float* depth_src, float w_photo,
                                  float w_reg, int set_cur, int set_prev, float* loss_prev_out,
                                  float* g_depth_tgt, float* g_depth_src, float* workspace, int B, int H,
                                  int W, void* stream);
int e2e_warp_photo_lossgrad_chain_flush(float* workspace, int set, int reg_kind, float* loss_out, int B,
                                        int H, int W, void* stream);

#define E2E_TERM_GEOMETRIC 1
#define E2E_TERM_AUTO_MASKING 2
#define E2E_TERM_MIN_REPROJECTION 4
int64_t e2e_warp_photo_terms_lossgrad_workspace_floats(int B, int H, int W);
int e2e_warp_photo_terms_lossgrad(const float* depth_tgt, const float* depth_src, const float* src,
                                  e2e_strides src_strides, const float* tgt, e2e_strides tgt_strides,
                                  const float* K, const float* inv_K, const float* T, int use_mask,
                                  int padding_mode, int reg_kind, const float* reg_init_tgt,
                                  const float* reg_init_src, int terms, const float* tie_noise, float w_photo,
                                  float w_reg, float w_geometric, float* loss_out, float* g_depth_tgt,
                                  float* g_depth_src, float* workspace, int B, int H, int W, void* stream);

int64_t e2e_smoothness_norm_lossgrad_workspace_floats(int H, int W);
int e2e_smoothness_norm_lossgrad(const float* disp, const float* img, e2e_strides img_strides, float weight,
                                 float* loss_out, float* g_disp, float* workspace, int H, int W,
                                 void* stream);


int e2e_vertex_normal_maps(const float* depth, const float* K, const float* pose, float alpha_den,
                           float* V, float* Nm, float* Vg, float* Ng, float* alpha, int B, int H,
                           int W, void* stream);
int e2e_vertex_maps_bwd(const float* depth, const float* K, const float* pose, const float* g_V,
                        const float* g_Vg, float* g_depth, int B, int H, int W, void* stream);

int e2e_transform_points(const float* points, const float* T, float* out, int64_t n,
                         int transpose_rotation_only, void* stream);

int64_t e2e_pf_workspace_bytes(int64_t map_capacity, int H, int W);
int e2e_pf_associate(const float* map_points, const float* map_normals, const float* map_ccounts,
                     int64_t M, const float* K, const float* pose, const float* Vg, const float* Ng,
                     float dist_th, float dot_th, void* workspace, int64_t map_capacity, int H, int W,
                     void* stream);
int e2e_pf_table(int which, int64_t M, void* workspace, int64_t map_capacity, int H, int W,
                 long long* rows, long long* count_out, void* stream);
int e2e_pf_fuse_append(float* map_points, float* map_normals, float* map_colors, float* map_ccounts,
                       int64_t M, int64_t map_capacity, const float* depth, const float* Vg,
                       const float* Ng, const float* rgb, const float* alpha, void* workspace, int H,
                       int W, long long* new_count_out, void* stream);

int e2e_pf_associate_dev(const float* map_points, const float* map_normals, const float* map_ccounts,
                         const long long* map_count_dev, const float* K, const float* pose, const float* Vg,
                         const float* Ng, float dist_th, float dot_th, void* workspace, int64_t map_capacity,
                         int H, int W, void* stream);
int e2e_pf_active_subsample_dev(const float* map_points, const float* map_normals, const long long* map_count_dev,
                                int64_t map_capacity, void* workspace, int H, int W, int dsratio, float* tgt,
                                float* tgt_normals, long long* tgt_count_dev, int64_t tgt_capacity, void* stream);
int e2e_pf_fuse_append_dev(float* map_points, float* map_normals, float* map_colors, float* map_ccounts,
                           long long* map_count_dev, int64_t map_capacity, const float* depth, const float* Vg,
                           const float* Ng, const float* rgb, const float* alpha, void* workspace, int H, int W,
                           void* stream);
int e2e_frame_append_dev(float* map_points, float* map_normals, float* map_colors, float* map_ccounts,
                         long long* map_count_dev, int64_t map_capacity, const float* depth, const float* rgb,
                         const float* K, const float* pose, float alpha_den, void* workspace, int H, int W, void* stream);


int64_t e2e_knn1_workspace_bytes(int64_t n1, int64_t n2);
int e2e_knn1_fwd(const float* p1, int64_t n1, const float* p2, int64_t n2, float* dists,
                 long long* idx, void* workspace, int algorithm, void* stream);
int e2e_knn1_bwd(const float* g_dists, const float* p1, const float* p2, const long long* idx,
                 int64_t n1, float* g_p1, void* stream);
int e2e_knn1_bwd_ref(const float* g_dists, const float* p1, const float* p2, const long long* idx,
                     int64_t n1, int64_t n2, long long* scratch_fixed, float* g_p2, void* stream);

int e2e_knn1_index_build(const float* p2, int64_t n2, int64_t max_queries, void* index, void* stream);
int e2e_knn1_index_query(const float* p1, int64_t n1, int64_t n2, int64_t max_queries, void* index,
                         float* dists, long long* idx, void* stream);
int64_t e2e_knn1_index_capacity_bytes(int64_t max_queries, int64_t n2_capacity);
int e2e_knn1_index_build_dev(const float* p2, const long long* n2_dev, int64_t n2_capacity, int64_t max_queries,
                             void* index, void* stream);
int e2e_knn1_index_query_dev(const float* p1, int64_t n1, int64_t n2_capacity, int64_t max_queries, void* index,
                             float* dists, long long* idx, void* stream);
int64_t e2e_knn1_index_capacity_bytes_res(int64_t max_queries, int64_t n2_capacity, int cells_per_axis);
int e2e_knn1_index_build_dev_res(const float* p2, const long long* n2_dev, int64_t n2_capacity, int64_t max_queries,
                                 void* index, int cells_per_axis, void* stream);
int e2e_knn1_index_query_dev_res(const float* p1, int64_t n1, const float* ref_points, const long long* warm_idx,
                                 int64_t n2_capacity, int64_t max_queries, void* index, int cells_per_axis,
                                 float* dists, long long* idx, void* stream);
int e2e_knn1_index_query_dev_image(const float* p1, int64_t n1, int row_len, int64_t n2_capacity, int64_t max_queries, void* index,
                                   float* dists, long long* idx, void* stream);
int e2e_knn1_index_query_dev_image_warm(const float* p1, int64_t n1, int row_len, const float* ref_points, const long long* warm_idx,
                                        int64_t n2_capacity, int64_t max_queries, void* index, float* dists, long long* idx, void* stream);


int64_t e2e_median_workspace_bytes(void);
int e2e_median_lower(const float* x, int64_t n, float* value_out, void* workspace, void* stream);

int64_t e2e_depth_scale_workspace_bytes(void);
int e2e_depth_scale_fwd(const float* disp, const float* median_gt, float* delta, float* depth,
                        float* median_delta, float* ratio_out, void* workspace, int64_t n,
                        void* stream);
int e2e_depth_scale_bwd(const float* g_depth, const float* delta, const float* median_gt,
                        const float* median_delta, float* g_disp, void* workspace, int64_t n,
                        void* stream);
int e2e_depth_scale_bwd_at(const float* g_depth, const float* delta, const float* median_gt,
                           const float* median_delta, const int* elements, int n_elements,
                           float* g_disp, void* workspace, int64_t n, void* stream);

int e2e_depth_fixed_scale_fwd(const float* disp, float scale, float* delta, float* depth, int64_t n,
                              void* stream);
int e2e_depth_fixed_scale_bwd(const float* g_depth, const float* disp, float scale, float* g_disp,
                              int64_t n, void* stream);

int64_t e2e_reduce_workspace_floats(void);
int e2e_mean_diff_fwd(const float* a, const float* b, int64_t n, int kind, float* out,
                      float* workspace, void* stream);
int e2e_mean_diff_bwd(const float* a, const float* b, const float* g_out, int64_t n, int kind,
                      float* g_b, void* stream);

int e2e_depth_metrics(const float* gt, const float* pred, int64_t n, int mask_zero_gt, float* out7,
                      float* workspace, void* stream);

int e2e_adam_step(float* params, const float* grads, float* exp_avg, float* exp_avg_sq, int64_t n,
                  float lr, float beta1, float beta2, float eps, int step, void* stream);
int e2e_adam_step_mean(float* params, const float* grad_sums, const float* participants, float* exp_avg,
                       float* exp_avg_sq, int64_t n, float lr, float beta1, float beta2, float eps,
                       int step, void* stream);
int e2e_adam_step_resident(float* params, const float* grad_sums, const float* participants, float* exp_avg,
                           float* exp_avg_sq, int64_t n, float beta1, float beta2, float eps,
                           const float* schedule, int schedule_len, int* step_counter, void* stream);

#define E2E_ACT_NONE 0
#define E2E_ACT_RELU 1
#define E2E_ACT_ELU 2
#define E2E_ACT_DISP 3

int e2e_conv_weight_layouts(const float* w, int Cout, int Cin, int KH, int KW, float* w_fwd,
                            int ld_fwd, float* w_bwd, int ld_bwd, void* stream);

int e2e_conv_weight_layouts_batched(const long long* desc, int nlayers, void* stream);

int e2e_conv2d_fwd(const float* src0, const float* src1, int C1, int up, const float* w_fwd,
                   int ld_fwd, const float* scale, const float* shift, const float* residual,
                   float* out, int B, int Hs, int Ws, int Cin, int Cout, int KH, int KW, int stride,
                   int pad, int pad_mode, int act, float in_sub, float in_mul, float* workspace,
                   void* stream);
int64_t e2e_conv2d_splitk_workspace_floats(int64_t rows, int cols, int K);
int64_t e2e_conv2d_bwd_data_workspace_floats(int B, int Hd, int Wd, int cols, int K, int stride);
int e2e_conv_workspace_flag_floats(void);
int e2e_conv_streamk_error_index(void);
int64_t e2e_conv_tuned_workspace_floats(int64_t rows, int cols);
int e2e_conv2d_fwd_tuned(const float* src0, const float* src1, int C1, int up, const float* w_fwd, int ld_fwd, const float* scale,
                         const float* shift, const float* residual, float* out, int B, int Hs, int Ws, int Cin, int Cout, int KH,
                         int KW, int stride, int pad, int pad_mode, int act, float in_sub, float in_mul, float* workspace, int tile_m,
                         int tile_n, int ksplit, void* stream);
int e2e_conv2d_bwd_data_fused_tuned(const float* da, const float* w_bwd, int ld_bwd, float* dxp, int B, int Hs, int Ws, int Cin, int Cout,
                                    int Ho, int Wo, int KH, int KW, int stride, int pad, int pad_mode, int accumulate, const float* x_in,
                                    int in_act, const float* pre_add, float* workspace, int tile_m, int tile_n, int ksplit, void* stream);
int64_t e2e_conv2d_wgrad_tuned_workspace_floats(int B, int Ho, int Wo, int Cin, int Cout, int KH, int KW, int has_bias, int target_workgroups);
int e2e_conv2d_bwd_weight_scaled_tuned(const float* da, const float* out_scale, const float* src0, const float* src1, int C1, int up,
                                       float* dw, float* dbias, float* workspace, int B, int Hs, int Ws, int Cin, int Cout, int Ho, int Wo,
                                       int KH, int KW, int stride, int pad, int pad_mode, int accumulate, float in_sub, float in_mul,
                                       int target_workgroups, void* stream);
int e2e_conv_gemm_choice(int64_t rows, int cols, int K, int chunk_depth, int allow_split, int* out3_host);

int e2e_conv2d_act_bwd(const float* dy, const float* y, const float* scale, float* dz, int64_t n,
                       int C, int act, void* stream);
int e2e_conv2d_act_bwd_acc(const float* dy, const float* y, const float* scale, float* dz, int64_t n,
                           int C, int act, int accumulate, void* stream);

int e2e_conv2d_bwd_data(const float* dz, const float* w_bwd, int ld_bwd, float* dxp, int B, int Hs,
                        int Ws, int Cin, int Cout, int Ho, int Wo, int KH, int KW, int stride,
                        int pad, int pad_mode, float* workspace, void* stream);
int e2e_conv2d_bwd_data_acc(const float* dz, const float* w_bwd, int ld_bwd, float* dxp, int B, int Hs,
                            int Ws, int Cin, int Cout, int Ho, int Wo, int KH, int KW, int stride,
                            int pad, int pad_mode, int accumulate, float* workspace, void* stream);
int e2e_conv2d_bwd_data_fused(const float* da, const float* w_bwd, int ld_bwd, float* dxp, int B, int Hs,
                              int Ws, int Cin, int Cout, int Ho, int Wo, int KH, int KW, int stride,
                              int pad, int pad_mode, int accumulate, const float* x_in, int in_act,
                              const float* pre_add, float* workspace, void* stream);
int e2e_conv2d_gather_adjoint(const float* dxp, int B, int Hs, int Ws, int Cin, int C1, int up,
                              int padded, float* d_src0, float* d_src1, int accumulate0,
                              int accumulate1, void* stream);

int e2e_conv2d_gather_adjoint_act(const float* dxp, int B, int Hs, int Ws, int Cin, int C1, int up,
                                  int padded, float* d_src0, float* d_src1, int accumulate0,
                                  int accumulate1, const float* src0, int act0, const float* src1,
                                  int act1, void* stream);

int64_t e2e_conv2d_wgrad_workspace_floats(int B, int Ho, int Wo, int Cin, int Cout, int KH, int KW,
                                          int has_bias);
int e2e_conv2d_bwd_weight(const float* dz, const float* src0, const float* src1, int C1, int up,
                          float* dw, float* dbias, float* workspace, int B, int Hs, int Ws, int Cin,
                          int Cout, int Ho, int Wo, int KH, int KW, int stride, int pad,
                          int pad_mode, int accumulate, float in_sub, float in_mul, void* stream);

int e2e_conv2d_bwd_weight_scaled(const float* da, const float* out_scale, const float* src0,
                                 const float* src1, int C1, int up, float* dw, float* dbias,
                                 float* workspace, int B, int Hs, int Ws, int Cin, int Cout, int Ho,
                                 int Wo, int KH, int KW, int stride, int pad, int pad_mode,
                                 int accumulate, float in_sub, float in_mul, void* stream);

typedef struct e2e_wgrad_reduce_desc {
    const float* slabs;
    float* dw;
    float* dbias;
    const float* scale;
    int S, Mpad, Npad, Cout, Cin, KH, KW, has_bias, accumulate;
    int zl;
    long long first_item;
} e2e_wgrad_reduce_desc;
int e2e_conv2d_bwd_weight_scaled_deferred(const float* da, const float* out_scale, const float* src0,
                                          const float* src1, int C1, int up, float* dw, float* dbias,
                                          float* workspace, int B, int Hs, int Ws, int Cin, int Cout, int Ho,
                                          int Wo, int KH, int KW, int stride, int pad, int pad_mode,
                                          int accumulate, float in_sub, float in_mul,
                                          e2e_wgrad_reduce_desc* desc_out_host, void* stream);
int e2e_conv2d_bwd_pair_deferred(const float* da, const float* w_bwd, int ld_bwd, float* dxp, int B, int Hs,
                                 int Ws, int Cin, int Cout, int Ho, int Wo, int KH, int KW, int stride,
                                 int pad, int pad_mode, int accumulate, const float* x_in, int in_act,
                                 const float* pre_add, float* workspace, const float* out_scale,
                                 const float* src0, const float* src1, int C1, int up, float* dw,
                                 float* dbias, float* workspace_w, int accumulate_w, float in_sub,
                                 float in_mul, e2e_wgrad_reduce_desc* desc_out_host, int wgrad_first,
                                 void* stream);
long long e2e_wgrad_reduce_batch_prepare(e2e_wgrad_reduce_desc* descs_host, int n);
int e2e_wgrad_reduce_batched(const e2e_wgrad_reduce_desc* descs_dev, int n, long long total_items, void* stream);

typedef struct e2e_copy_desc {
    const void* src;
    void* dst;
    long long bytes;
    long long first_item;
} e2e_copy_desc;
long long e2e_copy_batch_prepare(e2e_copy_desc* descs_host, int n);
int e2e_copy_batched(const e2e_copy_desc* descs_dev, int n, long long total_items, void* stream);

int e2e_maxpool3x3s2_fwd(const float* x, float* y, int B, int H, int W, int C, void* stream);
int e2e_maxpool3x3s2_bwd(const float* x, const float* dy, float* dx, int B, int H, int W, int C,
                         int accumulate, int mul_relu, void* stream);
int e2e_maxpool3x3s2_fwd_idx(const float* x, float* y, unsigned char* argmax, int B, int H, int W, int C, void* stream);
int e2e_maxpool3x3s2_bwd_idx(const float* x, const unsigned char* argmax, const float* dy, float* dx, int B, int H, int W, int C,
                             int accumulate, int mul_relu, void* stream);

int e2e_bn_fold(const float* gamma, const float* beta, const float* running_mean,
                const float* running_var, float eps, float* scale, float* shift, float* rstd, int C,
                void* stream);
int e2e_affine_fwd(const float* z, const float* scale, const float* shift, const float* residual, int relu,
                   float* y, int64_t n, int C, void* stream);
int64_t e2e_affine_bwd_workspace_floats(int C);
int e2e_affine_bwd(const float* dy, const float* z, const float* mean, const float* rstd, int64_t P,
                   int C, float* dgamma, float* dbeta, int accumulate, float* workspace, void* stream);

int e2e_upsample2_concat(const float* x, const float* skip, float* y, int B, int h, int w, int C1,
                         int C2, void* stream);

int e2e_head_fwd(const float* x, const float* w, const float* bias, float* y, int B, int H, int W,
                 int Cin, int act, void* stream);
int64_t e2e_head_workspace_floats(void);
int e2e_head_bwd(const float* dz, const float* x, const float* w, float* dx, float* dw, float* dbias,
                 float* workspace, int B, int H, int W, int Cin, void* stream);

int e2e_head_bwd_act(const float* dz, const float* x, const float* w, float* dx, float* dw, float* dbias,
                     float* workspace, int B, int H, int W, int Cin, int in_act, void* stream);


int64_t e2e_icp_workspace_bytes(void);
int e2e_icp_normal_equations(const float* src, const float* tgt, const float* tgt_normals,
                             const long long* idx, const float* dists, float dist_thresh, int64_t n,
                             double* out29, void* workspace, void* stream);

int64_t e2e_icp_state_doubles(void);
int e2e_icp_state_init(double* state, float* T32, float* step32, const float* prev_pose, float* pose_out,
                       double damp, void* stream);
int e2e_icp_update(const double* out29, double* state, float* T32, float* step32, const float* prev_pose,
                   float* pose_out, int mode, int phase, double lambda_max, double B, double B2, double nu,
                   void* stream);
int e2e_icp_reduce_update(const float* src, const float* tgt, const float* tgt_normals, const long long* idx,
                          const float* dists, float dist_thresh, int64_t n, void* workspace, double* state, float* T32,
                          float* step32, const float* prev_pose, float* pose_out, int mode, int phase,
                          double lambda_max, double B, double B2, double nu, void* stream);
int e2e_icp_source_subsample(const float* Vg, const float* depth, int H, int W, int dsratio, float* src,
                             int* status, void* stream);

int64_t e2e_aux_workspace_floats(void);

int e2e_smoothness_lossgrad(const float* disp, const float* img, e2e_strides img_strides, int B, int C,
                            int H, int W, float* loss_out, float* g_disp, float* workspace,
                            void* stream);

int e2e_geometric_consistency_lossgrad(const float* warped_depth, const float* interpolated_depth,
                                       const float* mask, int64_t n, float* stats_out3,
                                       float* g_warped, float* g_interpolated, float* workspace,
                                       void* stream);

int e2e_masked_l1_lossgrad(const float* prediction, const float* sparse_gt, const float* sparse_mask,
                           int64_t n, float* loss_out, float* g_prediction, float* workspace,
                           void* stream);

int e2e_min_reprojection_lossgrad(const float* errors, int B, int C, int H, int W, float* loss_out,
                                  float* g_errors, float* workspace, void* stream);

int e2e_mask_mul(const float* x, e2e_strides x_strides, const float* mask, int B, int C, int H, int W,
                 float* out, void* stream);
int e2e_channel_mean(const float* x, int B, int C, int H, int W, int adjoint, float* out, void* stream);
int e2e_mean_normalize(const float* d, const float* g, int B, int H, int W, float* out, float* workspace,
                       void* stream);

int e2e_masked_mean_lossgrad(const float* values, const float* gate, int64_t n, float weight, float* out3,
                             float* g_values, float* workspace, void* stream);

int e2e_disp_blend_fwd(const float* disp_pair, int H, int W, float* out, void* stream);
int e2e_disp_blend_bwd(const float* g_out, int H, int W, float* g_disp_pair, void* stream);

#ifdef __cplusplus
}
#endif
#endif
```

Before: 215.9.

## Carry earlier layers' batched weight-gradient reductions inside later paired backward launches

Adds a third role to the paired data/weight-gradient backward kernel that runs slices of the batched weight-gradient reduction for convolutions whose slabs are already complete. A host-side plan hands each one-launch pair the range of reduction items finished so far, and only the leftover items run in the final batched reduce. The aim is to fill idle CU time during the backward GEMMs and shrink the serial reduction at the end of each half. In exchange the paired grid gets larger, the reduce role runs with 256 threads instead of 512, and the reduction table must stay stable across calls, which is checked at runtime.

Measured after the change: 219.5, median of 6. +1.7%, better.

```diff
diff --git a/end-to-end-self-supervised-slam_amd/csrc/conv.hip b/end-to-end-self-supervised-slam_amd/csrc/conv.hip
--- a/end-to-end-self-supervised-slam_amd/csrc/conv.hip
+++ b/end-to-end-self-supervised-slam_amd/csrc/conv.hip
@@ -1386,16 +1386,30 @@
     unsigned wgx, wgy, wgz;
     unsigned first;
     int wgrad_first;
+    unsigned cbeg, cpad;
 };
+struct CarryArgs { const e2e_wgrad_reduce_desc* d; int n; unsigned wgs; long long first, items; };
+template <int NW>
+__device__ __forceinline__ void wgrad_reduce_item(const e2e_wgrad_reduce_desc* __restrict__ d, int n, long long item, f4v (*part)[64]);
 
 template <int DWM, int DWN, bool TWO>
-__global__ __launch_bounds__(256) void k_conv_bwd_pair(ConvArgs d, WgradArgs w, PairGrid pg) {
+__global__ __launch_bounds__(256) void k_conv_bwd_pair(ConvArgs d, WgradArgs w, PairGrid pg, CarryArgs c) {
     using DL = ConvGemmLds<DWM, DWN, 1, 1, 4, 32>;
     using WL = WgradGemm4Lds<2, 2, 32>;
-    static_assert(64 * DWM * DWN == 256, "both parts run 256 threads");
-    __shared__ union { DL d; WL w; } lds;
-    const bool in_first = blockIdx.x < pg.first;
-    const unsigned l = in_first ? blockIdx.x : blockIdx.x - pg.first;
+    static_assert(64 * DWM * DWN == 256, "all parts run 256 threads");
+    __shared__ union { DL d; WL w; float part[8 * 64 * 4]; } lds;
+    unsigned b = blockIdx.x;
+    if (b >= pg.cbeg) {
+        const unsigned ci = b - pg.cbeg;
+        if (ci < pg.cpad) {
+            if (ci < c.wgs)
+                for (long long item = c.first + ci; item < c.first + c.items; item += c.wgs) wgrad_reduce_item<4>(c.d, c.n, item, reinterpret_cast<f4v(*)[64]>(lds.part));
+            return;
+        }
+        b -= pg.cpad;
+    }
+    const bool in_first = b < pg.first;
+    const unsigned l = in_first ? b : b - pg.first;
     if (in_first == (pg.wgrad_first != 0)) {
         if (l >= pg.wgx * pg.wgy * pg.wgz) return;
         wgrad_gemm4_body<2, 2, 32, TWO>(w, PartIds{l, pg.wgx, pg.wgy, pg.wgz}, lds.w.As, lds.w.Bs);
@@ -1846,7 +1860,7 @@
     }
 }
 
-template <int ZL>
+template <int ZL, int NW>
 __device__ __forceinline__ void wgrad_reduce_group(const float* __restrict__ slabs, int S, int Mpad, int Npad, int Cout, int Cin, int KH, int KW, int has_bias,
                                                    float* __restrict__ dw, float* __restrict__ dbias, int accumulate, const float* __restrict__ scale,
                                                    int64_t base, int e, int w, f4v (*part)[64]) {
@@ -1859,17 +1873,22 @@
     const bool on = q < totalq;
     const int m = on ? (int)(q / nq) : 0, n = on ? (int)(q - (int64_t)m * nq) * 4 : 0;
     const f4v* src = (const f4v*)(slabs + (int64_t)m * Npad + n);
-    f4v sacc = zero;
-    int z = w;
-    for (; z + 3 * ZL < S; z += 4 * ZL) {
-        f4v v[4];
-#pragma unroll
-        for (int j = 0; j < 4; ++j) v[j] = on ? src[(int64_t)(z + ZL * j) * slab_q] : zero;
-#pragma unroll
-        for (int j = 0; j < 4; ++j) sacc += v[j];
-    }
-    for (; z < S; z += ZL) sacc += on ? src[(int64_t)z * slab_q] : zero;
-    part[w][e] = sacc;
+    static_assert(ZL % NW == 0, "every wave runs the same number of roles");
+#pragma unroll
+    for (int r = 0; r < ZL / NW; ++r) {
+        const int role = w + r * NW;
+        f4v sacc = zero;
+        int z = role;
+        for (; z + 3 * ZL < S; z += 4 * ZL) {
+            f4v v[4];
+#pragma unroll
+            for (int j = 0; j < 4; ++j) v[j] = on ? src[(int64_t)(z + ZL * j) * slab_q] : zero;
+#pragma unroll
+            for (int j = 0; j < 4; ++j) sacc += v[j];
+        }
+        for (; z < S; z += ZL) sacc += on ? src[(int64_t)z * slab_q] : zero;
+        part[role][e] = sacc;
+    }
     __syncthreads();
     if (w == 0 && on) {
         f4v t = part[0][e];
@@ -1899,26 +1918,34 @@
     __shared__ f4v part[ZL][64];
     const int64_t totalq = (int64_t)Cout * ((KH * KW * Cin + (has_bias ? 1 : 0) + 3) / 4);
     for (int64_t base = (int64_t)blockIdx.x * 64; base < totalq; base += (int64_t)gridDim.x * 64)
-        wgrad_reduce_group<ZL>(slabs, S, Mpad, Npad, Cout, Cin, KH, KW, has_bias, dw, dbias, accumulate, scale, base, threadIdx.x & 63, threadIdx.x >> 6, part);
-}
-
-__global__ __launch_bounds__(512) void k_wgrad_reduce_batched(const e2e_wgrad_reduce_desc* __restrict__ d, int n, long long total_items) {
+        wgrad_reduce_group<ZL, ZL>(slabs, S, Mpad, Npad, Cout, Cin, KH, KW, has_bias, dw, dbias, accumulate, scale, base, threadIdx.x & 63, threadIdx.x >> 6, part);
+}
+
+template <int NW>
+__device__ __forceinline__ void wgrad_reduce_item(const e2e_wgrad_reduce_desc* __restrict__ d, int n, long long item, f4v (*part)[64]) {
+    static_assert(NW == 8 || NW == 4, "512 or 256 threads");
+    const int e = threadIdx.x & 63, w = threadIdx.x >> 6;
+    int lo = 0, hi = n - 1;
+    while (lo < hi) {
+        const int mid = (lo + hi + 1) >> 1;
+        if (d[mid].first_item <= item) lo = mid; else hi = mid - 1;
+    }
+    const e2e_wgrad_reduce_desc D = d[lo];
+    const long long local = item - D.first_item;
+    if (D.zl == 8) {
+        wgrad_reduce_group<8, NW>(D.slabs, D.S, D.Mpad, D.Npad, D.Cout, D.Cin, D.KH, D.KW, D.has_bias, D.dw, D.dbias, D.accumulate, D.scale, local * 64, e, w, part);
+    } else {
+        constexpr int G = NW / 2;
+#pragma unroll
+        for (int r = 0; r < 4 / G; ++r)
+            wgrad_reduce_group<2, 2>(D.slabs, D.S, D.Mpad, D.Npad, D.Cout, D.Cin, D.KH, D.KW, D.has_bias, D.dw, D.dbias, D.accumulate, D.scale,
+                                     (local * 4 + r * G + (w >> 1)) * 64, e, w & 1, part + 2 * (w >> 1));
+    }
+}
+
+__global__ __launch_bounds__(512) void k_wgrad_reduce_batched(const e2e_wgrad_reduce_desc* __restrict__ d, int n, long long first_item, long long items) {
     __shared__ f4v part[8][64];
-    const int e = threadIdx.x & 63, w = threadIdx.x >> 6;
-    for (long long item = blockIdx.x; item < total_items; item += gridDim.x) {
-        int lo = 0, hi = n - 1;
-        while (lo < hi) {
-            const int mid = (lo + hi + 1) >> 1;
-            if (d[mid].first_item <= item) lo = mid; else hi = mid - 1;
-        }
-        const e2e_wgrad_reduce_desc D = d[lo];
-        const long long local = item - D.first_item;
-        if (D.zl == 8)
-            wgrad_reduce_group<8>(D.slabs, D.S, D.Mpad, D.Npad, D.Cout, D.Cin, D.KH, D.KW, D.has_bias, D.dw, D.dbias, D.accumulate, D.scale, local * 64, e, w, part);
-        else
-            wgrad_reduce_group<2>(D.slabs, D.S, D.Mpad, D.Npad, D.Cout, D.Cin, D.KH, D.KW, D.has_bias, D.dw, D.dbias, D.accumulate, D.scale,
-                                  (local * 4 + (w >> 1)) * 64, e, w & 1, part + 2 * (w >> 1));
-    }
+    for (long long item = first_item + blockIdx.x; item < first_item + items; item += gridDim.x) wgrad_reduce_item<8>(d, n, item, part);
 }
 
 __global__ __launch_bounds__(256) void k_weight_layouts(const float* __restrict__ w, int Cout, int Cin, int KH, int KW,
@@ -2594,7 +2621,7 @@
     return conv_fwd_impl(FwdOps{src0, src1, w_fwd, ld_fwd, scale, shift, residual, out, act}, g, workspace, GemmCfg{tile_m, tile_n, ksplit}, stream);
 }
 
-static int bwd_data_setup(const BwdDataOps& d, const ConvGeom& g, GemmCfg force, hipStream_t stream, ConvArgs& a, bool& done) {
+static int bwd_data_setup(const BwdDataOps& d, const ConvGeom& g, GemmCfg force, hipStream_t stream, ConvArgs& a, bool& done, bool dry = false) {
     const int B = g.B, Hs = g.Hs, Ws = g.Ws, Cin = g.Cin, Cout = g.Cout, Ho = g.Ho, Wo = g.Wo, KH = g.KH, KW = g.KW, stride = g.stride, pad = g.pad;
     const int pad_mode = g.pad_mode, ld_bwd = d.ld_bwd;
     done = false;
@@ -2607,7 +2634,7 @@
                 "e2e_conv2d_bwd_data: gradients must stay below 1 GB, weights below 2 GB (32-bit buffer offsets), kernels up to 3 x 3");
     if (!force.bm && KH == 3 && KW == 3 && stride == 1 && pad == 1 && pad_mode == 1 && Cin == 16 && Cout == 16 && !d.accumulate && !d.in_act && !d.pre_add && ld_bwd >= 16) {
         ThinArgs t{d.dz, d.w_bwd, nullptr, d.dxp, B, Ho, Wo, Hs + 2, Ws + 2, ld_bwd, ACT_NONE, 2, 1};
-        hipLaunchKernelGGL((k_conv3x3_thin<16, 1, false, 8>), dim3((Ws + 2 + 63) / 64, (Hs + 2 + 7) / 8, B), dim3(256), 0, stream, t);
+        if (!dry) hipLaunchKernelGGL((k_conv3x3_thin<16, 1, false, 8>), dim3((Ws + 2 + 63) / 64, (Hs + 2 + 7) / 8, B), dim3(256), 0, stream, t);
         done = true;
         return E2E_OK;
     }
@@ -2618,7 +2645,7 @@
     a.Hd = Hs + 2 * pp; a.Wd = Ws + 2 * pp; a.off = pad_mode == 1 ? 0 : pad;
     a.Ncols = Cin; a.ldw = ld_bwd; a.KH = KH; a.KW = KW; a.stride = stride; a.pad = pad; a.pad_mode = 0; a.act = ACT_NONE;
     a.cls = (stride == 2 && cls_rows(B, a.Hd, a.Wd) < (1 << 24)) ? 1 : 0;
-    if (a.cls && (KH < 2 || KW < 2) && !d.accumulate)
+    if (a.cls && (KH < 2 || KW < 2) && !d.accumulate && !dry)
         (void)hipMemsetAsync(d.dxp, 0, (size_t)B * a.Hd * a.Wd * Cin * sizeof(float), stream);
     if (d.accumulate) a.res = d.dxp;
     a.xin = d.in_act ? d.x_in : nullptr; a.dact = d.in_act; a.pre = d.pre_add;
@@ -2837,7 +2864,7 @@
 enum WgradKernel { WK_DONE, WK_GEMM16, WK_GEMM4_32, WK_GEMM4_64, WK_GEMM_32, WK_GEMM_64 };
 struct WgradLaunch { WgradKernel k; dim3 g; int Sz; };
 
-static int wgrad_setup(const WgradIn& in, const ConvGeom& g, int wg_target, const WgradOut& o, hipStream_t st, WgradArgs& a, WgradLaunch& L) {
+static int wgrad_setup(const WgradIn& in, const ConvGeom& g, int wg_target, const WgradOut& o, hipStream_t st, WgradArgs& a, WgradLaunch& L, bool dry = false) {
     const int B = g.B, Cin = g.Cin, Cout = g.Cout, Ho = g.Ho, Wo = g.Wo;
     const bool tuned = wg_target != 0;
     if (!tuned) wg_target = WGRAD_TARGET;
@@ -2852,6 +2879,7 @@
     a.Ngemm = g.KH * g.KW * Cin + a.has_bias;
     const WgradPlan p = wgrad_choose(g, a.has_bias, in.src1 != nullptr, tuned, wg_target);
     const int S = (int)p.S;
+    if (dry && (p.path == WP_STEM || p.path == WP_THIN || p.path == WP_TAPS)) return E2E_OK;
     if (p.path == WP_STEM) {
         StemWgradArgs ta{in.dz, in.src0, in.workspace, B, g.Hs, g.Ws, Ho, Wo, 2, p.nxg, g.in_sub, g.in_mul};
         hipLaunchKernelGGL(k_wgrad7x7_stem, dim3(p.nxg, p.ny, B), dim3(256), 0, st, ta);
@@ -2934,51 +2962,114 @@
     return bwd_weight_impl(WgradIn{da, src0, src1, workspace}, g, WgradOut{dw, dbias, out_scale, accumulate, desc_out}, stream);
 }
 
+struct PairOps {
+    const float *da, *w_bwd; int ld_bwd; float* dxp; int accumulate; const float* x_in; int in_act; const float* pre_add; float* workspace;
+    const float *out_scale, *src0, *src1; float *dw, *dbias, *workspace_w; int accumulate_w; e2e_wgrad_reduce_desc* desc_out;
+};
+struct PairCarry { const e2e_wgrad_reduce_desc* descs; int n; long long first, items; int place; };
+#ifndef CARRY_WGS
+#define CARRY_WGS 2048
+#endif
+
+struct PairPlan { ConvArgs ad; bool data_done; WgradArgs aw; WgradLaunch lw; GemmLaunch pd; bool paired, d14; };
+
+static int bwd_pair_plan(const PairOps& q, const ConvGeom& g, const WgradOut& o, hipStream_t st, PairPlan& P, bool dry) {
+    int rc = bwd_data_setup(BwdDataOps{q.da, q.w_bwd, q.ld_bwd, q.dxp, q.accumulate, q.x_in, q.in_act, q.pre_add}, g, GemmCfg{0, 0, 0}, st, P.ad, P.data_done, dry);
+    if (rc != E2E_OK) return rc;
+    rc = wgrad_setup(WgradIn{q.da, q.src0, q.src1, q.workspace_w}, g, 0, o, st, P.aw, P.lw, dry);
+    if (rc != E2E_OK) return rc;
+    P.pd = GemmLaunch{};
+    if (!P.data_done) P.pd = plan_gemm<true>(P.ad, 4, q.workspace, GemmCfg{0, 0, 0});
+    P.d14 = P.pd.c.bm == 32 && P.pd.c.bn == 128;
+    const bool d22 = P.pd.c.bm == 64 && P.pd.c.bn == 64;
+    P.paired = !P.data_done && P.pd.kind == GK_TILE && P.pd.cb == 32 && (P.d14 || d22) && P.lw.k == WK_GEMM4_64;
+    return E2E_OK;
+}
+
+static int wgrad_reduce_range(const e2e_wgrad_reduce_desc* descs_dev, int n, long long first_item, long long items, hipStream_t st) {
+    hipLaunchKernelGGL(k_wgrad_reduce_batched, dim3((unsigned)(items < 4096 ? items : 4096)), dim3(512), 0, st, descs_dev, n, first_item, items);
+    return E2E_OK;
+}
+
+static int bwd_pair_impl(const PairOps& q, const ConvGeom& g, int wgrad_first, const PairCarry& cy, const char* who, void* stream) {
+    E2E_REQUIRE(q.desc_out, E2E_ERR_ARG, "%s: desc_out is NULL", who);
+    E2E_REQUIRE(cy.items >= 0 && cy.first >= 0 && (cy.items == 0 || (cy.descs && cy.n > 0)) && cy.place >= 0 && cy.place <= 2, E2E_ERR_ARG,
+                "%s: bad carry range", who);
+    const hipStream_t st = (hipStream_t)stream;
+    const WgradOut o{q.dw, q.dbias, q.out_scale, q.accumulate_w, q.desc_out};
+    PairPlan P;
+    const int rc = bwd_pair_plan(q, g, o, st, P, false);
+    if (rc != E2E_OK) return rc;
+    ConvArgs& ad = P.ad;
+    const WgradArgs& aw = P.aw;
+    const WgradLaunch& lw = P.lw;
+    if (P.paired) {
+        PairGrid pg;
+        pg.dgx = P.pd.g.x; pg.dgy = P.pd.g.y; pg.dgz = P.pd.g.z;
+        pg.wgx = lw.g.x; pg.wgy = lw.g.y; pg.wgz = lw.g.z;
+        const unsigned nd = pg.dgx * pg.dgy * pg.dgz, nw = pg.wgx * pg.wgy * pg.wgz;
+        pg.wgrad_first = wgrad_first ? 1 : 0;
+        pg.first = ((wgrad_first ? nw : nd) + 7u) / 8u * 8u;
+        const unsigned second = wgrad_first ? nd : nw;
+        CarryArgs ca{cy.descs, cy.n, (unsigned)(cy.items < CARRY_WGS ? cy.items : CARRY_WGS), cy.first, cy.items};
+        pg.cbeg = 0xffffffffu; pg.cpad = 0;
+        if (ca.wgs) {
+            pg.cbeg = cy.place == 0 ? pg.first + second : cy.place == 1 ? pg.first : 0u;
+            pg.cpad = cy.place == 0 ? ca.wgs : (ca.wgs + 7u) / 8u * 8u;
+        }
+        const dim3 grid(pg.first + second + pg.cpad);
+        const bool two = aw.src1 != nullptr;
+        if (P.d14) {
+            if (two) hipLaunchKernelGGL((k_conv_bwd_pair<1, 4, true>), grid, dim3(256), 0, st, ad, aw, pg, ca);
+            else hipLaunchKernelGGL((k_conv_bwd_pair<1, 4, false>), grid, dim3(256), 0, st, ad, aw, pg, ca);
+        } else {
+            if (two) hipLaunchKernelGGL((k_conv_bwd_pair<2, 2, true>), grid, dim3(256), 0, st, ad, aw, pg, ca);
+            else hipLaunchKernelGGL((k_conv_bwd_pair<2, 2, false>), grid, dim3(256), 0, st, ad, aw, pg, ca);
+        }
+    } else {
+        if (!P.data_done) launch_gemm_main<true>(ad, P.pd, q.workspace, st);
+        if (lw.k != WK_DONE) wgrad_launch_gemm(aw, lw, st);
+    }
+    if (!P.data_done) launch_gemm_tail(ad, P.pd, st);
+    if (lw.k != WK_DONE) wgrad_reduce(aw, o, lw.Sz, aw.Mpad, aw.Npad, lw.Sz >= 8 ? 8 : 2, st);
+    if (!P.paired && cy.items > 0) wgrad_reduce_range(cy.descs, cy.n, cy.first, cy.items, st);
+    E2E_LAUNCH_CHECK(who);
+    return E2E_OK;
+}
+
 int e2e_conv2d_bwd_pair_deferred(const float* da, const float* w_bwd, int ld_bwd, float* dxp, int B, int Hs, int Ws, int Cin, int Cout, int Ho, int Wo,
                                  int KH, int KW, int stride, int pad, int pad_mode, int accumulate, const float* x_in, int in_act, const float* pre_add,
                                  float* workspace, const float* out_scale, const float* src0, const float* src1, int C1, int up, float* dw, float* dbias,
                                  float* workspace_w, int accumulate_w, float in_sub, float in_mul, e2e_wgrad_reduce_desc* desc_out, int wgrad_first,
                                  void* stream) {
-    E2E_REQUIRE(desc_out, E2E_ERR_ARG, "e2e_conv2d_bwd_pair_deferred: desc_out is NULL");
-    const hipStream_t st = (hipStream_t)stream;
-    ConvArgs ad;
-    bool data_done;
     GEOM_BWD_WEIGHT(g);
-    int rc = bwd_data_setup(BwdDataOps{da, w_bwd, ld_bwd, dxp, accumulate, x_in, in_act, pre_add}, g, GemmCfg{0, 0, 0}, st, ad, data_done);
-    if (rc != E2E_OK) return rc;
-    const WgradOut o{dw, dbias, out_scale, accumulate_w, desc_out};
-    WgradArgs aw;
-    WgradLaunch lw;
-    rc = wgrad_setup(WgradIn{da, src0, src1, workspace_w}, g, 0, o, st, aw, lw);
-    if (rc != E2E_OK) return rc;
-    GemmLaunch pd{};
-    if (!data_done) pd = plan_gemm<true>(ad, 4, workspace, GemmCfg{0, 0, 0});
-    const bool d14 = pd.c.bm == 32 && pd.c.bn == 128, d22 = pd.c.bm == 64 && pd.c.bn == 64;
-    const bool paired = !data_done && pd.kind == GK_TILE && pd.cb == 32 && (d14 || d22) && lw.k == WK_GEMM4_64;
-    if (paired) {
-        PairGrid pg;
-        pg.dgx = pd.g.x; pg.dgy = pd.g.y; pg.dgz = pd.g.z;
-        pg.wgx = lw.g.x; pg.wgy = lw.g.y; pg.wgz = lw.g.z;
-        const unsigned nd = pg.dgx * pg.dgy * pg.dgz, nw = pg.wgx * pg.wgy * pg.wgz;
-        pg.wgrad_first = wgrad_first ? 1 : 0;
-        pg.first = ((wgrad_first ? nw : nd) + 7u) / 8u * 8u;
-        const dim3 grid(pg.first + (wgrad_first ? nd : nw));
-        const bool two = aw.src1 != nullptr;
-        if (d14) {
-            if (two) hipLaunchKernelGGL((k_conv_bwd_pair<1, 4, true>), grid, dim3(256), 0, st, ad, aw, pg);
-            else hipLaunchKernelGGL((k_conv_bwd_pair<1, 4, false>), grid, dim3(256), 0, st, ad, aw, pg);
-        } else {
-            if (two) hipLaunchKernelGGL((k_conv_bwd_pair<2, 2, true>), grid, dim3(256), 0, st, ad, aw, pg);
-            else hipLaunchKernelGGL((k_conv_bwd_pair<2, 2, false>), grid, dim3(256), 0, st, ad, aw, pg);
-        }
-    } else {
-        if (!data_done) launch_gemm_main<true>(ad, pd, workspace, st);
-        if (lw.k != WK_DONE) wgrad_launch_gemm(aw, lw, st);
-    }
-    if (!data_done) launch_gemm_tail(ad, pd, st);
-    if (lw.k != WK_DONE) wgrad_reduce(aw, o, lw.Sz, aw.Mpad, aw.Npad, lw.Sz >= 8 ? 8 : 2, st);
-    E2E_LAUNCH_CHECK("e2e_conv2d_bwd_pair_deferred");
-    return E2E_OK;
+    return bwd_pair_impl(PairOps{da, w_bwd, ld_bwd, dxp, accumulate, x_in, in_act, pre_add, workspace, out_scale, src0, src1, dw, dbias, workspace_w, accumulate_w, desc_out},
+                         g, wgrad_first, PairCarry{nullptr, 0, 0, 0, 0}, "e2e_conv2d_bwd_pair_deferred", stream);
+}
+
+int e2e_conv2d_bwd_pair_carry(const float* da, const float* w_bwd, int ld_bwd, float* dxp, int B, int Hs, int Ws, int Cin, int Cout, int Ho, int Wo,
+                              int KH, int KW, int stride, int pad, int pad_mode, int accumulate, const float* x_in, int in_act, const float* pre_add,
+                              float* workspace, const float* out_scale, const float* src0, const float* src1, int C1, int up, float* dw, float* dbias,
+                              float* workspace_w, int accumulate_w, float in_sub, float in_mul, e2e_wgrad_reduce_desc* desc_out, int wgrad_first,
+                              const e2e_wgrad_reduce_desc* carry_descs_dev, int carry_n, long long carry_first_item, long long carry_items, int carry_place,
+                              void* stream) {
+    GEOM_BWD_WEIGHT(g);
+    return bwd_pair_impl(PairOps{da, w_bwd, ld_bwd, dxp, accumulate, x_in, in_act, pre_add, workspace, out_scale, src0, src1, dw, dbias, workspace_w, accumulate_w, desc_out},
+                         g, wgrad_first, PairCarry{carry_descs_dev, carry_n, carry_first_item, carry_items, carry_place}, "e2e_conv2d_bwd_pair_carry", stream);
+}
+
+int e2e_conv2d_bwd_pair_is_one_launch(int ld_bwd, int B, int Hs, int Ws, int Cin, int Cout, int Ho, int Wo, int KH, int KW, int stride, int pad, int pad_mode,
+                                      int accumulate, int in_act, int has_pre_add, int has_workspace, int has_src1, int C1, int up, int has_bias) {
+    static float nowhere[4];
+    float* const x = nowhere;
+    const float in_sub = 0.f, in_mul = 1.f;
+    GEOM_BWD_WEIGHT(g);
+    e2e_wgrad_reduce_desc desc;
+    const PairOps q{x, x, ld_bwd, x, accumulate, in_act ? x : nullptr, in_act, has_pre_add ? x : nullptr, has_workspace ? x : nullptr, nullptr, x, has_src1 ? x : nullptr,
+                    x, has_bias ? x : nullptr, x, 0, &desc};
+    PairPlan P;
+    if (bwd_pair_plan(q, g, WgradOut{q.dw, q.dbias, nullptr, 0, &desc}, nullptr, P, true) != E2E_OK) return 0;
+    return P.paired ? 1 : 0;
 }
 
 long long e2e_wgrad_reduce_batch_prepare(e2e_wgrad_reduce_desc* descs_host, int n) {
@@ -2997,8 +3088,15 @@
 
 int e2e_wgrad_reduce_batched(const e2e_wgrad_reduce_desc* descs_dev, int n, long long total_items, void* stream) {
     E2E_REQUIRE(descs_dev && n > 0 && total_items > 0, E2E_ERR_ARG, "e2e_wgrad_reduce_batched: bad argument");
-    hipLaunchKernelGGL(k_wgrad_reduce_batched, dim3((unsigned)(total_items < 4096 ? total_items : 4096)), dim3(512), 0, (hipStream_t)stream, descs_dev, n, total_items);
+    wgrad_reduce_range(descs_dev, n, 0, total_items, (hipStream_t)stream);
     E2E_LAUNCH_CHECK("e2e_wgrad_reduce_batched");
+    return E2E_OK;
+}
+
+int e2e_wgrad_reduce_batched_range(const e2e_wgrad_reduce_desc* descs_dev, int n, long long first_item, long long items, void* stream) {
+    E2E_REQUIRE(descs_dev && n > 0 && first_item >= 0 && items > 0, E2E_ERR_ARG, "e2e_wgrad_reduce_batched_range: bad argument");
+    wgrad_reduce_range(descs_dev, n, first_item, items, (hipStream_t)stream);
+    E2E_LAUNCH_CHECK("e2e_wgrad_reduce_batched_range");
     return E2E_OK;
 }
 
diff --git a/end-to-end-self-supervised-slam_amd/e2ehip/netplan.py b/end-to-end-self-supervised-slam_amd/e2ehip/netplan.py
--- a/end-to-end-self-supervised-slam_amd/e2ehip/netplan.py
+++ b/end-to-end-self-supervised-slam_amd/e2ehip/netplan.py
@@ -8,6 +8,7 @@
 
 _f32 = torch.float32
 PAIR_WGRAD_FIRST = 0
+PAIR_CARRY_PLACE = 0
 
 
 class Buf:
@@ -99,10 +100,14 @@
             s.res.written = True
         if s.need_dx and plan.paired and not plan.overlap:
             pre = s.pre_from.out.g if (s.direct and s.pre_from is not None) else None
-            L.call("e2e_conv2d_bwd_pair_deferred", geom=s.geom, da=L.ptr(g), w_bwd=L.ptr(s.wb), ld_bwd=s.ldb, dxp=L.ptr(s.src0.g if s.direct else s.dxp),
-                   accumulate=(1 if s.src0.written else 0) if s.direct else 0, x_in=L.ptr(s.src0.t) if s.direct else None,
-                   in_act=s.src0.act if s.direct else 0, pre_add=L.ptr(pre), workspace=L.ptr(s.ws_b), workspace_w=L.ptr(s.ws_w), accumulate_w=0,
-                   wgrad_first=PAIR_WGRAD_FIRST, stream=st, **s._wgrad_operands(plan))
+            acc, in_act = (1 if s.src0.written else 0) if s.direct else 0, s.src0.act if s.direct else 0
+            carry = plan.carry_for(s, lambda: L.query("e2e_conv2d_bwd_pair_is_one_launch", geom=s.geom, ld_bwd=s.ldb, accumulate=acc, in_act=in_act,
+                                                      has_pre_add=1 if pre is not None else 0, has_workspace=1 if s.ws_b is not None else 0,
+                                                      has_src1=1 if s.src1 is not None else 0, has_bias=1 if s.bias is not None else 0))
+            L.call("e2e_conv2d_bwd_pair_carry" if carry else "e2e_conv2d_bwd_pair_deferred", geom=s.geom, da=L.ptr(g), w_bwd=L.ptr(s.wb), ld_bwd=s.ldb,
+                   dxp=L.ptr(s.src0.g if s.direct else s.dxp), accumulate=acc, x_in=L.ptr(s.src0.t) if s.direct else None, in_act=in_act, pre_add=L.ptr(pre),
+                   workspace=L.ptr(s.ws_b), workspace_w=L.ptr(s.ws_w), accumulate_w=0, wgrad_first=PAIR_WGRAD_FIRST, stream=st, **s._wgrad_operands(plan),
+                   **(carry or {}))
             if s.direct:
                 s.src0.written = True
             else:
@@ -117,6 +122,7 @@
             else:
                 L.call("e2e_conv2d_bwd_data", geom=s.geom, dz=L.ptr(g), w_bwd=L.ptr(s.wb), ld_bwd=s.ldb, dxp=L.ptr(s.dxp), workspace=L.ptr(s.ws_b), stream=st)
                 self._gather_adjoint(st)
+        plan.carry_for(s, None)
         st_w = plan.fork(st)
         L.call("e2e_conv2d_bwd_weight_scaled_deferred", geom=s.geom, da=L.ptr(g), workspace=L.ptr(s.ws_w), accumulate=0, stream=st_w, **s._wgrad_operands(plan))
 
@@ -210,6 +216,7 @@
         from depth_estimation.networks import BasicBlock
         self.model, self.dev, self.overlap = model, torch.device(device), overlap
         self.paired = os.environ.get("E2E_PAIRED_BWD", "1") != "0"
+        self.carry = self.paired and not overlap and os.environ.get("E2E_CARRY_REDUCE", "1") != "0"
         self.B, self.H, self.W = B, H, W
         if H % 32 or W % 32:
             raise ValueError(f"launch plan: the encoder halves the image five times and the decoder doubles it back before every skip "
@@ -272,6 +279,7 @@
         self._retired_tables = []
         self._move_tables = {}
         self._reduce_tables = {}
+        self._carrying = None
 
     def _add(self, op):
         self.ops.append(op)
@@ -398,6 +406,7 @@
         st = L.stream()
         for op in self.ops:
             op.out.written = False
+        self._begin_half("late", self.ops[self.split_index:])
         for op in reversed(self.ops[self.split_index:]):
             op.bwd(self, st)
         self.join()
@@ -411,13 +420,43 @@
             raise RuntimeError("launch plan: backward_early_layers() follows backward_late_layers()")
         for op, w in zip(self.ops, state):
             op.out.written = w
+        self._begin_half("early", self.ops[:self.split_index])
         for op in reversed(self.ops[:self.split_index]):
             op.bwd(self, st)
         self.join()
         self._reduce_weight_gradients("early", self.ops[:self.split_index])
 
+    @staticmethod
+    def _half_convs(ops):
+        return [op for op in reversed(ops) if isinstance(op, _Conv)]
+
+    def _table_key(self, convs):
+        return tuple((self.sink(op.weight).data_ptr(), self.sink(op.bias).data_ptr() if op.bias is not None else 0, op.ws_w.data_ptr(),
+                      op.scale.data_ptr() if op.scale is not None else 0) for op in convs)
+
+    def _begin_half(self, which, ops):
+        self._carrying = None
+        held = self._reduce_tables.get(which) if self.carry else None
+        if held is not None:
+            convs = self._half_convs(ops)
+            if held[4] == self._table_key(convs):
+                self._carrying = [held, convs, 0, 0]
+
+    def carry_for(self, conv, one_launch):
+        c = self._carrying
+        if c is None:
+            return None
+        (_, table, _, firsts, _), convs, i, done = c
+        if i >= len(convs) or convs[i] is not conv:
+            raise RuntimeError("launch plan: backward order differs from the reduction table's")
+        c[2] = i + 1
+        if one_launch is None or firsts[i] == done or not one_launch():
+            return None
+        c[3] = firsts[i]
+        return dict(carry_descs_dev=L.ptr(table), carry_n=len(convs), carry_first_item=done, carry_items=firsts[i] - done, carry_place=PAIR_CARRY_PLACE)
+
     def _reduce_weight_gradients(self, which, ops):
-        convs = [op for op in ops if isinstance(op, _Conv)]
+        convs = self._half_convs(ops)
         if not convs:
             return
         arr = (L.WgradReduceDesc * len(convs))(*[op.reduce_desc for op in convs])
@@ -426,13 +465,20 @@
             raise RuntimeError("launch plan: malformed backward-weight reduction descriptor")
         raw = bytes(arr)
         held = self._reduce_tables.get(which)
+        c, self._carrying = self._carrying, None
+        if c is not None:
+            if held is not c[0] or held[0] != raw or c[2] != len(convs):
+                raise RuntimeError("launch plan: the backward-weight reduction table changed while its reductions were being carried")
+            if c[3] < total:
+                L.call("e2e_wgrad_reduce_batched_range", L.ptr(held[1]), len(convs), c[3], total - c[3], L.stream())
+            return
         if held is None or held[0] != raw:
             if torch.cuda.is_current_stream_capturing():
                 raise RuntimeError("launch plan: the backward-weight reduction table changed under stream capture; run the plan eagerly once first")
             table = torch.frombuffer(bytearray(raw), dtype=torch.uint8).to(self.dev)
             if held is not None:
                 self._retired_tables.append(held[1])
-            held = self._reduce_tables[which] = (raw, table, total)
+            held = self._reduce_tables[which] = (raw, table, total, [d.first_item for d in arr], self._table_key(convs))
         L.call("e2e_wgrad_reduce_batched", L.ptr(held[1]), len(convs), held[2], L.stream())
 
     def split_offset(self, flat):
diff --git a/include/e2eslam.h b/include/e2eslam.h
--- a/include/e2eslam.h
+++ b/include/e2eslam.h
@@ -309,8 +309,23 @@
                                  float* dbias, float* workspace_w, int accumulate_w, float in_sub,
                                  float in_mul, e2e_wgrad_reduce_desc* desc_out_host, int wgrad_first,
                                  void* stream);
+int e2e_conv2d_bwd_pair_carry(const float* da, const float* w_bwd, int ld_bwd, float* dxp, int B, int Hs,
+                              int Ws, int Cin, int Cout, int Ho, int Wo, int KH, int KW, int stride,
+                              int pad, int pad_mode, int accumulate, const float* x_in, int in_act,
+                              const float* pre_add, float* workspace, const float* out_scale,
+                              const float* src0, const float* src1, int C1, int up, float* dw,
+                              float* dbias, float* workspace_w, int accumulate_w, float in_sub,
+                              float in_mul, e2e_wgrad_reduce_desc* desc_out_host, int wgrad_first,
+                              const e2e_wgrad_reduce_desc* carry_descs_dev, int carry_n,
+                              long long carry_first_item, long long carry_items, int carry_place,
+                              void* stream);
+int e2e_conv2d_bwd_pair_is_one_launch(int ld_bwd, int B, int Hs, int Ws, int Cin, int Cout, int Ho, int Wo,
+                                      int KH, int KW, int stride, int pad, int pad_mode, int accumulate,
+                                      int in_act, int has_pre_add, int has_workspace, int has_src1, int C1,
+                                      int up, int has_bias);
 long long e2e_wgrad_reduce_batch_prepare(e2e_wgrad_reduce_desc* descs_host, int n);
 int e2e_wgrad_reduce_batched(const e2e_wgrad_reduce_desc* descs_dev, int n, long long total_items, void* stream);
+int e2e_wgrad_reduce_batched_range(const e2e_wgrad_reduce_desc* descs_dev, int n, long long first_item, long long items, void* stream);
 
 typedef struct e2e_copy_desc {
     const void* src;
```
